# Jonetz/TreeDetection

Measured on AMD Instinct MI355X. Metric: tiles/sec (1000x1000 RGB+nDSM) predict_tiles model stage, higher is better.
Workload: dtype f32

## Files before the change

### include/treedet.h

```cpp
#ifndef TREEDET_H
#define TREEDET_H

#include <stddef.h>
#include <stdint.h>

#ifdef __cplusplus
extern "C" {
#endif

typedef int td_status;
typedef struct td_engine td_engine;

enum {
    TD_OK = 0,
    TD_ERR_INVALID = -1,
    TD_ERR_HIP = -2,
    TD_ERR_WEIGHTS = -3,
    TD_ERR_CAPACITY = -4,
    TD_ERR_STATE = -5,
    TD_ERR_UNSUPPORTED = -6
};

enum { TD_PRECISION_FP32 = 0, TD_PRECISION_FP16 = 1 };
enum { TD_INPUT_F32_CHW = 0,
       TD_INPUT_U8_HWC = 1 };

typedef struct td_model_desc {
    int32_t num_classes;
    int32_t precision;
    int32_t pre_nms_topk;
    int32_t post_nms_topk;
    int32_t detections_per_image;
    float rpn_nms_thresh;
    float score_thresh;
    float nms_thresh;
    float mask_thresh;
} td_model_desc;

typedef struct td_tensor_desc {
    const char* name;
    const float* data;
    int32_t ndim;
    int64_t shape[4];
} td_tensor_desc;

#define TD_MASK_SIDE 28

typedef struct td_detections {
    float* boxes;
    float* scores;
    int32_t* classes;
    int32_t* count;
    float* mask_probs;
    int32_t* mask_region;
    int64_t* mask_offset;
    uint32_t* mask_bits;
    int64_t mask_words_per_image;
} td_detections;

void td_model_desc_default(td_model_desc* desc);
td_status td_engine_create(const td_model_desc* desc, int device, td_engine** out);
td_status td_engine_load_weights(td_engine* e, const td_tensor_desc* tensors, size_t n);
td_status td_engine_reserve(td_engine* e, int max_batch, int max_hp, int max_wp);
td_status td_engine_forward(td_engine* e, const void* images, int input_format, const int32_t* hw_valid,
                            const int32_t* hw_out, int B, int Hp, int Wp, void* stream, td_detections* out);
#define TD_PHASE_STEM 6
td_status td_engine_forward_phase(td_engine* e, int phase, const void* images, int input_format, const int32_t* hw_valid,
                                  const int32_t* hw_out, int B, int Hp, int Wp, void* stream, td_detections* out);
td_status td_engine_tensor(td_engine* e, const char* name, void** dev_ptr, int64_t dims[4], int* elem_size);
td_status td_engine_read_tensor(td_engine* e, const char* name, void* dst_dev, int64_t bytes, void* stream);
#define TD_PROF_CATEGORIES 9
td_status td_engine_profile_enable(td_engine* e, int enable);
td_status td_engine_profile_read(td_engine* e, double* ms, int64_t* launches, double* flops, double* bytes, int reset);
#define TD_PROF_CLASSES 7
#define TD_CLS_WINO_GEMM 0
#define TD_CLS_WINO_XFORM 1
#define TD_CLS_CONV1X1 2
#define TD_CLS_CONV3X3 3
#define TD_CLS_FC 4
#define TD_CLS_MASK_HEAD 5
#define TD_CLS_TAIL 6
#define TD_PEAK_F32_MFMA_TFLOPS 157.3
#define TD_PEAK_F16_MFMA_TFLOPS 2500.0
#define TD_HBM_ACHIEVABLE_TBS 6.3
td_status td_engine_profile_classes(td_engine* e, double* ms, int64_t* launches, double* exec_flops, double* bytes, double* tmin_ms, int reset);
const char* td_last_error(void);
void td_engine_destroy(td_engine* e);

td_status td_resize_tile_u8(const uint8_t* src, int h, int w, int c, uint8_t* dst, int out_h, int out_w,
                            int dst_pitch_px, void* tmp_dev , void* stream);
td_status td_resize_batch_u8(const uint8_t* const* src_tiles, int n, int h, int w, int c, uint8_t* dst, int out_h,
                             int out_w, int dst_pitch_px, int64_t dst_image_stride_bytes, void* tmp_dev, void* stream);
td_status td_resize_bilinear_f64(const double* src, int c, int h, int w, float* dst, int out_h, int out_w, int dst_pitch_px,
                                 int64_t dst_plane_stride, void* stream);
td_status td_windows_u16_to_input(const uint16_t* raster, int height, int width, int c, const int32_t* windows, int n, int32_t* band1_max,
                                  float* dst, int out_h, int out_w, int dst_pitch_px, int64_t dst_plane_stride, int64_t dst_image_stride,
                                  void* stream);
void td_resize_shape(int h, int w, int short_edge, int max_size, int* out_h, int* out_w);

td_status td_bottleneck_tail_nhwc(const void* x, const void* w2, const float* scale2, const float* bias2, const void* w3,
                                  const float* scale3, const float* bias3, const void* shortcut, void* y, int B, int H, int W,
                                  int mid, int cout, int precision, void* stream);
td_status td_conv2d_nhwc(const void* x, const void* w, const float* scale, const float* bias,
                         const void* residual, int res_shift, void* y, int B, int H, int W, int Cin,
                         int Cout, int KH, int KW, int stride, int pad, int relu, int precision,
                         void* stream);
td_status td_conv2d_rows_nhwc(const void* x, const void* w, const float* scale, const float* bias, void* y, int B, int H, int W,
                              int Cin, int Cout, int KH, int KW, int pad, int relu, int out_mode, const int32_t* rows_dyn,
                              int rows_mul, int precision, void* stream);
td_status td_conv2d_head_nhwc(const void* x, const void* w, const float* bias, const void* head_w, const float* head_b,
                              float* head_y, int B, int H, int W, int Cin, int KH, int KW, int pad, int head_n, int precision,
                              void* stream);
td_status td_conv2d_winograd_nhwc(const float* x, const float* w, const float* scale, const float* bias, float* y, int B,
                                  int H, int W, int Cin, int Cout, int relu, void* stream);
td_status td_conv2d_winograd_head_nhwc(const float* x, const float* w, const float* bias, const float* head_w, const float* head_b,
                                       float* head_y, int B, int H, int W, int Cin, int head_n, void* stream);
td_status td_conv_path(const int32_t* rules, int64_t wino_elems, const int32_t* layer, const int32_t* call, const int32_t* head,
                       int32_t* out);
typedef struct td_workspace_row {
    char name[32];
    char public_name[32];
    int32_t kind;
    int32_t elem_size;
    int32_t phase;
    int32_t pad_;
    int64_t dims[4];
    int64_t alloc_bytes;
} td_workspace_row;
td_status td_workspace_plan(int precision, int winograd, int post_nms_topk, int detections_per_image, const int32_t* widths, int B,
                            int Hp, int Wp, td_workspace_row* rows, int cap, int* n_rows);
td_status td_nms(const float* boxes, const float* scores, int n, float iou_thresh, int32_t* keep_idx,
                 int32_t* keep_count, void* stream);
td_status td_roi_align(const void* feat, int H, int W, int C, const float* rois, int R, float spatial_scale,
                       int pooled, void* out, int precision, void* stream);
td_status td_paste_masks(const float* mask_probs, const float* boxes, int n, int out_h, int out_w,
                         float thresh, int32_t* mask_region, int64_t* mask_offset, uint32_t* mask_bits,
                         int64_t mask_words_cap, void* stream);

td_status td_paste_masks_batch(const float* mask_probs, const float* boxes, const int32_t* counts, const int32_t* out_hw,
                               int batch, int dets_per_image, float thresh, int32_t* mask_region, int64_t* mask_offset,
                               uint32_t* mask_bits, int64_t mask_words_per_image, void* stream);

#define TD_CONTOUR_MAX 256
td_status td_trace_contours_dev(const int32_t* mask_region, const int64_t* mask_offset, const uint32_t* mask_bits,
                                int64_t mask_words_per_image, const int32_t* counts, int batch, int dets_per_image,
                                int16_t* points, int points_cap, int32_t* image_points, int32_t* det_info,
                                int32_t* contour_info, void* stream);

int td_find_contours(const uint8_t* img, int h, int w, int32_t* points, int max_points, int32_t* starts,
                     int max_contours);
int td_tile_polygons_json(const int32_t* mask_region, const int64_t* mask_offset, const uint32_t* mask_bits,
                          int64_t mask_words, const float* scores, const int32_t* classes, int n,
                          const double* transform, const char* image_id, char* buf, int64_t cap, int64_t* needed);

int td_tile_prediction_file(int device, const int32_t* mask_region, const int64_t* mask_offset, const uint32_t* mask_bits_dev,
                            uint32_t* rows_host, int64_t mask_words, const float* scores, const int32_t* classes, int n,
                            const double* transform, const char* image_id, const char* path, int64_t* bytes_written);

int td_batch_prediction_files(int device, int n_tiles, int dets_per_image, const int32_t* mask_region, const int64_t* mask_offset,
                              const uint32_t* mask_bits_dev, uint32_t* rows_host, int64_t bits_stride_words, const float* scores,
                              const int32_t* classes, const int32_t* counts, const double* transforms, const char* image_id,
                              const char* const* paths, int threads, int32_t* status, int64_t* bytes_written);

int64_t td_tiff_lzw_decode(const uint8_t* src, int64_t n, uint8_t* dst, int64_t cap);
int64_t td_tiff_packbits_decode(const uint8_t* src, int64_t n, uint8_t* dst, int64_t cap);
int64_t td_tiff_lzw_encode(const uint8_t* src, int64_t n, uint8_t* dst, int64_t cap);
td_status td_tiff_lzw_decode_dev(const uint8_t* comp, const int64_t* block_off, const int64_t* block_nbytes, int nblocks,
                                 uint8_t* blocks_out, int64_t block_cap, int64_t* decoded, int32_t* status, void* stream);
td_status td_tiff_inflate_dev(const uint8_t* comp, const int64_t* block_off, const int64_t* block_nbytes, int nblocks,
                              uint8_t* blocks_out, int64_t block_cap, int64_t* decoded, int32_t* status, void* stream);
td_status td_tiff_inflate_verified_dev(const uint8_t* comp, const int64_t* block_off, const int64_t* block_nbytes, int nblocks,
                                       uint8_t* blocks_out, int64_t block_cap, int64_t* decoded, int32_t* status, int64_t* end_off,
                                       void* stream);
td_status td_tiff_adler32_blocks_dev(const uint8_t* blocks, int64_t block_cap, const int64_t* decoded, const uint8_t* comp,
                                     const int64_t* block_off, const int64_t* block_nbytes, const int64_t* end_off, int nblocks,
                                     int32_t* status, void* stream);
td_status td_adler32_dev(const uint8_t* data_dev, int64_t n, uint32_t* out_dev, void* stream);
int64_t td_tiff_inflate(const uint8_t* src, int64_t n, uint8_t* dst, int64_t cap);
int64_t td_tiff_inflate_verified(const uint8_t* src, int64_t n, uint8_t* dst, int64_t cap);
int64_t td_tiff_zstd_decode(const uint8_t* src, int64_t n, uint8_t* dst, int64_t cap);
#define TD_ZSTD_STATS 32
int64_t td_zstd_stream_stats(const uint8_t* src, int64_t n, int64_t* counters);
td_status td_tiff_zstd_decode_dev(const uint8_t* comp, const int64_t* block_off, const int64_t* block_nbytes, int nblocks,
                                  uint8_t* blocks_out, int64_t block_cap, int64_t* decoded, int32_t* status, uint8_t* scratch,
                                  int64_t scratch_bytes, void* stream);
int64_t td_tiff_zstd_scratch_bytes(int nblocks);
td_status td_tiff_blocks_to_image_dev(const uint8_t* blocks, int64_t block_cap, int block_w, int block_h, int blocks_across,
                                      int blocks_down, int spp, int predictor, uint8_t* image, int width, int height, void* stream);
td_status td_tiff_blocks_to_image_u16_dev(const uint8_t* blocks, int64_t block_cap, int block_w, int block_h, int blocks_across,
                                          int blocks_down, int spp, int predictor, uint16_t* image, int width, int height, void* stream);
td_status td_tiff_blocks_to_image_f32_dev(const uint8_t* blocks, int64_t block_cap, int block_w, int block_h, int blocks_across,
                                          int blocks_down, int spp, int predictor, float* image, int width, int height, void* stream);
td_status td_tiff_planes_to_image_dev(const uint8_t* blocks, int64_t block_cap, int block_w, int block_h, int blocks_across,
                                      int blocks_down, int spp, int plane_mask, int predictor, uint8_t* image, int width, int height,
                                      void* stream);
td_status td_tiff_planes_to_image_u16_dev(const uint8_t* blocks, int64_t block_cap, int block_w, int block_h, int blocks_across,
                                          int blocks_down, int spp, int plane_mask, int predictor, uint16_t* image, int width, int height,
                                          void* stream);
td_status td_tiff_planes_to_image_f32_dev(const uint8_t* blocks, int64_t block_cap, int block_w, int block_h, int blocks_across,
                                          int blocks_down, int spp, int plane_mask, int predictor, float* image, int width, int height,
                                          void* stream);
#define TD_JPEG_TABSET_BYTES 11904
td_status td_tiff_jpeg_plan(const uint8_t* tables, int64_t tables_len, const uint8_t* data, const int64_t* block_off,
                            const int64_t* block_nbytes, int nblocks, int photometric, int bands, int block_w, const int32_t* block_rows,
                            int64_t* block_info, int64_t* segs, int64_t seg_cap, void* tabsets, int64_t tabset_cap, int64_t* totals);
td_status td_tiff_jpeg_decode_dev(const uint8_t* comp, const int64_t* block_info, int nblocks, const int64_t* segs, int nseg,
                                  const void* tabsets, int16_t* coef, uint8_t* planes, int64_t coef_count, int32_t* status, uint8_t* image,
                                  int width, int height, int bands, int block_w, int block_h, int blocks_across, void* stream);
int64_t td_jpeg_decode(const uint8_t* src, int64_t n, uint8_t* dst, int64_t cap, int32_t* shape);
td_status td_tiff_jpeg_decode_long_dev(const uint8_t* comp, const int64_t* block_info, int nblocks, const int64_t* segs_short, int nshort,
                                       const int64_t* segs_long, int nlong, int subseq_bytes, const void* tabsets, int16_t* coef,
                                       uint8_t* planes, int64_t coef_count, int32_t* status, int64_t* stats, uint8_t* image, int width,
                                       int height, int bands, int block_w, int block_h, int blocks_across, void* stream);
int64_t td_jpeg_decode_sync(const uint8_t* src, int64_t n, uint8_t* dst, int64_t cap, int32_t* shape, int subseq_bytes, int lanes,
                            int64_t* stats);
int64_t td_read_window(int fd, int64_t file_off, int64_t row_stride, int64_t row_bytes, int64_t rows, uint8_t* dst);
int64_t td_read_windows(int fd, int n, const int64_t* file_off, int64_t row_stride, const int64_t* row_bytes, const int64_t* rows,
                        uint8_t* dst, const int64_t* dst_off, int threads);
int td_tiff_unpredict(void* data, int64_t rows, int64_t cols, int samples, int bytes_per_sample);
int td_tiff_unpredict_float(void* data, int64_t rows, int64_t cols, int samples, int bytes_per_sample);

int td_tile_polygons_json_dev(const int16_t* points, int64_t points_cap, const int32_t* det_info, const int32_t* contour_info,
                              const int32_t* mask_region, const int64_t* mask_offset, const uint32_t* mask_bits,
                              int64_t mask_words, const float* scores, const int32_t* classes, int n,
                              const double* transform, const char* image_id, char* buf, int64_t cap, int64_t* needed);

int td_simplify_ring(const double* xy, int n, double tolerance, double* out_xy, int out_cap);

int td_ring_is_valid(const double* xy, int n);
int td_stitch_tile_json(const char* json, int64_t len, const double* box, double tolerance, int32_t srs_id,
                        uint8_t* blobs, int64_t blob_cap, int64_t* blob_offsets, double* scores, int max_features,
                        int64_t* needed_bytes, int* needed_features);

int td_stitch_tile_files(const char* paths, const int64_t* path_offsets, int n_files, const double* boxes, double tolerance,
                         const int32_t* srs_ids, int threads, uint8_t* blobs, int64_t blob_cap, int64_t* blob_offsets,
                         double* scores, int max_features, int32_t* file_status, int64_t* needed_bytes, int* needed_features);

int td_region_relate(const double* ring_xy, const int64_t* ring_start, const int32_t* ring_poly, int n_rings,
                     const double* query_xy, const int64_t* query_start, int n_queries, uint8_t* flags);

#define TD_RELATE_QUERY_CAP 256
#define TD_RELATE_MEET_CAP 254
#define TD_RELATE_RING_CAP 64
td_status td_region_relate_dev(const double* ring_xy, const int64_t* ring_start, const int32_t* ring_poly, int n_rings, int64_t n_vertices,
                               const int32_t* edge_ring, const int32_t* bin_start, const int32_t* bin_edges, int n_bins,
                               int64_t n_bin_edges, double ymin, double ymax, double inv_h, const double* query_xy,
                               const int64_t* query_start, int n_queries, int64_t n_query_vertices, uint8_t* flags, int32_t* status,
                               int check_index, void* stream);

td_status td_crown_stats(const float* raster, int rows, int cols, const double* transform, const int32_t* window,
                         const float* circles, int n, int mode, float radius_scale, float* out, void* stream);

#define TD_ZONAL_RING_CAP 512
td_status td_crown_zonal_dev(const float* raster, int rows, int cols, const double* transform, const double* xy, int64_t n_xy,
                             const int64_t* start, int n, float* out, int32_t* pos, int32_t* status, void* stream);
// ... 46 lines not shown
```

### treedetection_amd/_lib.py

```python
from __future__ import annotations

import ctypes as C
import os
import threading
from typing import Optional

_HERE = os.path.dirname(os.path.abspath(__file__))
LIB_PATH = os.path.join(_HERE, "libtreedet_hip.so")

_lib: Optional[C.CDLL] = None
ERR_INVALID = -1
ERR_CAPACITY = -4
ERR_STATE = -5
ERR_UNSUPPORTED = -6
JPEG_TABSET_BYTES = 11904
SAMPLE_U8, SAMPLE_F32, SAMPLE_U16 = 0, 1, 2
RESAMPLE_MODES = {"f32": 0, "u8": 1, "ndvi": 2}
ZSTD_STATS = ("frames block_raw block_rle block_comp max_blocks_per_frame lit_raw lit_rle lit_huff lit_treeless lit_streams_1 lit_streams_4 "
              "hufw_direct hufw_fse seq0 LL_predef LL_rle LL_fse LL_repeat OF_predef OF_rle OF_fse OF_repeat ML_predef ML_rle ML_fse ML_repeat "
              "window_desc single_segment checksum seq_long seq_2byte skippable").split()
RING_PAIR_CAP, RING_PAIR_WPB, RING_PAIR_GRID = 1024, 4, 2048
RELATE_QUERY_CAP, RELATE_MEET_CAP, RELATE_RING_CAP = 256, 254, 64
ZONAL_RING_CAP = 512


class TdError(RuntimeError):
    """A libtreedet_hip call returned a negative status (message from td_last_error)."""


class ModelDesc(C.Structure):
    _fields_ = [("num_classes", C.c_int32), ("precision", C.c_int32), ("pre_nms_topk", C.c_int32),
                ("post_nms_topk", C.c_int32), ("detections_per_image", C.c_int32),
                ("rpn_nms_thresh", C.c_float), ("score_thresh", C.c_float), ("nms_thresh", C.c_float),
                ("mask_thresh", C.c_float)]


class TensorDesc(C.Structure):
    _fields_ = [("name", C.c_char_p), ("data", C.c_void_p), ("ndim", C.c_int32), ("shape", C.c_int64 * 4)]


class SeamSource(C.Structure):
    _fields_ = [("data", C.c_void_p), ("pitch", C.c_int64), ("rows", C.c_int32), ("row0", C.c_int32), ("col0", C.c_int32),
                ("r_lo", C.c_int32), ("c_lo", C.c_int32), ("r_hi", C.c_int32), ("c_hi", C.c_int32), ("has_own", C.c_int32),
                ("own", C.c_double)]


class WorkspaceRow(C.Structure):
    _fields_ = [("name", C.c_char * 32), ("public_name", C.c_char * 32), ("kind", C.c_int32), ("elem_size", C.c_int32),
                ("phase", C.c_int32), ("pad_", C.c_int32), ("dims", C.c_int64 * 4), ("alloc_bytes", C.c_int64)]


class Detections(C.Structure):
    _fields_ = [("boxes", C.c_void_p), ("scores", C.c_void_p), ("classes", C.c_void_p), ("count", C.c_void_p),
                ("mask_probs", C.c_void_p), ("mask_region", C.c_void_p), ("mask_offset", C.c_void_p),
                ("mask_bits", C.c_void_p), ("mask_words_per_image", C.c_int64)]


SIGNATURES = {
    "td_model_desc_default": (None, [C.POINTER(ModelDesc)]),
    "td_engine_create": (C.c_int, [C.POINTER(ModelDesc), C.c_int, C.POINTER(C.c_void_p)]),
    "td_engine_load_weights": (C.c_int, [C.c_void_p, C.POINTER(TensorDesc), C.c_size_t]),
    "td_engine_reserve": (C.c_int, [C.c_void_p, C.c_int, C.c_int, C.c_int]),
    "td_engine_forward": (C.c_int, [C.c_void_p, C.c_void_p, C.c_int, C.POINTER(C.c_int32), C.POINTER(C.c_int32),
                                    C.c_int, C.c_int, C.c_int, C.c_void_p, C.POINTER(Detections)]),
    "td_engine_forward_phase": (C.c_int, [C.c_void_p, C.c_int, C.c_void_p, C.c_int, C.POINTER(C.c_int32), C.POINTER(C.c_int32),
                                          C.c_int, C.c_int, C.c_int, C.c_void_p, C.POINTER(Detections)]),
    "td_engine_tensor": (C.c_int, [C.c_void_p, C.c_char_p, C.POINTER(C.c_void_p), C.POINTER(C.c_int64),
                                   C.POINTER(C.c_int)]),
    "td_engine_read_tensor": (C.c_int, [C.c_void_p, C.c_char_p, C.c_void_p, C.c_int64, C.c_void_p]),
    "td_engine_profile_enable": (C.c_int, [C.c_void_p, C.c_int]),
    "td_engine_profile_read": (C.c_int, [C.c_void_p, C.POINTER(C.c_double), C.POINTER(C.c_int64), C.POINTER(C.c_double),
                                         C.POINTER(C.c_double), C.c_int]),
    "td_engine_profile_classes": (C.c_int, [C.c_void_p, C.POINTER(C.c_double), C.POINTER(C.c_int64), C.POINTER(C.c_double),
                                            C.POINTER(C.c_double), C.POINTER(C.c_double), C.c_int]),
    "td_last_error": (C.c_char_p, []),
    "td_engine_destroy": (None, [C.c_void_p]),
    "td_resize_tile_u8": (C.c_int, [C.c_void_p, C.c_int, C.c_int, C.c_int, C.c_void_p, C.c_int, C.c_int, C.c_int,
                                    C.c_void_p, C.c_void_p]),
    "td_resize_batch_u8": (C.c_int, [C.POINTER(C.c_void_p), C.c_int, C.c_int, C.c_int, C.c_int, C.c_void_p, C.c_int, C.c_int,
                                     C.c_int, C.c_int64, C.c_void_p, C.c_void_p]),
    "td_bottleneck_tail_nhwc": (C.c_int, [C.c_void_p] * 9 + [C.c_int] * 6 + [C.c_void_p]),
    "td_resize_bilinear_f64": (C.c_int, [C.c_void_p, C.c_int, C.c_int, C.c_int, C.c_void_p, C.c_int, C.c_int, C.c_int, C.c_int64, C.c_void_p]),
    "td_windows_u16_to_input": (C.c_int, [C.c_void_p, C.c_int, C.c_int, C.c_int, C.c_void_p, C.c_int, C.c_void_p, C.c_void_p, C.c_int, C.c_int,
                                          C.c_int, C.c_int64, C.c_int64, C.c_void_p]),
    "td_resize_shape": (None, [C.c_int, C.c_int, C.c_int, C.c_int, C.POINTER(C.c_int), C.POINTER(C.c_int)]),
    "td_conv2d_nhwc": (C.c_int, [C.c_void_p, C.c_void_p, C.c_void_p, C.c_void_p, C.c_void_p, C.c_int, C.c_void_p]
                       + [C.c_int] * 11 + [C.c_void_p]),
    "td_conv2d_rows_nhwc": (C.c_int, [C.c_void_p] * 5 + [C.c_int] * 10 + [C.c_void_p, C.c_int, C.c_int, C.c_void_p]),
    "td_conv2d_head_nhwc": (C.c_int, [C.c_void_p] * 6 + [C.c_int] * 9 + [C.c_void_p]),
    "td_conv2d_winograd_head_nhwc": (C.c_int, [C.c_void_p] * 6 + [C.c_int] * 5 + [C.c_void_p]),
    "td_conv2d_winograd_nhwc": (C.c_int, [C.c_void_p] * 5 + [C.c_int] * 6 + [C.c_void_p]),
    "td_conv_path": (C.c_int, [C.POINTER(C.c_int32), C.c_int64, C.POINTER(C.c_int32), C.POINTER(C.c_int32), C.POINTER(C.c_int32),
                               C.POINTER(C.c_int32)]),
    "td_workspace_plan": (C.c_int, [C.c_int] * 4 + [C.POINTER(C.c_int32)] + [C.c_int] * 3 + [C.POINTER(WorkspaceRow), C.c_int, C.POINTER(C.c_int)]),
    "td_nms": (C.c_int, [C.c_void_p, C.c_void_p, C.c_int, C.c_float, C.c_void_p, C.c_void_p, C.c_void_p]),
    "td_roi_align": (C.c_int, [C.c_void_p, C.c_int, C.c_int, C.c_int, C.c_void_p, C.c_int, C.c_float, C.c_int,
                               C.c_void_p, C.c_int, C.c_void_p]),
    "td_paste_masks": (C.c_int, [C.c_void_p, C.c_void_p, C.c_int, C.c_int, C.c_int, C.c_float, C.c_void_p,
                                 C.c_void_p, C.c_void_p, C.c_int64, C.c_void_p]),
    "td_paste_masks_batch": (C.c_int, [C.c_void_p, C.c_void_p, C.c_void_p, C.POINTER(C.c_int32), C.c_int, C.c_int, C.c_float,
                                       C.c_void_p, C.c_void_p, C.c_void_p, C.c_int64, C.c_void_p]),
    "td_crown_stats": (C.c_int, [C.c_void_p, C.c_int, C.c_int, C.POINTER(C.c_double), C.POINTER(C.c_int32), C.c_void_p, C.c_int,
                                 C.c_int, C.c_float, C.c_void_p, C.c_void_p]),
    "td_crown_zonal_dev": (C.c_int, [C.c_void_p, C.c_int, C.c_int, C.POINTER(C.c_double), C.c_void_p, C.c_int64, C.c_void_p, C.c_int,
                                     C.c_void_p, C.c_void_p, C.c_void_p, C.c_void_p]),
    "td_crown_zonal": (C.c_int, [C.c_void_p, C.c_int, C.c_int, C.POINTER(C.c_double), C.c_void_p, C.c_int64, C.c_void_p, C.c_int,
                                 C.c_void_p, C.c_void_p, C.c_void_p]),
    "td_crown_labels_dev": (C.c_int, [C.c_int, C.c_int, C.POINTER(C.c_double), C.c_void_p, C.c_int64, C.c_void_p, C.c_void_p, C.c_int,
                                      C.c_void_p, C.c_void_p, C.c_void_p]),
    "td_crown_labels": (C.c_int, [C.c_int, C.c_int, C.POINTER(C.c_double), C.c_void_p, C.c_int64, C.c_void_p, C.c_void_p, C.c_int,
                                  C.c_void_p, C.c_void_p]),
    "td_resample_gdal_dev": (C.c_int, [C.c_void_p, C.c_int, C.c_int, C.c_int, C.c_int, C.POINTER(C.c_int32), C.c_int]
                             + [C.c_void_p] * 4 + [C.c_int, C.c_int64] + [C.c_void_p] * 4 + [C.c_int, C.c_int64]
                             + [C.c_void_p, C.c_void_p, C.c_int, C.c_void_p]),
    "td_seam_first_dev": (C.c_int, [C.c_void_p, C.c_int, C.c_int, C.c_int, C.c_int, C.c_double, C.POINTER(SeamSource), C.POINTER(SeamSource),
                                    C.c_void_p]),
    "td_crown_pairs_count": (C.c_int, [C.c_void_p, C.c_void_p, C.c_int, C.c_float, C.c_uint16, C.c_void_p, C.c_float, C.c_void_p, C.c_void_p,
                                       C.c_void_p]),
    "td_crown_pairs_fill": (C.c_int, [C.c_void_p, C.c_void_p, C.c_int, C.c_float, C.c_uint16, C.c_void_p, C.c_void_p, C.c_void_p, C.c_void_p]),
    "td_crown_pairs_greedy": (C.c_int, [C.c_void_p, C.c_void_p, C.c_void_p, C.c_void_p, C.c_int, C.c_void_p]),
    "td_ring_pairs_area_dev": (C.c_int, [C.c_void_p, C.c_void_p, C.c_int, C.c_void_p, C.c_void_p, C.c_int, C.c_void_p, C.c_int64, C.c_void_p,
                                         C.c_void_p, C.c_void_p]),
    "td_ring_pairs_area": (C.c_int, [C.c_void_p, C.c_void_p, C.c_int, C.c_void_p, C.c_void_p, C.c_int, C.c_void_p, C.c_int64, C.c_void_p,
                                     C.c_void_p]),
    "td_trace_contours_dev": (C.c_int, [C.c_void_p, C.c_void_p, C.c_void_p, C.c_int64, C.c_void_p, C.c_int, C.c_int, C.c_void_p,
                                        C.c_int, C.c_void_p, C.c_void_p, C.c_void_p, C.c_void_p]),
    "td_find_contours": (C.c_int, [C.c_void_p, C.c_int, C.c_int, C.c_void_p, C.c_int, C.c_void_p, C.c_int]),
    "td_batch_prediction_files": (C.c_int, [C.c_int, C.c_int, C.c_int, C.c_void_p, C.c_void_p, C.c_void_p, C.c_void_p, C.c_int64, C.c_void_p,
                                          C.c_void_p, C.c_void_p, C.c_void_p, C.c_char_p, C.POINTER(C.c_char_p), C.c_int, C.c_void_p, C.c_void_p]),
    "td_tiff_lzw_decode": (C.c_int64, [C.c_void_p, C.c_int64, C.c_void_p, C.c_int64]),
    "td_tiff_packbits_decode": (C.c_int64, [C.c_void_p, C.c_int64, C.c_void_p, C.c_int64]),
    "td_tiff_lzw_encode": (C.c_int64, [C.c_void_p, C.c_int64, C.c_void_p, C.c_int64]),
    "td_tiff_inflate": (C.c_int64, [C.c_void_p, C.c_int64, C.c_void_p, C.c_int64]),
    "td_tiff_inflate_dev": (C.c_int, [C.c_void_p, C.c_void_p, C.c_void_p, C.c_int, C.c_void_p, C.c_int64, C.c_void_p, C.c_void_p, C.c_void_p]),
    "td_tiff_inflate_verified": (C.c_int64, [C.c_void_p, C.c_int64, C.c_void_p, C.c_int64]),
    "td_tiff_inflate_verified_dev": (C.c_int, [C.c_void_p, C.c_void_p, C.c_void_p, C.c_int, C.c_void_p, C.c_int64, C.c_void_p, C.c_void_p, C.c_void_p,
                                               C.c_void_p]),
    "td_tiff_zstd_decode": (C.c_int64, [C.c_void_p, C.c_int64, C.c_void_p, C.c_int64]),
    "td_zstd_stream_stats": (C.c_int64, [C.c_void_p, C.c_int64, C.c_void_p]),
    "td_tiff_zstd_decode_dev": (C.c_int, [C.c_void_p, C.c_void_p, C.c_void_p, C.c_int, C.c_void_p, C.c_int64, C.c_void_p, C.c_void_p, C.c_void_p,
                                          C.c_int64, C.c_void_p]),
    "td_tiff_zstd_scratch_bytes": (C.c_int64, [C.c_int]),
    "td_tiff_adler32_blocks_dev": (C.c_int, [C.c_void_p, C.c_int64, C.c_void_p, C.c_void_p, C.c_void_p, C.c_void_p, C.c_void_p, C.c_int, C.c_void_p,
                                             C.c_void_p]),
    "td_adler32_dev": (C.c_int, [C.c_void_p, C.c_int64, C.c_void_p, C.c_void_p]),
    "td_tiff_lzw_decode_dev": (C.c_int, [C.c_void_p, C.c_void_p, C.c_void_p, C.c_int, C.c_void_p, C.c_int64, C.c_void_p, C.c_void_p, C.c_void_p]),
    "td_tiff_blocks_to_image_dev": (C.c_int, [C.c_void_p, C.c_int64, C.c_int, C.c_int, C.c_int, C.c_int, C.c_int, C.c_int, C.c_void_p, C.c_int, C.c_int, C.c_void_p]),
    "td_tiff_blocks_to_image_u16_dev": (C.c_int, [C.c_void_p, C.c_int64, C.c_int, C.c_int, C.c_int, C.c_int, C.c_int, C.c_int, C.c_void_p, C.c_int,
                                                  C.c_int, C.c_void_p]),
    "td_tiff_blocks_to_image_f32_dev": (C.c_int, [C.c_void_p, C.c_int64, C.c_int, C.c_int, C.c_int, C.c_int, C.c_int, C.c_int, C.c_void_p, C.c_int,
                                                  C.c_int, C.c_void_p]),
    "td_tiff_planes_to_image_dev": (C.c_int, [C.c_void_p, C.c_int64, C.c_int, C.c_int, C.c_int, C.c_int, C.c_int, C.c_int, C.c_int, C.c_void_p,
                                              C.c_int, C.c_int, C.c_void_p]),
    "td_tiff_planes_to_image_u16_dev": (C.c_int, [C.c_void_p, C.c_int64, C.c_int, C.c_int, C.c_int, C.c_int, C.c_int, C.c_int, C.c_int, C.c_void_p,
                                                  C.c_int, C.c_int, C.c_void_p]),
    "td_tiff_planes_to_image_f32_dev": (C.c_int, [C.c_void_p, C.c_int64, C.c_int, C.c_int, C.c_int, C.c_int, C.c_int, C.c_int, C.c_int, C.c_void_p,
                                                  C.c_int, C.c_int, C.c_void_p]),
    "td_tiff_jpeg_plan": (C.c_int, [C.c_void_p, C.c_int64, C.c_void_p, C.c_void_p, C.c_void_p, C.c_int, C.c_int, C.c_int, C.c_int, C.c_void_p,
                                    C.c_void_p, C.c_void_p, C.c_int64, C.c_void_p, C.c_int64, C.c_void_p]),
    "td_tiff_jpeg_decode_dev": (C.c_int, [C.c_void_p, C.c_void_p, C.c_int, C.c_void_p, C.c_int, C.c_void_p, C.c_void_p, C.c_void_p, C.c_int64,
                                          C.c_void_p, C.c_void_p] + [C.c_int] * 6 + [C.c_void_p]),
    "td_jpeg_decode": (C.c_int64, [C.c_void_p, C.c_int64, C.c_void_p, C.c_int64, C.c_void_p]),
    "td_tiff_jpeg_decode_long_dev": (C.c_int, [C.c_void_p, C.c_void_p, C.c_int, C.c_void_p, C.c_int, C.c_void_p, C.c_int, C.c_int, C.c_void_p,
                                               C.c_void_p, C.c_void_p, C.c_int64, C.c_void_p, C.c_void_p, C.c_void_p] + [C.c_int] * 6 + [C.c_void_p]),
    "td_jpeg_decode_sync": (C.c_int64, [C.c_void_p, C.c_int64, C.c_void_p, C.c_int64, C.c_void_p, C.c_int, C.c_int, C.c_void_p]),
    "td_read_windows": (C.c_int64, [C.c_int, C.c_int, C.c_void_p, C.c_int64, C.c_void_p, C.c_void_p, C.c_void_p, C.c_void_p, C.c_int]),
    "td_tiff_unpredict": (C.c_int, [C.c_void_p, C.c_int64, C.c_int64, C.c_int, C.c_int]),
    "td_tiff_unpredict_float": (C.c_int, [C.c_void_p, C.c_int64, C.c_int64, C.c_int, C.c_int]),
    "td_region_relate": (C.c_int, [C.c_void_p, C.c_void_p, C.c_void_p, C.c_int, C.c_void_p, C.c_void_p, C.c_int, C.c_void_p]),
    "td_region_relate_dev": (C.c_int, [C.c_void_p, C.c_void_p, C.c_void_p, C.c_int, C.c_int64, C.c_void_p, C.c_void_p, C.c_void_p, C.c_int, C.c_int64,
                                       C.c_double, C.c_double, C.c_double, C.c_void_p, C.c_void_p, C.c_int, C.c_int64, C.c_void_p, C.c_void_p,
                                       C.c_int, C.c_void_p]),
    "td_simplify_ring": (C.c_int, [C.c_void_p, C.c_int, C.c_double, C.c_void_p, C.c_int]),
    "td_ring_is_valid": (C.c_int, [C.c_void_p, C.c_int]),
    "td_stitch_tile_json": (C.c_int, [C.c_char_p, C.c_int64, C.POINTER(C.c_double), C.c_double, C.c_int32, C.c_void_p,
                                      C.c_int64, C.c_void_p, C.c_void_p, C.c_int, C.POINTER(C.c_int64), C.POINTER(C.c_int)]),
    "td_stitch_tile_files": (C.c_int, [C.c_char_p, C.c_void_p, C.c_int, C.c_void_p, C.c_double, C.c_void_p, C.c_int, C.c_void_p, C.c_int64,
                                       C.c_void_p, C.c_void_p, C.c_int, C.c_void_p, C.POINTER(C.c_int64), C.POINTER(C.c_int)]),
    "td_tile_polygons_json_dev": (C.c_int, [C.c_void_p, C.c_int64, C.c_void_p, C.c_void_p, C.c_void_p, C.c_void_p, C.c_void_p, C.c_int64,
                                            C.c_void_p, C.c_void_p, C.c_int, C.POINTER(C.c_double), C.c_char_p, C.c_void_p, C.c_int64,
                                            C.POINTER(C.c_int64)]),
    "td_read_window": (C.c_int64, [C.c_int, C.c_int64, C.c_int64, C.c_int64, C.c_int64, C.c_void_p]),
    "td_tile_prediction_file": (C.c_int, [C.c_int, C.c_void_p, C.c_void_p, C.c_void_p, C.c_void_p, C.c_int64, C.c_void_p, C.c_void_p,
                                          C.c_int, C.POINTER(C.c_double), C.c_char_p, C.c_char_p, C.POINTER(C.c_int64)]),
    "td_tile_polygons_json": (C.c_int, [C.c_void_p, C.c_void_p, C.c_void_p, C.c_int64, C.c_void_p, C.c_void_p, C.c_int,
                                        C.POINTER(C.c_double), C.c_char_p, C.c_void_p, C.c_int64, C.POINTER(C.c_int64)]),
}


def load() -> C.CDLL:
    global _lib
    if _lib is not None:
        return _lib
    host_only = os.environ.get("TD_HOST_LIB")
    if host_only:
        lib = C.CDLL(host_only, mode=C.RTLD_GLOBAL)
        for name, (res, args) in SIGNATURES.items():
            fn = getattr(lib, name, None)
            if fn is not None:
                fn.restype = res
                fn.argtypes = args
        _lib = lib
        return lib
    if not os.path.exists(LIB_PATH):
        raise TdError(f"{LIB_PATH} not found — build it first: python -c 'import __graft_entry__ as g; g.build()' "
                      f"(or make -C treedetection_amd/csrc). There is no CPU fallback.")
    import torch

    lib = C.CDLL(LIB_PATH, mode=C.RTLD_GLOBAL)
    for name, (res, args) in SIGNATURES.items():
        fn = getattr(lib, name)
        fn.restype = res
        fn.argtypes = args
    _lib = lib
    return lib


def check(status: int, what: str = "") -> None:
    if status < 0:
        msg = load().td_last_error().decode("utf-8", "replace")
        raise TdError(f"{what or 'libtreedet_hip'} failed ({status}): {msg}")


CONV_FORMS = ("direct", "split", "winograd F(2x2)", "winograd F(4x4)", "winograd F(4x4) folded")
CONV_HEADS = ("own launch", "in the output transform", "if the tile owns 256 channels")


def conv_path(rules, wino_elems, layer, call, head=None) -> dict:
    arr = lambda v, n: (C.c_int32 * n)(*[int(x) for x in v])
    out = (C.c_int32 * 10)()
    check(load().td_conv_path(arr(rules, 8), int(wino_elems), arr(layer, 9), arr(call, 10), arr(head, 9) if head is not None else None, out),
          "td_conv_path")
    return {"form": CONV_FORMS[out[0]], "head": CONV_HEADS[out[1]], "key": tuple(out[3:8]) if out[2] else None,
            "slab_tiles": out[8], "fold_group": out[9]}
# ... 42 lines not shown
```

### treedetection_amd/csrc/api.cpp

```cpp
#include "common.h"
#include "detect.h"
#include <cstdarg>
#include <cstdio>
#include <cmath>
#include <cstdlib>
#include <vector>


namespace {
td_status scratch(void** p, size_t bytes) {
    TD_HIP_CHECK(hipMalloc(p, bytes ? bytes : 16));
    return TD_OK;
}
}

extern "C" {

void td_model_desc_default(td_model_desc* d) {
    d->num_classes = 1;
    d->precision = TD_PRECISION_FP32;
    d->pre_nms_topk = 1000;
    d->post_nms_topk = 1000;
    d->detections_per_image = 100;
    d->rpn_nms_thresh = 0.7f;
    d->score_thresh = 0.3f;
    d->nms_thresh = 0.5f;
    d->mask_thresh = 0.5f;
}

static td_status conv2d_api(ConvArgs& a, int precision, void* stream);

td_status td_conv2d_nhwc(const void* x, const void* w, const float* scale, const float* bias,
                         const void* residual, int res_shift, void* y, int B, int H, int W, int Cin,
                         int Cout, int KH, int KW, int stride, int pad, int relu, int precision,
                         void* stream) {
    TD_REQUIRE(x && w && y, "td_conv2d_nhwc: null pointer");
    TD_REQUIRE(stride >= 1 && KH >= 1 && KW >= 1 && B >= 1, "td_conv2d_nhwc: bad geometry");
    ConvArgs a{};
    a.x = x; a.w = w; a.scale = scale; a.bias = bias; a.res = residual; a.y = y;
    a.B = B; a.H = H; a.W = W; a.Cin = Cin; a.Cout = Cout; a.KH = KH; a.KW = KW;
    a.stride = stride; a.pad = pad;
    a.Ho = (H + 2 * pad - KH) / stride + 1;
    a.Wo = (W + 2 * pad - KW) / stride + 1;
    a.res_shift = res_shift; a.relu = relu; a.out_mode = 0;
    a.M = B * a.Ho * a.Wo; a.m_dyn = nullptr; a.m_mul = 1;
    a.out_f32 = (precision & 0x10000) && (precision & 0xff) == TD_PRECISION_FP16 ? 1 : 0;
    a.tile_cfg = ((precision >> 8) & 0xff) - 1;
    a.tile_strict = (precision & 0x20000) ? 1 : 0;
    return conv2d_api(a, precision, stream);
}

td_status td_conv2d_rows_nhwc(const void* x, const void* w, const float* scale, const float* bias, void* y, int B, int H, int W,
                              int Cin, int Cout, int KH, int KW, int pad, int relu, int out_mode, const int32_t* rows_dyn,
                              int rows_mul, int precision, void* stream) {
    TD_REQUIRE(x && w && y, "td_conv2d_rows_nhwc: null pointer");
    TD_REQUIRE(KH >= 1 && KW >= 1 && B >= 1, "td_conv2d_rows_nhwc: bad geometry");
    TD_REQUIRE(out_mode == 0 || out_mode == 1, "td_conv2d_rows_nhwc: out_mode %d (0 plain, 1 pixel shuffle)", out_mode);
    TD_REQUIRE(!rows_dyn || rows_mul >= 1, "td_conv2d_rows_nhwc: rows_mul %d with a device row count", rows_mul);
    ConvArgs a{};
    a.x = x; a.w = w; a.scale = scale; a.bias = bias; a.y = y;
    a.B = B; a.H = H; a.W = W; a.Cin = Cin; a.Cout = Cout; a.KH = KH; a.KW = KW;
    a.stride = 1; a.pad = pad;
    a.Ho = H + 2 * pad - KH + 1;
    a.Wo = W + 2 * pad - KW + 1;
    a.relu = relu; a.out_mode = out_mode;
    a.M = B * a.Ho * a.Wo; a.m_dyn = rows_dyn; a.m_mul = rows_dyn ? rows_mul : 1;
    a.out_f32 = (precision & 0x10000) && (precision & 0xff) == TD_PRECISION_FP16 ? 1 : 0;
    a.tile_cfg = ((precision >> 8) & 0xff) - 1;
    a.tile_strict = (precision & 0x20000) ? 1 : 0;
    return conv2d_api(a, precision, stream);
}

td_status td_conv2d_head_nhwc(const void* x, const void* w, const float* bias, const void* head_w, const float* head_b,
                              float* head_y, int B, int H, int W, int Cin, int KH, int KW, int pad, int head_n, int precision,
                              void* stream) {
    TD_REQUIRE(x && w && head_w && head_y, "td_conv2d_head_nhwc: null pointer");
    TD_REQUIRE((precision & 0xff) == TD_PRECISION_FP16, "td_conv2d_head_nhwc: float16 tensors only");
    TD_REQUIRE(KH >= 1 && KW >= 1 && B >= 1 && head_n >= 1 && head_n <= 32, "td_conv2d_head_nhwc: bad geometry");
    ConvArgs a{};
    a.x = x; a.w = w; a.bias = bias;
    a.B = B; a.H = H; a.W = W; a.Cin = Cin; a.Cout = 256; a.KH = KH; a.KW = KW;
    a.stride = 1; a.pad = pad;
    a.Ho = H + 2 * pad - KH + 1;
    a.Wo = W + 2 * pad - KW + 1;
    a.relu = 1; a.M = B * a.Ho * a.Wo; a.m_mul = 1;
    a.tile_cfg = ((precision >> 8) & 0xff) - 1;
    TD_REQUIRE(conv_head_capable(a.tile_cfg, TD_PRECISION_FP16), "td_conv2d_head_nhwc: tile id %d does not own 256 output channels per block", a.tile_cfg);
    a.head_w = head_w; a.head_b = head_b; a.head_y = head_y; a.head_n = head_n;
    a.y = head_y;
    return conv2d_api(a, precision, stream);
}

static td_status conv2d_api(ConvArgs& a, int precision, void* stream) {
    hipStream_t s = static_cast<hipStream_t>(stream);
    ConvArgs with_frag = a;
    with_frag.w_frag = a.w;
    with_frag.w_split = a.w;
    if (conv_tile(a.tile_cfg) && conv_tile(a.tile_cfg)->family == TILE_SPLIT && !conv_tile_refusal(a.tile_cfg, with_frag, precision & 0xff)) {
        const size_t n = (size_t)a.Cout * a.Cin;
        std::vector<float> wh(n);
        std::vector<unsigned char> packed;
        TD_HIP_CHECK(hipStreamSynchronize(s));
        TD_HIP_CHECK(hipMemcpy(wh.data(), a.w, n * sizeof(float), hipMemcpyDeviceToHost));
        conv_split_pack(wh.data(), a.Cout, a.Cin, packed);
        void* ws = nullptr;
        td_status st = scratch(&ws, packed.size());
        if (st < 0) return st;
        hipError_t herr = hipMemcpy(ws, packed.data(), packed.size(), hipMemcpyHostToDevice);
        a.w_split = ws;
        if (herr == hipSuccess) st = conv2d_launch(a, precision & 0xff, s);
        hipError_t herr2 = hipStreamSynchronize(s);
        (void)hipFree(ws);
        if (st < 0) return st;
        TD_HIP_CHECK(herr);
        TD_HIP_CHECK(herr2);
        return TD_OK;
    }
    if (!conv_tile(a.tile_cfg) || !conv_tile(a.tile_cfg)->frag || conv_tile_refusal(a.tile_cfg, with_frag, precision & 0xff))
        return conv2d_launch(a, precision & 0xff, s);
    const int es = (precision & 0xff) == TD_PRECISION_FP16 ? 2 : 4;
    const size_t n = (size_t)a.Cout * a.KH * a.KW * a.Cin;
    std::vector<unsigned char> bits(n * es), packed;
    TD_HIP_CHECK(hipStreamSynchronize(s));
    TD_HIP_CHECK(hipMemcpy(bits.data(), a.w, n * es, hipMemcpyDeviceToHost));
    conv_bd_pack(bits.data(), es, a.Cout, a.KH, a.KW, a.Cin, packed);
    void* wf = nullptr;
    td_status st = scratch(&wf, packed.size());
    if (st < 0) return st;
    hipError_t herr = hipMemcpy(wf, packed.data(), packed.size(), hipMemcpyHostToDevice);
    a.w_frag = wf;
    if (herr == hipSuccess) st = conv2d_launch(a, precision & 0xff, s);
    hipError_t herr2 = hipStreamSynchronize(s);
    (void)hipFree(wf);
    if (st < 0) return st;
    TD_HIP_CHECK(herr);
    TD_HIP_CHECK(herr2);
    return TD_OK;
}

static td_status wino_api(const float* x, const float* w, const float* scale, const float* bias, float* y, int B, int H, int W, int Cin,
                          int Cout, int relu, void* stream, const float* head_w, const float* head_b, float* head_y, int head_n);

td_status td_conv2d_winograd_nhwc(const float* x, const float* w, const float* scale, const float* bias, float* y, int B, int H,
                                  int W, int Cin, int Cout, int relu, void* stream) {
    TD_REQUIRE(y, "td_conv2d_winograd_nhwc: bad arguments");
    return wino_api(x, w, scale, bias, y, B, H, W, Cin, Cout, relu, stream, nullptr, nullptr, nullptr, 0);
}

td_status td_conv2d_winograd_head_nhwc(const float* x, const float* w, const float* bias, const float* head_w, const float* head_b,
                                       float* head_y, int B, int H, int W, int Cin, int head_n, void* stream) {
    TD_REQUIRE(head_w && head_y && head_n >= 1 && head_n <= 32, "td_conv2d_winograd_head_nhwc: bad arguments");
    return wino_api(x, w, nullptr, bias, nullptr, B, H, W, Cin, 256, 1, stream, head_w, head_b, head_y, head_n);
}

static td_status wino_api(const float* x, const float* w, const float* scale, const float* bias, float* y, int B, int H, int W, int Cin,
                          int Cout, int relu, void* stream, const float* head_w, const float* head_b, float* head_y, int head_n) {
    TD_REQUIRE(x && w && B >= 1 && H >= 1 && W >= 1, "td_conv2d_winograd_nhwc: bad arguments");
    TD_REQUIRE(Cin % 32 == 0 && Cout % 4 == 0, "td_conv2d_winograd_nhwc: Cin must be a multiple of 32, Cout of 4");
    hipStream_t s = static_cast<hipStream_t>(stream);
    const char* tenv = getenv("TD_WINO_TILE");
    const bool f43 = head_w || (tenv && atoi(tenv) == 4);
    const int P = f43 ? 36 : 16;
    const size_t T = f43 ? (size_t)B * ((H + 3) / 4) * ((W + 3) / 4) : (size_t)B * ((H + 1) / 2) * ((W + 1) / 2);
    std::vector<float> wh((size_t)Cout * 9 * Cin), uh((size_t)P * Cout * Cin);
    TD_HIP_CHECK(hipMemcpy(wh.data(), w, wh.size() * sizeof(float), hipMemcpyDeviceToHost));
    if (f43) wino43_filter_transform(wh.data(), Cout, Cin, uh.data());
    else wino_filter_transform(wh.data(), Cout, Cin, uh.data());
    void *U = nullptr, *V = nullptr, *Mb = nullptr;
    td_status st;
    if ((st = scratch(&U, uh.size() * 4)) < 0 || (st = scratch(&V, P * T * Cin * 4)) < 0 || (st = scratch(&Mb, P * T * Cout * 4)) < 0) {
        (void)hipFree(U); (void)hipFree(V); (void)hipFree(Mb);
        return st;
    }
    TD_HIP_CHECK(hipMemcpy(U, uh.data(), uh.size() * 4, hipMemcpyHostToDevice));
    const char* folde = getenv("TD_WINO_FOLD");
    const bool fold = f43 && !head_w && folde && atoi(folde) != 0;
    if (fold) TD_REQUIRE(wino43_fused_ok(B, H, W, Cin, Cout), "td_conv2d_winograd_nhwc: TD_WINO_FOLD needs Cin %% 128 == 0, Cout %% 64 == 0");
    const char* fenv = getenv("TD_WINO_FUSED");
    WinoRun r{};
    r.form = fold ? CONV_WINO43_FOLD : f43 ? CONV_WINO43 : CONV_WINO22;
    r.fused_input = !fenv || atoi(fenv) != 0;
    r.slab_tiles = (int)T; r.fold_group = B;
    r.x = x; r.U = static_cast<float*>(U); r.scale = scale; r.bias = bias; r.y = y;
    r.B = B; r.H = H; r.W = W; r.cin = Cin; r.cout = Cout; r.relu = relu;
    r.V = static_cast<float*>(V); r.M = static_cast<float*>(Mb); r.m_mul = 1; r.gemm_cfg = -1;
    r.head_w = head_w; r.head_b = head_b; r.head_y = head_y; r.head_n = head_n;
    st = wino_run(r, s);
    hipError_t herr = hipStreamSynchronize(s);
    (void)hipFree(U); (void)hipFree(V); (void)hipFree(Mb);
    if (st < 0) return st;
    TD_HIP_CHECK(herr);
    return TD_OK;
}

td_status td_resize_tile_u8(const uint8_t* src, int h, int w, int c, uint8_t* dst, int out_h, int out_w,
                            int dst_pitch_px, void* tmp_dev, void* stream) {
    return resize_tile_u8_launch(src, h, w, c, dst, out_h, out_w, dst_pitch_px, tmp_dev, static_cast<hipStream_t>(stream));
}

td_status td_resize_batch_u8(const uint8_t* const* src_tiles, int n, int h, int w, int c, uint8_t* dst, int out_h,
                             int out_w, int dst_pitch_px, int64_t dst_image_stride_bytes, void* tmp_dev, void* stream) {
    return resize_batch_u8_launch(src_tiles, n, h, w, c, dst, out_h, out_w, dst_pitch_px, (size_t)dst_image_stride_bytes,
                                  tmp_dev, static_cast<hipStream_t>(stream));
}

td_status td_bottleneck_tail_nhwc(const void* x, const void* w2, const float* scale2, const float* bias2, const void* w3,
                                  const float* scale3, const float* bias3, const void* shortcut, void* y, int B, int H, int W,
                                  int mid, int cout, int precision, void* stream) {
    TD_REQUIRE(x && w2 && w3 && shortcut && y && B > 0 && H > 0 && W > 0, "td_bottleneck_tail_nhwc: null argument or empty tensor");
    TailArgs a{};
    a.x = x; a.w2 = w2; a.scale2 = scale2; a.bias2 = bias2; a.w3 = w3; a.scale3 = scale3; a.bias3 = bias3; a.res = shortcut; a.y = y;
    a.B = B; a.H = H; a.W = W; a.MID = mid; a.COUT = cout; a.M = B * H * W;
    return bottleneck_tail_launch(a, precision, static_cast<hipStream_t>(stream));
}

td_status td_resize_bilinear_f64(const double* src, int c, int h, int w, float* dst, int out_h, int out_w, int dst_pitch_px,
                                 int64_t dst_plane_stride, void* stream) {
    return resize_bilinear_f64_launch(src, c, h, w, dst, out_h, out_w, dst_pitch_px, (long long)dst_plane_stride, static_cast<hipStream_t>(stream));
}

td_status td_windows_u16_to_input(const uint16_t* raster, int height, int width, int c, const int32_t* windows, int n, int32_t* band1_max,
                                  float* dst, int out_h, int out_w, int dst_pitch_px, int64_t dst_plane_stride, int64_t dst_image_stride,
                                  void* stream) {
    return windows_u16_to_input_launch(raster, height, width, c, windows, n, band1_max, dst, out_h, out_w, dst_pitch_px,
                                       (long long)dst_plane_stride, (long long)dst_image_stride, static_cast<hipStream_t>(stream));
}

void td_resize_shape(int h, int w, int short_edge, int max_size, int* out_h, int* out_w) {
    const double scale = (double)short_edge / (double)(h < w ? h : w);
    double newh, neww;
    if (h < w) { newh = short_edge; neww = scale * w; }
    else { newh = scale * h; neww = short_edge; }
    const double mx = newh > neww ? newh : neww;
    if (mx > max_size) {
        const double s2 = (double)max_size / mx;
        newh *= s2;
        neww *= s2;
    }
    *out_h = (int)(newh + 0.5);
    *out_w = (int)(neww + 0.5);
}

td_status td_nms(const float* boxes, const float* scores, int n, float iou_thresh, int32_t* keep_idx,
                 int32_t* keep_count, void* stream) {
    TD_REQUIRE(boxes && scores && keep_idx && keep_count, "td_nms: null pointer");
    TD_REQUIRE(n >= 0 && n <= 32768, "td_nms: n=%d must be in [0, 32768]", n);
    hipStream_t s = static_cast<hipStream_t>(stream);
    if (n == 0) {
        TD_HIP_CHECK(hipMemsetAsync(keep_count, 0, sizeof(int32_t), s));
        return TD_OK;
    }
    void *sb = nullptr, *ss = nullptr, *si = nullptr, *sc = nullptr, *mk = nullptr, *kp = nullptr;
    td_status st;
    if ((st = scratch(&sb, sizeof(float) * 4 * n)) < 0) return st;
    if ((st = scratch(&ss, sizeof(float) * n)) < 0) return st;
    if ((st = scratch(&si, sizeof(int) * n)) < 0) return st;
    if ((st = scratch(&sc, sizeof(int))) < 0) return st;
    if ((st = scratch(&mk, sizeof(unsigned long long) * n * td_cdiv(n, 64))) < 0) return st;
    if ((st = scratch(&kp, sizeof(int) * n)) < 0) return st;
    if (n > 1024) {
        st = nms_big_launch(boxes, scores, n, iou_thresh, (float*)sb, (float*)ss, (int*)si, (int*)sc, (unsigned long long*)mk, (int*)kp, keep_count, s);
    } else {
        st = sort_boxes_launch(boxes, scores, nullptr, nullptr, 1, n, (float*)sb, (float*)ss, (int*)si, (int*)sc, s);
        if (st >= 0) st = nms_launch((float*)sb, (int*)sc, nullptr, 1, n, iou_thresh, (unsigned long long*)mk, (int*)kp, keep_count, n, s);
    }
    if (st >= 0) st = gather_keep_launch((int*)si, (int*)kp, keep_count, n, keep_idx, s);
    hipError_t herr = hipStreamSynchronize(s);
    (void)hipFree(sb); (void)hipFree(ss); (void)hipFree(si); (void)hipFree(sc); (void)hipFree(mk); (void)hipFree(kp);
    if (st < 0) return st;
    TD_HIP_CHECK(herr);
    return TD_OK;
}

td_status td_roi_align(const void* feat, int H, int W, int C, const float* rois, int R, float spatial_scale,
                       int pooled, void* out, int precision, void* stream) {
    TD_REQUIRE(feat && rois && out, "td_roi_align: null pointer");
    TD_REQUIRE(H >= 1 && W >= 1 && pooled >= 1 && R >= 0, "td_roi_align: bad geometry");
    if (R == 0) return TD_OK;
    return roi_align_single_launch(feat, H, W, C, rois, R, spatial_scale, pooled, out, precision, static_cast<hipStream_t>(stream));
}

td_status td_paste_masks(const float* mask_probs, const float* boxes, int n, int out_h, int out_w, float thresh,
                         int32_t* mask_region, int64_t* mask_offset, uint32_t* mask_bits, int64_t mask_words_cap,
                         void* stream) {
    TD_REQUIRE(mask_probs && boxes && mask_region && mask_offset && mask_bits, "td_paste_masks: null pointer");
    TD_REQUIRE(n >= 0 && n <= 1024 && out_h >= 1 && out_w >= 1, "td_paste_masks: bad shape");
    if (n == 0) return TD_OK;
    hipStream_t s = static_cast<hipStream_t>(stream);
    void* cnt = nullptr;
    td_status st = scratch(&cnt, sizeof(int));
    if (st < 0) return st;
    TD_HIP_CHECK(hipMemcpy(cnt, &n, sizeof(int), hipMemcpyHostToDevice));
    ImgSizes outsz{};
    outsz.h[0] = out_h;
    outsz.w[0] = out_w;
    st = paste_masks_launch(mask_probs, boxes, (int*)cnt, outsz, 1, n, thresh, mask_region,
                            reinterpret_cast<long long*>(mask_offset), mask_bits, mask_words_cap, s);
    hipError_t herr = hipStreamSynchronize(s);
    (void)hipFree(cnt);
    if (st < 0) return st;
    TD_HIP_CHECK(herr);
    return TD_OK;
}

td_status td_paste_masks_batch(const float* mask_probs, const float* boxes, const int32_t* counts, const int32_t* out_hw,
                               int batch, int dets_per_image, float thresh, int32_t* mask_region, int64_t* mask_offset,
                               uint32_t* mask_bits, int64_t mask_words_per_image, void* stream) {
    TD_REQUIRE(mask_probs && boxes && counts && out_hw && mask_region && mask_offset && mask_bits,
               "td_paste_masks_batch: null pointer");
    TD_REQUIRE(batch >= 1 && batch <= TD_MAX_BATCH && dets_per_image >= 1 && dets_per_image <= 1024,
               "td_paste_masks_batch: batch %d (max %d) / detections per image %d (max 1024)", batch, TD_MAX_BATCH, dets_per_image);
    ImgSizes outsz{};
    for (int i = 0; i < batch; ++i) {
        TD_REQUIRE(out_hw[2 * i] >= 1 && out_hw[2 * i + 1] >= 1, "td_paste_masks_batch: bad output size of image %d", i);
        outsz.h[i] = out_hw[2 * i];
        outsz.w[i] = out_hw[2 * i + 1];
        const int64_t need = (int64_t)dets_per_image * ((outsz.w[i] + 2 + 31) / 32) * outsz.h[i];
        TD_REQUIRE(mask_words_per_image >= need, "td_paste_masks_batch: image %d needs %lld mask words, capacity %lld", i,
                   (long long)need, (long long)mask_words_per_image);
    }
    return paste_masks_launch(mask_probs, boxes, counts, outsz, batch, dets_per_image, thresh, mask_region,
                              reinterpret_cast<long long*>(mask_offset), mask_bits, mask_words_per_image,
                              static_cast<hipStream_t>(stream));
}

}
```

### treedetection_amd/csrc/bottleneck.hip

```cpp
#include "common.h"
#include "conv_tiles.h"
#include <cstdlib>
#include <utility>

namespace {

constexpr int cmax(int x, int y) { return x > y ? x : y; }

template <typename F, int... I>
__device__ __forceinline__ void static_for_impl(F&& f, std::integer_sequence<int, I...>) {
    (f(std::integral_constant<int, I>{}), ...);
}
template <int N, typename F>
__device__ __forceinline__ void static_for(F&& f) {
    static_for_impl(f, std::make_integer_sequence<int, N>{});
}

template <typename T, int MID, bool OVERLAP, int MT, bool FAST = false>
struct TailGeom {
    static constexpr int ES = sizeof(T);
    static constexpr int KE = Elem<T>::PER_CHUNK;
    static constexpr int KC = MID / KE;
    static constexpr int BM = 64 * MT, THREADS = 256, LDROWS = 32;
    static constexpr int NT1 = MID / 64;
    static constexpr int STAGE1 = 2 * (BM + MID) * CHUNK_BYTES;
    static constexpr int W3_BYTES = KC * 128 * CHUNK_BYTES;
    static_assert(!FAST || MT == 1, "the wave-private epilogue is written for 64-row blocks");
    static constexpr int EPI_BYTES = FAST ? 4 * 16 * 64 * 4 : conv_epilogue_lds_bytes<T, MT, 2, 2, 2, 1, false>();
    static constexpr int EPI_OFF = OVERLAP || (FAST && ES == 2) ? W3_BYTES : 0;
    static constexpr int R0 = cmax(STAGE1, cmax(W3_BYTES, EPI_OFF + EPI_BYTES));
    static constexpr int T2_BYTES = KC * BM * CHUNK_BYTES;
    static constexpr int LDS_BYTES = R0 + T2_BYTES;
    static constexpr int BPC = 160 * 1024 / LDS_BYTES >= 4 ? 4 : 160 * 1024 / LDS_BYTES;
};

template <typename T, int MID, bool OVERLAP, int MT, bool FAST>
__device__ __forceinline__ void bottleneck_tail_body(const TailArgs& a, char* lds) {
    typedef TailGeom<T, MID, OVERLAP, MT, FAST> G;
    constexpr int ES = G::ES, KE = G::KE, KC = G::KC, BM = G::BM, LDROWS = G::LDROWS, NT1 = G::NT1;
    constexpr int AROWS = BM / LDROWS, BROWS1 = MID / LDROWS, BROWS3 = 128 / LDROWS;
    char* As = lds;
    char* Bs = lds + 2 * BM * CHUNK_BYTES;
    char* W3s = lds;
    char* Epi = lds + G::EPI_OFF;
    char* T2s = lds + G::R0;

    const int M = a.M;
    const int nblk = (M + BM - 1) / BM;
    if ((int)blockIdx.x >= nblk) return;
    const int m0 = xcd_remap(blockIdx.x, nblk) * BM;
    const int tid = threadIdx.x;
    const int lane = tid & 63, wave = tid >> 6;
    const int wm = wave >> 1, wn = wave & 1;
    const int ld_c = tid & 7, ld_r = tid >> 3;

    const int K2 = 9 * MID;
    const int nit = 9 * KC;
    const unsigned pix_bytes = (unsigned)MID * ES;
    const __amdgpu_buffer_rsrc_t xrsrc = __builtin_amdgcn_make_buffer_rsrc(
        const_cast<void*>(a.x), 0, (int)((size_t)a.B * a.H * a.W * pix_bytes), 0x00020000);
    const __amdgpu_buffer_rsrc_t w2rsrc = __builtin_amdgcn_make_buffer_rsrc(
        const_cast<void*>(a.w2), 0, (int)((size_t)MID * K2 * ES), 0x00020000);
    const __amdgpu_buffer_rsrc_t w3rsrc = __builtin_amdgcn_make_buffer_rsrc(
        const_cast<void*>(a.w3), 0, (int)((size_t)a.COUT * MID * ES), 0x00020000);
    constexpr unsigned OOB = 0xfffffff0u;
    const unsigned src_piece = (unsigned)(ld_c ^ ((ld_r >> 1) & 7)) * 16;

    unsigned a_off[AROWS], a_ok[AROWS];
#pragma unroll
    for (int i = 0; i < AROWS; ++i) {
        const int m = m0 + ld_r + LDROWS * i;
        a_off[i] = 0;
        a_ok[i] = 0;
        if (m < M) {
            const int hw = a.H * a.W;
            const int b = m / hw;
            const int rem = m - b * hw;
            const int oy = rem / a.W;
            const int ox = rem - oy * a.W;
            const int iy0 = oy - 1, ix0 = ox - 1;
            a_off[i] = (unsigned)((b * a.H + iy0) * a.W + ix0) * pix_bytes + src_piece;
            for (int ky = 0; ky < 3; ++ky)
                for (int kx = 0; kx < 3; ++kx)
                    if ((unsigned)(iy0 + ky) < (unsigned)a.H && (unsigned)(ix0 + kx) < (unsigned)a.W)
                        a_ok[i] |= 1u << (ky * 3 + kx);
        }
    }
    unsigned b_off[BROWS1];
#pragma unroll
    for (int i = 0; i < BROWS1; ++i) b_off[i] = (unsigned)(ld_r + LDROWS * i) * (unsigned)K2 * ES + src_piece;

    typedef __attribute__((address_space(3))) void lds_void;
    const unsigned wave_rows = (unsigned)__builtin_amdgcn_readfirstlane(wave) * 8u;
    int ld_tap = 0, ld_ky = 0, ld_kx = 0, ld_cc = 0;
    auto stage = [&](int buf) {
        const unsigned xs = (unsigned)(ld_ky * a.W + ld_kx) * pix_bytes + (unsigned)ld_cc * CHUNK_BYTES;
        const unsigned ws = (unsigned)ld_tap * pix_bytes + (unsigned)ld_cc * CHUNK_BYTES;
#pragma unroll
        for (int i = 0; i < AROWS; ++i) {
            const unsigned off = ((a_ok[i] >> ld_tap) & 1u) ? a_off[i] + xs : OOB;
            char* dst = As + ((unsigned)buf * BM + (unsigned)LDROWS * i + wave_rows) * CHUNK_BYTES;
            __builtin_amdgcn_raw_ptr_buffer_load_lds(xrsrc, (lds_void*)dst, 16, off, 0, 0, 0);
        }
#pragma unroll
        for (int i = 0; i < BROWS1; ++i) {
            char* dst = Bs + ((unsigned)buf * MID + (unsigned)LDROWS * i + wave_rows) * CHUNK_BYTES;
            __builtin_amdgcn_raw_ptr_buffer_load_lds(w2rsrc, (lds_void*)dst, 16, b_off[i] + ws, 0, 0, 0);
        }
        if (++ld_kx == 3) {
            ld_kx = 0;
            ++ld_ky;
        }
        if (++ld_tap == 9) {
            ld_tap = 0;
            ld_ky = 0;
            ld_kx = 0;
            ++ld_cc;
        }
    };

    const unsigned swz = (lane >> 1) & 7, hi = lane >> 5;
    unsigned frag_off[4];
#pragma unroll
    for (int kk = 0; kk < 4; ++kk) frag_off[kk] = (unsigned)(lane & 31) * CHUNK_BYTES + (((unsigned)(2 * kk) + hi) ^ swz) * 16;

    float sc2[NT1], bi2[NT1];
#pragma unroll
    for (int j = 0; j < NT1; ++j) {
        const int n = wn * 32 * NT1 + j * 32 + (lane & 31);
        sc2[j] = a.scale2 ? a.scale2[n] : 1.f;
        bi2[j] = a.bias2 ? a.bias2[n] : 0.f;
    }
    constexpr int NP = MID / 32;
    [[maybe_unused]] float sc3[NP][2], bi3[NP][2];
    if constexpr (FAST) {
#pragma unroll
        for (int nc = 0; nc < NP; ++nc)
#pragma unroll
            for (int j = 0; j < 2; ++j) {
                const int n = nc * 128 + wn * 64 + j * 32 + (lane & 31);
                sc3[nc][j] = a.scale3 ? a.scale3[n] : 1.f;
                bi3[nc][j] = a.bias3 ? a.bias3[n] : 0.f;
            }
    }

    f32x16 acc2[MT][NT1];
#pragma unroll
    for (int i = 0; i < MT; ++i)
#pragma unroll
        for (int j = 0; j < NT1; ++j)
#pragma unroll
            for (int r = 0; r < 16; ++r) acc2[i][j][r] = 0.f;

#if defined(TD_TAIL_DIAG) && (TD_TAIL_DIAG & 1)
    if (false)
#endif
    {
    stage(0);
    asm volatile("s_waitcnt vmcnt(0)" ::: "memory");
    __builtin_amdgcn_s_barrier();
    }
#if defined(TD_TAIL_DIAG) && (TD_TAIL_DIAG & 1)
    for (int it = 0; it < 0; ++it) {
#else
    for (int it = 0; it < nit; ++it) {
#endif
        const int cur = it & 1;
        if (it + 1 < nit) stage(cur ^ 1);
        const char* Ab = &As[(cur * BM + wm * 32 * MT) * CHUNK_BYTES];
        const char* Bb = &Bs[(cur * MID + wn * 32 * NT1) * CHUNK_BYTES];
#pragma unroll
        for (int kk = 0; kk < 4; ++kk) {
            f32x4 fa[MT], fb[NT1];
#pragma unroll
            for (int i = 0; i < MT; ++i) fa[i] = *reinterpret_cast<const f32x4*>(Ab + i * 32 * CHUNK_BYTES + frag_off[kk]);
#pragma unroll
            for (int j = 0; j < NT1; ++j) fb[j] = *reinterpret_cast<const f32x4*>(Bb + j * 32 * CHUNK_BYTES + frag_off[kk]);
#pragma unroll
            for (int i = 0; i < MT; ++i)
#pragma unroll
                for (int j = 0; j < NT1; ++j) Elem<T>::mma(fa[i], fb[j], acc2[i][j]);
        }
        asm volatile("s_waitcnt vmcnt(0)" ::: "memory");
        asm volatile("s_waitcnt lgkmcnt(0)" ::: "memory");
        __builtin_amdgcn_s_barrier();
    }

    auto stage_w3 = [&](int nc) {
#pragma unroll
        for (int kc = 0; kc < KC; ++kc)
#pragma unroll
            for (int i = 0; i < BROWS3; ++i) {
                const unsigned n = (unsigned)nc * 128u + (unsigned)(ld_r + LDROWS * i);
                const unsigned off = n < (unsigned)a.COUT ? n * pix_bytes + (unsigned)kc * CHUNK_BYTES + src_piece : OOB;
                char* dst = W3s + ((unsigned)kc * 128 + (unsigned)LDROWS * i + wave_rows) * CHUNK_BYTES;
                __builtin_amdgcn_raw_ptr_buffer_load_lds(w3rsrc, (lds_void*)dst, 16, off, 0, 0, 0);
            }
    };
    stage_w3(0);

    typedef unsigned u32x4 __attribute__((ext_vector_type(4)));
    constexpr int NDMA3 = KC * BROWS3;
    const int er = lane >> 3, ec = (lane & 7) * 8;
    [[maybe_unused]] u32x4 rb[2][4];
    [[maybe_unused]] unsigned eoff[4];
    [[maybe_unused]] __amdgpu_buffer_rsrc_t rrsrc, yrsrc;
    [[maybe_unused]] auto load_res = [&](int nc, int slot) __attribute__((always_inline)) {
#pragma unroll
        for (int k = 0; k < 4; ++k)
            rb[slot][k] = __builtin_amdgcn_raw_buffer_load_b128(rrsrc, eoff[k] == OOB ? OOB : eoff[k] + (unsigned)nc * 256u, 0, 0);
    };
    const int er4 = lane >> 4, ec4 = (lane & 15) * 4;
    [[maybe_unused]] u32x4 rbf[8];
    [[maybe_unused]] unsigned eoff8[8];
    [[maybe_unused]] auto load_res4 = [&](int nc) __attribute__((always_inline)) {
#pragma unroll
        for (int k = 0; k < 8; ++k)
            rbf[k] = __builtin_amdgcn_raw_buffer_load_b128(rrsrc, eoff8[k] == OOB ? OOB : eoff8[k] + (unsigned)nc * 512u, 0, 0);
    };
    if constexpr (FAST && sizeof(T) == 4) {
        const int bytes = (int)((size_t)M * a.COUT * ES);
        rrsrc = __builtin_amdgcn_make_buffer_rsrc(const_cast<void*>(a.res ? a.res : a.y), 0, bytes, 0x00020000);
        yrsrc = __builtin_amdgcn_make_buffer_rsrc(a.y, 0, bytes, 0x00020000);
#pragma unroll
        for (int k = 0; k < 8; ++k) {
            const int m = m0 + wm * 32 + 4 * k + er4;
            eoff8[k] = m < M ? ((unsigned)m * (unsigned)a.COUT + (unsigned)(wn * 64 + ec4)) * ES : OOB;
        }
#if !(defined(TD_TAIL_DIAG) && (TD_TAIL_DIAG & 4))
        if (a.res) load_res4(0);
#endif
    }
    if constexpr (FAST && sizeof(T) == 2) {
        const int bytes = (int)((size_t)M * a.COUT * ES);
        rrsrc = __builtin_amdgcn_make_buffer_rsrc(const_cast<void*>(a.res ? a.res : a.y), 0, bytes, 0x00020000);
        yrsrc = __builtin_amdgcn_make_buffer_rsrc(a.y, 0, bytes, 0x00020000);
#pragma unroll
        for (int k = 0; k < 4; ++k) {
            const int m = m0 + wm * 32 + 8 * k + er;
            eoff[k] = m < M ? ((unsigned)m * (unsigned)a.COUT + (unsigned)(wn * 64 + ec)) * ES : OOB;
        }
#if !(defined(TD_TAIL_DIAG) && (TD_TAIL_DIAG & 4))
        if (a.res) {
            load_res(0, 0);
            load_res(1, 1);
        }
#endif
    }

#pragma unroll
    for (int j = 0; j < NT1; ++j) {
        const int n = wn * 32 * NT1 + j * 32 + (lane & 31);
        const float sc = sc2[j], bi = bi2[j];
        const unsigned c = (unsigned)n / KE, e = (unsigned)n % KE;
        const unsigned piece = (e * ES) >> 4, inb = (e * ES) & 15;
#pragma unroll
        for (int i = 0; i < MT; ++i) {
            if constexpr (sizeof(T) == 4) {
#pragma unroll
                for (int q = 0; q < 16; ++q) {
                    float t = acc2[i][j][q];
                    if (a.scale2) t = __fmul_rn(t, sc);
                    if (a.bias2) t = __fadd_rn(t, bi);
                    t = t > 0.f ? t : 0.f;
                    const unsigned row = (unsigned)(wm * 32 * MT + i * 32 + (q & 3) + 8 * (q >> 2) + 4 * (lane >> 5));
                    *reinterpret_cast<float*>(T2s + (c * BM + row) * CHUNK_BYTES + ((piece ^ ((row >> 1) & 7)) << 4) + inb) = t;
                }
            } else {
                const int odd = lane & 1;
                const unsigned inb2 = ((e & ~1u) * ES) & 15;
#pragma unroll
                for (int q = 0; q < 16; q += 2) {
                    float t0 = acc2[i][j][q], t1 = acc2[i][j][q + 1];
                    if (a.scale2) { t0 = __fmul_rn(t0, sc); t1 = __fmul_rn(t1, sc); }
                    if (a.bias2) { t0 = __fadd_rn(t0, bi); t1 = __fadd_rn(t1, bi); }
                    t0 = t0 > 0.f ? t0 : 0.f;
                    t1 = t1 > 0.f ? t1 : 0.f;
                    const float give = odd ? t0 : t1;
                    const float got = __builtin_bit_cast(float, __builtin_amdgcn_update_dpp(
                        0, __builtin_bit_cast(int, give), 0xB1 , 0xf, 0xf, false));
                    typedef _Float16 f16x2 __attribute__((ext_vector_type(2)));
                    f16x2 pk;
                    pk[0] = (_Float16)(odd ? got : t0);
                    pk[1] = (_Float16)(odd ? t1 : got);
                    const unsigned row = (unsigned)(wm * 32 * MT + i * 32 + (q & 3) + 8 * (q >> 2) + 4 * (lane >> 5) + odd);
                    *reinterpret_cast<f16x2*>(T2s + (c * BM + row) * CHUNK_BYTES + ((piece ^ ((row >> 1) & 7)) << 4) + inb2) = pk;
                }
            }
        }
    }
    if constexpr (FAST) {
        if (a.res) asm volatile("s_waitcnt vmcnt(8) lgkmcnt(0)" ::: "memory");
        else asm volatile("s_waitcnt vmcnt(0) lgkmcnt(0)" ::: "memory");
    } else {
        asm volatile("s_waitcnt vmcnt(0) lgkmcnt(0)" ::: "memory");
    }
    __builtin_amdgcn_s_barrier();

#if defined(TD_TAIL_DIAG) && (TD_TAIL_DIAG & 2)
    if (tid == 0 && m0 == 0x7fffff00) static_cast<T*>(a.y)[0] = *reinterpret_cast<const T*>(T2s);
    return;
#endif
    if constexpr (FAST && sizeof(T) == 4) {
        float* Ew = reinterpret_cast<float*>(Epi) + (wave * 16 * 64);
        auto piece4 = [&](auto nc_c) __attribute__((always_inline)) {
            constexpr int nc = decltype(nc_c)::value;
            f32x16 acc3[2];
#pragma unroll
            for (int j = 0; j < 2; ++j)
#pragma unroll
                for (int r = 0; r < 16; ++r) acc3[j][r] = 0.f;
#pragma unroll
            for (int kc = 0; kc < KC; ++kc) {
                const char* Ab = T2s + (kc * BM + wm * 32) * CHUNK_BYTES;
                const char* Bb = W3s + (kc * 128 + wn * 64) * CHUNK_BYTES;
#pragma unroll
                for (int kk = 0; kk < 4; ++kk) {
                    const f32x4 fa = *reinterpret_cast<const f32x4*>(Ab + frag_off[kk]);
                    f32x4 fb[2];
#pragma unroll
                    for (int j = 0; j < 2; ++j) fb[j] = *reinterpret_cast<const f32x4*>(Bb + j * 32 * CHUNK_BYTES + frag_off[kk]);
#pragma unroll
                    for (int j = 0; j < 2; ++j) Elem<T>::mma(fa, fb[j], acc3[j]);
                }
            }
            asm volatile("s_waitcnt lgkmcnt(0)" ::: "memory");
            __builtin_amdgcn_s_barrier();
            f32x4 out[8];
#pragma unroll
            for (int h = 0; h < 2; ++h) {
#pragma unroll
                for (int g = 0; g < 2; ++g)
#pragma unroll
                    for (int e = 0; e < 4; ++e) {
                        const int lr = e + 8 * g + 4 * (lane >> 5);
                        const int flip = (((lr >> 2) & 1) << 5) ^ ((lr & 1) << 2);
#pragma unroll
                        for (int j = 0; j < 2; ++j) {
                            float t = acc3[j][4 * (2 * h + g) + e];
                            if (a.scale3) t = __fmul_rn(t, sc3[nc][j]);
                            if (a.bias3) t = __fadd_rn(t, bi3[nc][j]);
                            Ew[lr * 64 + ((j * 32 + (lane & 31)) ^ flip)] = t;
                        }
                    }
                __builtin_amdgcn_wave_barrier();
#pragma unroll
                for (int p = 0; p < 4; ++p) {
                    const int lr = 4 * p + er4;
                    const int flip = (((lr >> 2) & 1) << 5) ^ ((lr & 1) << 2);
                    const f32x4 v = *reinterpret_cast<const f32x4*>(&Ew[lr * 64 + (ec4 ^ flip)]);
                    const f32x4 rs = __builtin_bit_cast(f32x4, rbf[4 * h + p]);
                    f32x4 o;
#pragma unroll
                    for (int q = 0; q < 4; ++q) {
                        float t = v[q];
#if !(defined(TD_TAIL_DIAG) && (TD_TAIL_DIAG & 4))
                        if (a.res) t = __fadd_rn(t, rs[q]);
#endif
                        o[q] = t > 0.f ? t : 0.f;
                    }
                    out[4 * h + p] = o;
                }
                __builtin_amdgcn_wave_barrier();
            }
            if constexpr (nc + 1 < NP) {
                asm volatile("s_waitcnt lgkmcnt(0)" ::: "memory");
                __builtin_amdgcn_s_barrier();
                stage_w3(nc + 1);
#if !(defined(TD_TAIL_DIAG) && (TD_TAIL_DIAG & 4))
                if (a.res) {
                    load_res4(nc + 1);
                    asm volatile("s_waitcnt vmcnt(8)" ::: "memory");
                } else
#endif
                {
                    asm volatile("s_waitcnt vmcnt(0)" ::: "memory");
                }
                __builtin_amdgcn_s_barrier();
            }
#if !(defined(TD_TAIL_DIAG) && (TD_TAIL_DIAG & 8))
#pragma unroll
            for (int k = 0; k < 8; ++k)
                __builtin_amdgcn_raw_buffer_store_b128(__builtin_bit_cast(u32x4, out[k]), yrsrc, eoff8[k] == OOB ? OOB : eoff8[k] + (unsigned)nc * 512u, 0, 0);
#else
            if (m0 == 0x7fffff00) __builtin_amdgcn_raw_buffer_store_b128(__builtin_bit_cast(u32x4, out[0] + out[7]), yrsrc, 0, 0, 0);
#endif
        };
        static_for<NP>(piece4);
        return;
    }
    if constexpr (FAST && sizeof(T) == 2) {
        float* Ew = reinterpret_cast<float*>(Epi) + (wave * 16 * 64);
        auto piece = [&](auto nc_c) __attribute__((always_inline)) {
            constexpr int nc = decltype(nc_c)::value;
            f32x16 acc3[2];
#pragma unroll
            for (int j = 0; j < 2; ++j)
#pragma unroll
                for (int r = 0; r < 16; ++r) acc3[j][r] = 0.f;
#pragma unroll
            for (int kc = 0; kc < KC; ++kc) {
                const char* Ab = T2s + (kc * BM + wm * 32) * CHUNK_BYTES;
                const char* Bb = W3s + (kc * 128 + wn * 64) * CHUNK_BYTES;
#pragma unroll
                for (int kk = 0; kk < 4; ++kk) {
                    const f32x4 fa = *reinterpret_cast<const f32x4*>(Ab + frag_off[kk]);
                    f32x4 fb[2];
#pragma unroll
                    for (int j = 0; j < 2; ++j) fb[j] = *reinterpret_cast<const f32x4*>(Bb + j * 32 * CHUNK_BYTES + frag_off[kk]);
#pragma unroll
                    for (int j = 0; j < 2; ++j) Elem<T>::mma(fa, fb[j], acc3[j]);
                }
            }
            asm volatile("s_waitcnt lgkmcnt(0)" ::: "memory");
            __builtin_amdgcn_s_barrier();
            if constexpr (nc + 1 < NP) stage_w3(nc + 1);
            u32x4 out[4];
#pragma unroll
            for (int h = 0; h < 2; ++h) {
#pragma unroll
                for (int g = 0; g < 2; ++g)
#pragma unroll
                    for (int e = 0; e < 4; ++e) {
                        const int lr = e + 8 * g + 4 * (lane >> 5);
                        const int flip = (((lr >> 2) & 1) << 5) ^ ((lr & 1) << 2);
#pragma unroll
                        for (int j = 0; j < 2; ++j) {
                            float t = acc3[j][4 * (2 * h + g) + e];
                            if (a.scale3) t = __fmul_rn(t, sc3[nc][j]);
                            if (a.bias3) t = __fadd_rn(t, bi3[nc][j]);
                            Ew[lr * 64 + ((j * 32 + (lane & 31)) ^ flip)] = t;
                        }
                    }
                __builtin_amdgcn_wave_barrier();
#pragma unroll
                for (int p = 0; p < 2; ++p) {
                    const int lr = 8 * p + er;
                    const int flip = (((lr >> 2) & 1) << 5) ^ ((lr & 1) << 2);
                    f32x4 v[2];
                    v[0] = *reinterpret_cast<const f32x4*>(&Ew[lr * 64 + (ec ^ flip)]);
                    v[1] = *reinterpret_cast<const f32x4*>(&Ew[lr * 64 + ((ec + 4) ^ flip)]);
                    if constexpr (nc == 0) {
                        if (h == 0 && p == 0) asm volatile("s_waitcnt vmcnt(%0)" ::"n"(4 + (NP > 1 ? NDMA3 : 0)) : "memory");
                    }
                    typedef _Float16 f16x8v __attribute__((ext_vector_type(8)));
                    const f16x8v rs = __builtin_bit_cast(f16x8v, rb[nc & 1][2 * h + p]);
                    f16x8v o;
#pragma unroll
                    for (int q = 0; q < 8; ++q) {
                        float t = v[q >> 2][q & 3];
#if !(defined(TD_TAIL_DIAG) && (TD_TAIL_DIAG & 4))
                        if (a.res) t = __fadd_rn(t, (float)rs[q]);
#endif
                        t = t > 0.f ? t : 0.f;
                        o[q] = (_Float16)t;
                    }
                    out[2 * h + p] = __builtin_bit_cast(u32x4, o);
                }
                __builtin_amdgcn_wave_barrier();
            }
            if constexpr (nc + 1 < NP) {
                asm volatile("s_waitcnt vmcnt(0)" ::: "memory");
                __builtin_amdgcn_s_barrier();
            }
#if !(defined(TD_TAIL_DIAG) && (TD_TAIL_DIAG & 8))
#pragma unroll
            for (int k = 0; k < 4; ++k)
                __builtin_amdgcn_raw_buffer_store_b128(out[k], yrsrc, eoff[k] == OOB ? OOB : eoff[k] + (unsigned)nc * 256u, 0, 0);
#else
            if (m0 == 0x7fffff00) __builtin_amdgcn_raw_buffer_store_b128(out[0] + out[1] + out[2] + out[3], yrsrc, 0, 0, 0);
#endif
            if constexpr (nc + 2 < NP) {
#if !(defined(TD_TAIL_DIAG) && (TD_TAIL_DIAG & 4))
                if (a.res) load_res(nc + 2, nc & 1);
#endif
            }
        };
        static_for<NP>(piece);
        return;
    }
    ConvArgs e{};
    e.y = a.y; e.res = a.res; e.scale = a.scale3; e.bias = a.bias3;
#if defined(TD_TAIL_DIAG) && (TD_TAIL_DIAG & 4)
    e.res = nullptr;
#endif
    e.Cout = a.COUT; e.relu = 1; e.out_mode = 0; e.res_shift = 0; e.Ho = a.H; e.Wo = a.W;
    const int npieces = (a.COUT + 127) / 128;
    for (int nc = 0; nc < npieces; ++nc) {
        f32x16 acc3[MT][2];
#pragma unroll
        for (int i = 0; i < MT; ++i)
#pragma unroll
            for (int j = 0; j < 2; ++j)
#pragma unroll
                for (int r = 0; r < 16; ++r) acc3[i][j][r] = 0.f;
#pragma unroll
        for (int kc = 0; kc < KC; ++kc) {
            const char* Ab = T2s + (kc * BM + wm * 32 * MT) * CHUNK_BYTES;
            const char* Bb = W3s + (kc * 128 + wn * 64) * CHUNK_BYTES;
#pragma unroll
            for (int kk = 0; kk < 4; ++kk) {
                f32x4 fa[MT], fb[2];
#pragma unroll
                for (int i = 0; i < MT; ++i) fa[i] = *reinterpret_cast<const f32x4*>(Ab + i * 32 * CHUNK_BYTES + frag_off[kk]);
#pragma unroll
                for (int j = 0; j < 2; ++j) fb[j] = *reinterpret_cast<const f32x4*>(Bb + j * 32 * CHUNK_BYTES + frag_off[kk]);
#pragma unroll
                for (int i = 0; i < MT; ++i)
#pragma unroll
                    for (int j = 0; j < 2; ++j) Elem<T>::mma(fa[i], fb[j], acc3[i][j]);
            }
        }
        asm volatile("s_waitcnt lgkmcnt(0)" ::: "memory");
        __builtin_amdgcn_s_barrier();
        const bool more = nc + 1 < npieces;
        if (OVERLAP && more) stage_w3(nc + 1);
        conv_epilogue<T, T, MT, 2, 2, 2, 1, false>(e, acc3, Epi, M, m0, nc * 128, tid, lane, wm, wn);
        if (more) {
            if (!OVERLAP) {
                __syncthreads();
                stage_w3(nc + 1);
            }
            asm volatile("s_waitcnt vmcnt(0)" ::: "memory");
            __builtin_amdgcn_s_barrier();
        }
    }
}

template <typename T, int MID, bool OVERLAP, int MT, bool FAST, int BPC>
__global__ __launch_bounds__(256, BPC)
void bottleneck_tail_kernel(const TailArgs a) {
    static_assert(BPC >= 1 && BPC * TailGeom<T, MID, OVERLAP, MT, FAST>::LDS_BYTES <= 160 * 1024, "LDS footprint does not allow that many blocks per CU");
    __shared__ __attribute__((aligned(16))) char lds[TailGeom<T, MID, OVERLAP, MT, FAST>::LDS_BYTES];
    bottleneck_tail_body<T, MID, OVERLAP, MT, FAST>(a, lds);
}

template <typename T, int MID, bool OVERLAP, int MT, bool FAST = false>
td_status launch_tail(const TailArgs& a, hipStream_t stream) {
    typedef TailGeom<T, MID, OVERLAP, MT, FAST> G;
    const int tiles = td_cdiv(a.M, G::BM);
    hipLaunchKernelGGL((bottleneck_tail_kernel<T, MID, OVERLAP, MT, FAST, G::BPC>), dim3(tiles), dim3(256), 0, stream, a);
    TD_KERNEL_CHECK();
    return TD_OK;
}

}

bool bottleneck_tail_ok(int precision, int mid, int cout) {
    if (cout != 4 * mid) return false;
    if (precision == TD_PRECISION_FP32) return mid == 64;
    return mid == 64 || mid == 128;
}

td_status bottleneck_tail_launch(const TailArgs& a, int precision, hipStream_t stream) {
    TD_REQUIRE(bottleneck_tail_ok(precision, a.MID, a.COUT), "bottleneck tail: unsupported shape (precision %d, mid %d, out %d)", precision, a.MID, a.COUT);
    TD_REQUIRE(a.M == a.B * a.H * a.W && a.M > 0, "bottleneck tail: M must be B*H*W");
    const size_t es = precision == TD_PRECISION_FP16 ? 2 : 4;
    TD_REQUIRE((size_t)a.M * a.MID * es < 0xfffffff0ull - (1u << 20), "bottleneck tail: input tensor must stay below 4 GB (32-bit buffer offsets)");
    static const int forced = getenv("TD_TAIL_BM") ? atoi(getenv("TD_TAIL_BM")) : 0;
    const int bm = forced == 64 || forced == 128 ? forced : 64;
    static const int fast_env32 = getenv("TD_TAIL_FAST") ? atoi(getenv("TD_TAIL_FAST")) : 1;
    const bool fast32 = fast_env32 && (size_t)a.M * a.COUT * es < 0xfffffff0ull - (1u << 20);
    if (precision == TD_PRECISION_FP32) {
        if (bm == 64) return fast32 ? launch_tail<float, 64, false, 1, true>(a, stream) : launch_tail<float, 64, false, 1>(a, stream);
        return launch_tail<float, 64, false, 2>(a, stream);
    }
    static const int fast_env = getenv("TD_TAIL_FAST") ? atoi(getenv("TD_TAIL_FAST")) : 1;
    const bool fast = fast_env && (size_t)a.M * a.COUT * es < 0xfffffff0ull - (1u << 20);
    if (a.MID == 64) {
        if (bm == 64) return fast ? launch_tail<_Float16, 64, false, 1, true>(a, stream) : launch_tail<_Float16, 64, false, 1>(a, stream);
        return launch_tail<_Float16, 64, true, 2>(a, stream);
    }
    if (bm == 64) return fast ? launch_tail<_Float16, 128, false, 1, true>(a, stream) : launch_tail<_Float16, 128, false, 1>(a, stream);
    return launch_tail<_Float16, 128, true, 2>(a, stream);
}
```

### treedetection_amd/csrc/common.h

```cpp
#pragma once
#include <hip/hip_runtime.h>
#include <hip/hip_fp16.h>
#include <cstdint>
#include <cstddef>
#include "../../include/treedet.h"
#include "conv_path.h"
#include <string>
#include <vector>

void td_set_error(const char* fmt, ...);

int td_polygons_json_text(const int32_t* mask_region, const int64_t* mask_offset, const uint32_t* mask_bits, int64_t mask_words,
                          const float* scores, const int32_t* classes, int n, const double* transform, const char* image_id,
                          std::string& out, const char* who);

#define TD_HIP_CHECK(expr)                                                                         \
    do {                                                                                           \
        hipError_t _e = (expr);                                                                    \
        if (_e != hipSuccess) {                                                                    \
            td_set_error("%s failed: %s (%s:%d)", #expr, hipGetErrorString(_e), __FILE__, __LINE__); \
            return TD_ERR_HIP;                                                                     \
        }                                                                                          \
    } while (0)

#define TD_REQUIRE(cond, ...)            \
    do {                                 \
        if (!(cond)) {                   \
            td_set_error(__VA_ARGS__);   \
            return TD_ERR_INVALID;       \
        }                                \
    } while (0)

#define TD_KERNEL_CHECK() TD_HIP_CHECK(hipGetLastError())

td_status td_decode_ticket(hipStream_t s, int** ticket, int* cus);

static inline int td_cdiv(int a, int b) { return (a + b - 1) / b; }

struct ConvArgs {
    const void* x;
    const void* w;
    const float* scale;
    const float* bias;
    const void* res;
    void* y;
    int B, H, W, Cin, Cout, KH, KW, stride, pad, Ho, Wo;
    int res_shift;
    int relu;
    int out_mode;
    int M;
    const int* m_dyn;
    int m_mul;
    int m_off;
    int out_f32;
    int batch_count;
    long long x_bs, w_bs, y_bs;
    const void* w_frag;
    const void* w_split;
    int tile_cfg;
    int tile_strict;
    const void* head_w;
    const float* head_b;
    float* head_y;
    int head_n;
    int nlev;
    struct Level {
        const void* x;
        const void* w;
        const float* bias;
        void* y;
        float* head_y;
        int H, W, M, tile0;
    } lev[5];
    int ntiles;
};
enum ConvFamily : unsigned char { TILE_IGEMM, TILE_PP8, TILE_PLANE, TILE_BD, TILE_BS, TILE_RETIRED, TILE_SPLIT };
enum : unsigned char { TILE_F32 = 1 << TD_PRECISION_FP32, TILE_F16 = 1 << TD_PRECISION_FP16, TILE_ANY = TILE_F32 | TILE_F16 };
struct ConvTile {
    ConvFamily family;
    unsigned char variant;
    unsigned char prec;
    bool head;
    bool frag;
    signed char tune_rank;
    unsigned char max_ksteps;
    short min_cout, max_cout;
};
inline constexpr ConvTile TD_CONV_TILES[] = {
    {TILE_IGEMM,   0, TILE_ANY, false, false,  5, 0,   0,  0},
    {TILE_IGEMM,   0, TILE_ANY, false, false, 10, 0,   0,  0},
    {TILE_IGEMM,   0, TILE_ANY, false, false, 11, 0,   0,  0},
    {TILE_IGEMM,   0, TILE_ANY, false, false, 16, 0,   0,  0},
    {TILE_IGEMM,   0, TILE_ANY, false, false, -1, 0,   0,  0},
    {TILE_IGEMM,   0, TILE_ANY, false, false, -1, 0,   0,  0},
    {TILE_IGEMM,   0, TILE_ANY, false, false, -1, 0,   0,  0},
    {TILE_IGEMM,   0, TILE_ANY, false, false, -1, 0,   0,  0},
    {TILE_IGEMM,   0, TILE_ANY, false, false, -1, 0,   0,  0},
    {TILE_IGEMM,   0, TILE_ANY, true,  false, -1, 0,   0,  0},
    {TILE_IGEMM,   0, TILE_ANY, true,  false,  1, 0,   0,  0},
    {TILE_IGEMM,   0, TILE_ANY, false, false, -1, 0,   0,  0},
    {TILE_IGEMM,   0, TILE_ANY, true,  false, -1, 0,   0,  0},
    {TILE_IGEMM,   0, TILE_ANY, true,  false, -1, 0,   0,  0},
    {TILE_IGEMM,   0, TILE_ANY, false, false, -1, 4,   0,  0},
    {TILE_IGEMM,   0, TILE_ANY, false, false,  6, 4,   0,  0},
    {TILE_IGEMM,   0, TILE_ANY, false, false,  4, 4,   0,  0},
    {TILE_PP8,     0, TILE_F16, true,  false,  2, 0, 128,  0},
    {TILE_PLANE,   0, TILE_F32, false, false, 18, 0,   0,  0},
    {TILE_PLANE,   0, TILE_F32, false, false, 19, 0,   0,  0},
    {TILE_PLANE,   0, TILE_F32, false, false, 20, 0,   0,  0},
    {TILE_RETIRED, 0, 0,        false, false, -1, 0,   0,  0},
    {TILE_RETIRED, 0, 0,        false, false, -1, 0,   0,  0},
    {TILE_BD,      0, TILE_ANY, true,  true,   8, 0,   0,  0},
    {TILE_BD,      1, TILE_ANY, false, true,  12, 0,   0,  0},
    {TILE_BD,      2, TILE_ANY, false, true,  13, 0,   0,  0},
    {TILE_BD,      3, TILE_ANY, false, true,  14, 0,   0,  0},
    {TILE_BD,      4, TILE_ANY, true,  true,   9, 0,   0,  0},
    {TILE_RETIRED, 0, 0,        false, false, -1, 0,   0,  0},
    {TILE_BD,      5, TILE_ANY, true,  true,   3, 0,   0,  0},
    {TILE_BD,      6, TILE_ANY, false, true,   7, 0,   0,  0},
    {TILE_IGEMM,   0, TILE_ANY, false, false, 15, 0,   0, 32},
    {TILE_IGEMM,   0, TILE_ANY, false, false, 17, 0,   0, 32},
    {TILE_BS,      0, TILE_ANY, false, true,   0, 4, 128,  0},
    {TILE_SPLIT,   0, TILE_F32, false, false, 21, 0,   0,  0},
    {TILE_SPLIT,   1, TILE_F32, false, false, 22, 0,   0,  0},
    {TILE_SPLIT,   2, TILE_F32, false, false, 23, 0,   0,  0},
    {TILE_SPLIT,   3, TILE_F32, false, false, 24, 0,   0,  0},
};
static inline const ConvTile* conv_tile(int id) { return id >= 0 && id < (int)(sizeof TD_CONV_TILES / sizeof *TD_CONV_TILES) ? &TD_CONV_TILES[id] : nullptr; }
static inline bool conv_head_capable(int id, int precision) { return precision == TD_PRECISION_FP16 && conv_tile(id) && conv_tile(id)->head; }
const char* conv_tile_refusal(int id, const ConvArgs& a, int precision);
td_status conv2d_launch(const ConvArgs& a, int precision, hipStream_t stream);
td_status conv_pp8_grouped_launch(ConvArgs a, hipStream_t stream);
void conv_bd_pack(const void* w_ohwi, int elem_bytes, int cout, int kh, int kw, int cin, std::vector<unsigned char>& out);
bool conv_bd_ok(const ConvArgs& a, int precision);
td_status conv_bd_launch(const ConvArgs& a, int precision, int variant, hipStream_t stream);
bool conv_bs_ok(const ConvArgs& a, int precision);
td_status conv_bs_launch(const ConvArgs& a, int precision, hipStream_t stream);
void conv_split_pack(const float* w, int cout, int cin, std::vector<unsigned char>& out);
bool conv_split_ok(const ConvArgs& a, int precision);
td_status conv_split_launch(const ConvArgs& a, int variant, hipStream_t stream);
td_status wino_gemm_launch(const ConvArgs& a, hipStream_t stream);

struct TailArgs {
    const void* x;
    const void* w2;
    const float* scale2;
    const float* bias2;
    const void* w3;
    const float* scale3;
    const float* bias3;
    const void* res;
    void* y;
    int B, H, W, MID, COUT, M;
};
bool bottleneck_tail_ok(int precision, int mid, int cout);
td_status bottleneck_tail_launch(const TailArgs& a, int precision, hipStream_t stream);

td_status wino_input_launch(const float* x, int B, int H, int W, int C, float* V, const int* m_dyn, int m_mul, long long t0, int Ts,
                            hipStream_t s);
td_status wino_output_launch(const float* Mb, int B, int H, int W, int N, const float* scale, const float* bias, int relu,
                             float* y, const int* m_dyn, int m_mul, long long t0, int Ts, hipStream_t s);
void wino_filter_transform(const float* w_ohwi, int N, int C, float* U);
td_status wino43_input_launch(const float* x, int B, int H, int W, int C, float* V, const int* m_dyn, hipStream_t s);
td_status wino43_fused_launch(const float* V, const float* U, int B, int H, int W, int C, int N, const float* scale, const float* bias,
                              int relu, float* y, const int* m_dyn, hipStream_t s);
td_status wino43_output_launch(const float* Mb, int B, int H, int W, int N, const float* scale, const float* bias, int relu,
                               float* y, const int* m_dyn, hipStream_t s);
td_status wino43_output_head_launch(const float* Mb, int B, int H, int W, int N, const float* scale, const float* bias, int relu,
                                    const float* head_w, const float* head_b, float* head_y, int head_n, hipStream_t s);
void wino43_filter_transform(const float* w_ohwi, int N, int C, float* U);
struct WinoRun {
    int form;
    bool fused_input;
    int slab_tiles;
    int fold_group;
    const float *x, *U, *scale, *bias;
    float* y;
    int B, H, W, cin, cout, relu;
    float *V, *M;
    const int* m_dyn;
    int m_mul;
    int gemm_cfg;
    const float *head_w, *head_b;
    float* head_y;
    int head_n;
};
ConvArgs wino_plane_args(const WinoRun& r, int n, long long t0);
ConvArgs wino43_plane_args(const WinoRun& r);
enum { WINO_STEP_INPUT, WINO_STEP_GEMM, WINO_STEP_OUTPUT };
struct WinoHook {
    void* ctx;
    void (*begin)(void* ctx, int step, long long n);
    void (*end)(void* ctx);
};
td_status wino_run(const WinoRun& r, hipStream_t s, const WinoHook* hook = nullptr);

struct ImgSizes {
    int h[64];
    int w[64];
};
#define TD_MAX_BATCH 64
td_status stem_launch(const void* images, int input_format, const ImgSizes& valid, int B, int Hp, int Wp,
                      const float* w_kc , const float* scale, const float* bias, void* y,
                      int cout, int precision, hipStream_t stream, const void* w16 = nullptr, const float* bias16 = nullptr);
void stem_mfma_prepare(const float* w_kc, const float* scale, const float* bias, int cout, std::vector<unsigned short>& w16_bits,
                       std::vector<float>& bias16);
td_status maxpool3x3s2_launch(const void* x, void* y, int B, int H, int W, int C, int precision, hipStream_t stream);
td_status subsample2_launch(const void* x, void* y, int B, int H, int W, int C, int precision, hipStream_t stream);
td_status resize_batch_u8_launch(const uint8_t* const* srcs, int n, int h, int w, int c, uint8_t* dst, int out_h,
                                 int out_w, int dst_pitch_px, size_t dst_img_bytes, void* tmp, hipStream_t stream);
td_status resize_bilinear_f64_launch(const double* src, int c, int h, int w, float* dst, int out_h, int out_w, int dst_pitch,
                                     long long dst_plane, hipStream_t stream);
td_status windows_u16_to_input_launch(const uint16_t* raster, int H, int W, int C, const int32_t* windows, int n, int* band1_max, float* dst,
                                      int out_h, int out_w, int dst_pitch, long long dst_plane, long long dst_image, hipStream_t stream);
td_status resize_tile_u8_launch(const uint8_t* src, int h, int w, int c, uint8_t* dst, int out_h, int out_w,
                                int dst_pitch_px, void* tmp, hipStream_t stream);
```

### treedetection_amd/csrc/conv_split.hip

```cpp
#include "common.h"
#include "conv_tiles.h"
#include <utility>

namespace {

typedef __bf16 bf16x8 __attribute__((ext_vector_type(8)));
typedef __bf16 bf16x2 __attribute__((ext_vector_type(2)));
typedef float f32x2 __attribute__((ext_vector_type(2)));
typedef unsigned u32x4 __attribute__((ext_vector_type(4)));

constexpr int SPLIT_CHUNK_BYTES = 6144;

template <int... R, class F>
__device__ __forceinline__ void static_for(std::integer_sequence<int, R...>, F&& f) {
    (f(std::integral_constant<int, R>{}), ...);
}

__device__ __forceinline__ void split8(const f32x4& lo, const f32x4& hi, bf16x8 (&p)[3]) {
    u32x4 w[3];
#pragma unroll
    for (int e = 0; e < 4; ++e) {
        f32x2 v = e < 2 ? f32x2{lo[2 * e], lo[2 * e + 1]} : f32x2{hi[2 * e - 4], hi[2 * e - 3]};
#pragma unroll
        for (int k = 0; k < 3; ++k) {
            const unsigned u = __builtin_bit_cast(unsigned, __builtin_convertvector(v, bf16x2));
            w[k][e] = u;
            if (k < 2) {
                const f32x2 back = {__builtin_bit_cast(float, u << 16), __builtin_bit_cast(float, u & 0xffff0000u)};
                v = v - back;
            }
        }
    }
#pragma unroll
    for (int k = 0; k < 3; ++k) p[k] = __builtin_bit_cast(bf16x8, w[k]);
}

template <int MT, int NT, int WM, int WN>
__device__ __forceinline__ void conv_split_body(const ConvArgs& a, char* lds) {
    constexpr int THREADS = 64 * WM * WN;
    constexpr int BM = 32 * MT * WM, BN = 32 * NT * WN;
    constexpr int LDROWS = THREADS / 8;
    constexpr int AROWS = BM / LDROWS;
    static_assert(BM % LDROWS == 0 && AROWS >= 1 && LDROWS % 16 == 0, "tile / thread-count mismatch");
    char* As = lds;

    int M = a.M;
    if (a.m_dyn) {
        int md = *a.m_dyn * a.m_mul - a.m_off;
        md = md < 0 ? 0 : md;
        M = md < M ? md : M;
    }
    const int tiles_n = (a.Cout + BN - 1) / BN;
    const int tiles_m = (M + BM - 1) / BM;
    const int nblk = tiles_m * tiles_n;
    if ((int)blockIdx.x >= nblk) return;
    const int pid = xcd_remap(blockIdx.x, nblk);
    const int tm = pid / tiles_n, tn = pid - tm * tiles_n;
    const int m0 = tm * BM, n0 = tn * BN;

    const int tid = threadIdx.x;
    const int lane = tid & 63, wave = tid >> 6;
    const int wm = wave / WN, wn = wave - wm * WN;
    const int ld_c = tid & 7, ld_r = tid >> 3;
    const int nit = a.Cin / 32;
    const unsigned pix_bytes = (unsigned)a.Cin * 4u;
    const __amdgpu_buffer_rsrc_t xrsrc = __builtin_amdgcn_make_buffer_rsrc(
        const_cast<void*>(a.x), 0, (int)((size_t)a.B * a.H * a.W * pix_bytes), 0x00020000);
    const int ntiles32 = (a.Cout + 31) / 32;
    const __amdgpu_buffer_rsrc_t wrsrc = __builtin_amdgcn_make_buffer_rsrc(
        const_cast<void*>(a.w_split), 0, (int)((size_t)ntiles32 * nit * SPLIT_CHUNK_BYTES), 0x00020000);
    constexpr unsigned OOB = 0xfffffff0u;
    const unsigned src_piece = (unsigned)(ld_c ^ ((ld_r >> 1) & 7)) * 16;

    unsigned a_off[AROWS];
#pragma unroll
    for (int i = 0; i < AROWS; ++i) {
        const int m = m0 + ld_r + LDROWS * i;
        a_off[i] = OOB;
        if (m < M && a.stride == 1) {
            a_off[i] = (unsigned)m * pix_bytes + src_piece;
        } else if (m < M) {
            const int hw = a.Ho * a.Wo;
            const int b = m / hw;
            const int rem = m - b * hw;
            const int oy = rem / a.Wo;
            const int ox = rem - oy * a.Wo;
            a_off[i] = (unsigned)((b * a.H + oy * a.stride) * a.W + ox * a.stride) * pix_bytes + src_piece;
        }
    }
    unsigned w_off[NT];
#pragma unroll
    for (int j = 0; j < NT; ++j) {
        const int nt = n0 / 32 + wn * NT + j;
        w_off[j] = nt < ntiles32 ? (unsigned)nt * (unsigned)nit * (unsigned)SPLIT_CHUNK_BYTES + (unsigned)lane * 16u : OOB;
    }

    unsigned w_dead[NT], a_dead[AROWS];
#pragma unroll
    for (int j = 0; j < NT; ++j) w_dead[j] = w_off[j] == OOB ? ~0u : 0u;
#pragma unroll
    for (int i = 0; i < AROWS; ++i) a_dead[i] = a_off[i] == OOB ? ~0u : 0u;

    typedef __attribute__((address_space(3))) void lds_void;
    const unsigned wave_rows = (unsigned)__builtin_amdgcn_readfirstlane(wave) * 8u;
    auto stage_a = [&](int stage, int it) {
#pragma unroll
        for (int i = 0; i < AROWS; ++i) {
            const unsigned off = a_off[i] == OOB || it >= nit ? OOB : a_off[i] + (unsigned)it * CHUNK_BYTES;
            char* dst = As + ((unsigned)stage * BM + (unsigned)LDROWS * i + wave_rows) * CHUNK_BYTES;
            __builtin_amdgcn_raw_ptr_buffer_load_lds(xrsrc, (lds_void*)dst, 16, off, 0, 0, 0);
        }
    };
    auto load_b = [&](f32x4 (&fb)[NT][3], int it, int sl) {
#pragma unroll
        for (int j = 0; j < NT; ++j)
#pragma unroll
            for (int q = 0; q < 3; ++q) {
                const unsigned off = w_off[j] == OOB || it >= nit ? OOB : w_off[j] + (unsigned)it * (unsigned)SPLIT_CHUNK_BYTES + (unsigned)(3 * sl + q) * 1024u;
                fb[j][q] = __builtin_bit_cast(f32x4, __builtin_amdgcn_raw_buffer_load_b128(wrsrc, off, 0, 0));
            }
    };

    f32x16 acc[MT][NT];
#pragma unroll
    for (int i = 0; i < MT; ++i)
#pragma unroll
        for (int j = 0; j < NT; ++j)
#pragma unroll
            for (int r = 0; r < 16; ++r) acc[i][j][r] = 0.f;
    const unsigned swz = (lane >> 1) & 7, hi = lane >> 5;
    unsigned frag_off[4];
#pragma unroll
    for (int kk = 0; kk < 4; ++kk)
        frag_off[kk] = (unsigned)(wm * 32 * MT + (lane & 31)) * CHUNK_BYTES + (((unsigned)(2 * kk) + hi) ^ swz) * 16;
    auto split_a = [&](int stage, int sl, bf16x8 (&pa)[MT][3]) {
        const char* Ab = &As[stage * BM * CHUNK_BYTES];
#pragma unroll
        for (int i = 0; i < MT; ++i) {
            const f32x4 lo = *reinterpret_cast<const f32x4*>(Ab + i * 32 * CHUNK_BYTES + frag_off[2 * sl]);
            const f32x4 up = *reinterpret_cast<const f32x4*>(Ab + i * 32 * CHUNK_BYTES + frag_off[2 * sl + 1]);
            split8(lo, up, pa[i]);
        }
    };
    auto mma_range = [&](const bf16x8 (&pa)[MT][3], const f32x4 (&fb)[NT][3], auto q0_c, auto q1_c) {
        constexpr int PA[6] = {0, 2, 1, 0, 1, 0}, QB[6] = {2, 0, 1, 1, 0, 0};
        constexpr int Q0 = decltype(q0_c)::value, Q1 = decltype(q1_c)::value;
#pragma unroll
        for (int q = Q0; q < Q1; ++q) {
            const int t = q / (MT * NT), i = (q / NT) % MT, j = q % NT;
            acc[i][j] = __builtin_amdgcn_mfma_f32_32x32x16_bf16(pa[i][PA[t]], __builtin_bit_cast(bf16x8, fb[j][QB[t]]), acc[i][j], 0, 0, 0);
        }
    };
    auto mma = [&](const bf16x8 (&pa)[MT][3], const f32x4 (&fb)[NT][3]) {
        mma_range(pa, fb, std::integral_constant<int, 0>{}, std::integral_constant<int, 6 * MT * NT>{});
    };

    constexpr bool PACED = MT == 4;
    constexpr int PACE_VALU = 4;
    constexpr int A_YOUNGER = 3 * NT * 3 + AROWS;
    static_assert(A_YOUNGER < 64, "vmcnt immediate");
    f32x4 fb[3][NT][3];
    bf16x8 pa[2][MT][3];
    stage_a(0, 0);
    stage_a(1, 1);
    stage_a(2, 2);
    load_b(fb[0], 0, 0);
    load_b(fb[1], 0, 1);
    asm volatile("s_waitcnt vmcnt(0)" ::: "memory");
    __builtin_amdgcn_s_barrier();
    split_a(0, 0, pa[0]);
    auto step = [&](auto c_c, auto s_c, int it) {
        constexpr int C = decltype(c_c)::value, S = decltype(s_c)::value, G = 2 * C + S;
        if constexpr (S == 1) {
            asm volatile("s_waitcnt vmcnt(%0)" ::"n"(A_YOUNGER) : "memory");
            asm volatile("s_waitcnt lgkmcnt(0)" ::: "memory");
            __builtin_amdgcn_s_barrier();
        }
        if constexpr (!PACED) {
            load_b(fb[(G + 2) % 3], it + 1, S);
            if constexpr (S == 1) stage_a(C, it + 3);
            __builtin_amdgcn_sched_barrier(0);
            if constexpr (S == 0) split_a(C, 1, pa[1]);
            else split_a((C + 1) % 3, 0, pa[0]);
            mma(pa[S], fb[G % 3]);
        } else {
            constexpr int REQS = 3 * NT + (S == 1 ? AROWS : 0), NMMA = 6 * MT * NT;
            static_assert(REQS < NMMA && PACE_VALU * (NMMA - REQS) >= 36 * MT, "the paced step has a gap for every request and for the split");
            const char* Ab = &As[(S == 0 ? C : (C + 1) % 3) * BM * CHUNK_BYTES];
            f32x4 raw[MT][2];
#pragma unroll
            for (int i = 0; i < MT; ++i)
#pragma unroll
                for (int h = 0; h < 2; ++h) raw[i][h] = *reinterpret_cast<const f32x4*>(Ab + i * 32 * CHUNK_BYTES + frag_off[2 * (1 - S) + h]);
            __builtin_amdgcn_sched_barrier(0);
            f32x4 (&fn)[NT][3] = fb[(G + 2) % 3];
            static_for(std::make_integer_sequence<int, REQS>{}, [&](auto r_c) {
                constexpr int R = decltype(r_c)::value;
                mma_range(pa[S], fb[G % 3], std::integral_constant<int, R>{}, std::integral_constant<int, R + 1>{});
                if constexpr (R < 3 * NT) {
                    constexpr int j = R / 3, q = R % 3;
                    const unsigned dead = w_dead[j] | (it + 1 >= nit ? ~0u : 0u);
                    const unsigned off = ((w_off[j] + (unsigned)(it + 1) * (unsigned)SPLIT_CHUNK_BYTES + (unsigned)(3 * S + q) * 1024u) & ~dead) | (OOB & dead);
                    fn[j][q] = __builtin_bit_cast(f32x4, __builtin_amdgcn_raw_buffer_load_b128(wrsrc, off, 0, 0));
                } else {
                    constexpr int i = R - 3 * NT;
                    const unsigned dead = a_dead[i] | (it + 3 >= nit ? ~0u : 0u);
                    const unsigned off = ((a_off[i] + (unsigned)(it + 3) * CHUNK_BYTES) & ~dead) | (OOB & dead);
                    char* dst = As + ((unsigned)C * BM + (unsigned)LDROWS * i + wave_rows) * CHUNK_BYTES;
                    __builtin_amdgcn_raw_ptr_buffer_load_lds(xrsrc, (lds_void*)dst, 16, off, 0, 0, 0);
                }
                __builtin_amdgcn_sched_barrier(0);
            });
            mma_range(pa[S], fb[G % 3], std::integral_constant<int, REQS>{}, std::integral_constant<int, NMMA>{});
#pragma unroll
            for (int i = 0; i < MT; ++i) {
                split8(raw[i][0], raw[i][1], pa[1 - S][i]);
#pragma unroll
                for (int k = 0; k < 3; ++k) {
                    u32x4 pin = __builtin_bit_cast(u32x4, pa[1 - S][i][k]);
                    asm volatile("" : "+v"(pin));
                    pa[1 - S][i][k] = __builtin_bit_cast(bf16x8, pin);
                }
            }
#pragma unroll
            for (int g = REQS; g < NMMA; ++g) {
                __builtin_amdgcn_sched_group_barrier(0x008, 1, 0);
                __builtin_amdgcn_sched_group_barrier(0x002, PACE_VALU, 0);
            }
            __builtin_amdgcn_sched_barrier(0);
        }
    };
    for (int it = 0; it < nit; it += 3) {
        step(std::integral_constant<int, 0>{}, std::integral_constant<int, 0>{}, it);
        step(std::integral_constant<int, 0>{}, std::integral_constant<int, 1>{}, it);
        if (it + 1 < nit) {
            step(std::integral_constant<int, 1>{}, std::integral_constant<int, 0>{}, it + 1);
            step(std::integral_constant<int, 1>{}, std::integral_constant<int, 1>{}, it + 1);
        }
        if (it + 2 < nit) {
            step(std::integral_constant<int, 2>{}, std::integral_constant<int, 0>{}, it + 2);
            step(std::integral_constant<int, 2>{}, std::integral_constant<int, 1>{}, it + 2);
        }
    }
    asm volatile("s_waitcnt vmcnt(0)" ::: "memory");
    asm volatile("s_waitcnt lgkmcnt(0)" ::: "memory");
    __builtin_amdgcn_s_barrier();
    conv_epilogue<float, float, MT, NT, WM, WN, 1>(a, acc, lds, M, m0, n0, tid, lane, wm, wn);
}

template <int MT, int NT, int WM, int WN, int WPE>
__global__ __launch_bounds__(64 * WM * WN, WPE)
void conv_split_kernel(const ConvArgs a) {
    constexpr int STAGE_BYTES = 3 * 32 * MT * WM * CHUNK_BYTES;
    constexpr int EPI_BYTES = conv_epilogue_lds_bytes<float, MT, NT, WM, WN, 1>();
    constexpr int LDS_BYTES = STAGE_BYTES > EPI_BYTES ? STAGE_BYTES : EPI_BYTES;
    constexpr int BLOCKS_PER_CU = 4 * WPE / (WM * WN) > 0 ? 4 * WPE / (WM * WN) : 1;
    static_assert(LDS_BYTES * BLOCKS_PER_CU <= 160 * 1024, "the blocks the registers allow on a CU must fit its LDS");
    __shared__ __attribute__((aligned(16))) char lds[LDS_BYTES];
    conv_split_body<MT, NT, WM, WN>(a, lds);
}

template <int MT, int NT, int WM, int WN, int WPE>
td_status launch_split(const ConvArgs& a, hipStream_t stream) {
    const int tiles = td_cdiv(a.M, 32 * MT * WM) * td_cdiv(a.Cout, 32 * NT * WN);
    hipLaunchKernelGGL((conv_split_kernel<MT, NT, WM, WN, WPE>), dim3(tiles), dim3(64 * WM * WN), 0, stream, a);
    TD_KERNEL_CHECK();
    return TD_OK;
}

inline unsigned short bf16_rne(float f) {
    unsigned u = __builtin_bit_cast(unsigned, f);
    if ((u & 0x7fffffffu) > 0x7f800000u) return (unsigned short)((u >> 16) | 0x40);
    u += 0x7fffu + ((u >> 16) & 1u);
    return (unsigned short)(u >> 16);
}

}

void conv_split_pack(const float* w, int cout, int cin, std::vector<unsigned char>& out) {
    const int nit = cin / 32, nt32 = (cout + 31) / 32;
    out.assign((size_t)nt32 * nit * SPLIT_CHUNK_BYTES, (unsigned char)0);
    unsigned short* o = reinterpret_cast<unsigned short*>(out.data());
    for (int t = 0; t < nt32; ++t)
        for (int c = 0; c < nit; ++c)
            for (int s = 0; s < 2; ++s)
                for (int l = 0; l < 64; ++l) {
                    const int n = t * 32 + (l & 31), h = l >> 5;
                    if (n >= cout) continue;
                    for (int e = 0; e < 8; ++e) {
                        float v = w[(size_t)n * cin + (size_t)c * 32 + 16 * s + 8 * (e >> 2) + 4 * h + (e & 3)];
                        for (int p = 0; p < 3; ++p) {
                            const unsigned short b = bf16_rne(v);
                            o[(((((size_t)t * nit + c) * 2 + s) * 3 + p) * 64 + l) * 8 + e] = b;
                            v = v - __builtin_bit_cast(float, (unsigned)b << 16);
                        }
                    }
                }
}

bool conv_split_ok(const ConvArgs& a, int precision) {
    return precision == TD_PRECISION_FP32 && a.w_split && a.KH == 1 && a.KW == 1 && a.pad == 0 && a.stride >= 1 && a.out_mode == 0 &&
           a.batch_count <= 1 && !a.out_f32 && !a.head_w && a.Cin >= 32 && a.Cin % 32 == 0 &&
           (size_t)((a.Cout + 31) / 32) * (size_t)(a.Cin / 32) * SPLIT_CHUNK_BYTES < 0xfffffff0ull - (1u << 20);
}

td_status conv_split_launch(const ConvArgs& a, int variant, hipStream_t stream) {
    TD_REQUIRE(conv_split_ok(a, TD_PRECISION_FP32), "split-bf16 contraction: unsupported launch (fp32 1x1 without padding, split filter bank)");
    switch (variant) {
        case 3: return launch_split<2, 2, 1, 2, 2>(a, stream);
        case 2: return launch_split<2, 4, 1, 2, 1>(a, stream);
        case 1: return launch_split<2, 2, 2, 2, 2>(a, stream);
        default: return launch_split<4, 2, 1, 4, 1>(a, stream);
    }
}
```

### treedetection_amd/csrc/conv_tiles.h

```cpp
#pragma once
#include "common.h"
#include <type_traits>

typedef float f32x16 __attribute__((ext_vector_type(16)));
typedef float f32x4 __attribute__((ext_vector_type(4)));
typedef _Float16 f16x8 __attribute__((ext_vector_type(8)));
typedef _Float16 f16x4 __attribute__((ext_vector_type(4)));

namespace {

constexpr int CHUNK_BYTES = 128;

__device__ __forceinline__ int xcd_remap(int bid, int nblk) {
    const int q = nblk >> 3, r = nblk & 7;
    const int xcd = bid & 7, local = bid >> 3;
    const int start = xcd < r ? xcd * (q + 1) : r * (q + 1) + (xcd - r) * q;
    return start + local;
}

template <typename T>
struct Elem;
template <>
struct Elem<float> {
    static constexpr int PER_CHUNK = 32;
    static __device__ __forceinline__ void mma(const f32x4& fa, const f32x4& fb, f32x16& acc) {
#pragma unroll
        for (int e = 0; e < 4; ++e) acc = __builtin_amdgcn_mfma_f32_32x32x2f32(fa[e], fb[e], acc, 0, 0, 0);
    }
    static __device__ __forceinline__ float to_f32(float v) { return v; }
};
template <>
struct Elem<_Float16> {
    static constexpr int PER_CHUNK = 64;
    static __device__ __forceinline__ void mma(const f32x4& fa, const f32x4& fb, f32x16& acc) {
#if defined(TD_DIAG_MFMA16B)
        f32x4 q[2];
#pragma unroll
        for (int k = 0; k < 2; ++k) {
            q[k] = f32x4{acc[4 * k], acc[4 * k + 1], acc[4 * k + 2], acc[4 * k + 3]};
            q[k] = __builtin_amdgcn_mfma_f32_16x16x32_f16(__builtin_bit_cast(f16x8, fa), __builtin_bit_cast(f16x8, fb), q[k], 0, 0, 0);
#pragma unroll
            for (int e = 0; e < 4; ++e) acc[4 * k + e] = q[k][e];
        }
#elif defined(TD_DIAG_MFMA16)
        f32x4 q[4];
#pragma unroll
        for (int k = 0; k < 4; ++k) {
            q[k] = f32x4{acc[4 * k], acc[4 * k + 1], acc[4 * k + 2], acc[4 * k + 3]};
            q[k] = __builtin_amdgcn_mfma_f32_16x16x32_f16(__builtin_bit_cast(f16x8, fa), __builtin_bit_cast(f16x8, fb), q[k], 0, 0, 0);
#pragma unroll
            for (int e = 0; e < 4; ++e) acc[4 * k + e] = q[k][e];
        }
#else
        acc = __builtin_amdgcn_mfma_f32_32x32x16_f16(__builtin_bit_cast(f16x8, fa), __builtin_bit_cast(f16x8, fb), acc, 0, 0, 0);
#endif
    }
    static __device__ __forceinline__ float to_f32(_Float16 v) { return (float)v; }
};

template <typename TO, int MT, int NT, int WM, int WN, int RWM, bool WIDE_OK = true>
constexpr int conv_epilogue_lds_bytes() {
    constexpr int BM = 32 * MT * WM, BN = 32 * NT * WN;
    constexpr int f32 = RWM * 32 * MT * (BN + 4) * 4;
    constexpr int f16 = sizeof(TO) == 2 && WIDE_OK ? BM * (BN + 8) * 2 : 0;
    return f32 > f16 ? f32 : f16;
}

template <typename T, typename TO, int MT, int NT, int WM, int WN, int RWM, bool WIDE_OK = true>
__device__ __forceinline__ void conv_epilogue(const ConvArgs& a, f32x16 (&acc)[MT][NT], char* lds, int M, int m0, int n0,
                                              int tid, int lane, int wm, int wn) {
    constexpr int THREADS = 64 * WM * WN;
    constexpr int BM = 32 * MT * WM, BN = 32 * NT * WN;
    constexpr int CS = BN + 4;
    constexpr int WROW = 32 * MT;
    TO* __restrict__ Y = static_cast<TO*>(a.y);
    const T* __restrict__ Rs = static_cast<const T*>(a.res);
    const int hw = a.Ho * a.Wo;

    constexpr bool WIDE = sizeof(TO) == 2 && THREADS >= 512 && WIDE_OK;
    constexpr bool E16 = sizeof(TO) == 2 && WIDE_OK;
    if constexpr (E16) {
        if (!Rs && a.out_mode == 0 && (a.Cout & 7) == 0) {
            constexpr int HS = BN + 8;
            _Float16* Hs = reinterpret_cast<_Float16*>(lds);
            const int odd = lane & 1;
#pragma unroll
            for (int j = 0; j < NT; ++j) {
                const int col = wn * 32 * NT + j * 32 + (lane & 31);
                const int nn = n0 + col;
                float sc = 1.f, bi = 0.f;
                if (nn < a.Cout) {
                    if (a.scale) sc = a.scale[nn];
                    if (a.bias) bi = a.bias[nn];
                }
#pragma unroll
                for (int i = 0; i < MT; ++i) {
#pragma unroll
                    for (int r = 0; r < 16; r += 2) {
                        float t0 = acc[i][j][r], t1 = acc[i][j][r + 1];
                        if (a.scale) { t0 = __fmul_rn(t0, sc); t1 = __fmul_rn(t1, sc); }
                        if (a.bias) { t0 = __fadd_rn(t0, bi); t1 = __fadd_rn(t1, bi); }
                        if (a.relu) { t0 = t0 > 0.f ? t0 : 0.f; t1 = t1 > 0.f ? t1 : 0.f; }
                        const float give = odd ? t0 : t1;
                        const float got = __builtin_bit_cast(float, __builtin_amdgcn_update_dpp(
                            0, __builtin_bit_cast(int, give), 0xB1 , 0xf, 0xf, false));
                        typedef _Float16 f16x2 __attribute__((ext_vector_type(2)));
                        f16x2 pk;
                        pk[0] = (_Float16)(odd ? got : t0);
                        pk[1] = (_Float16)(odd ? t1 : got);
                        const int row = wm * WROW + i * 32 + (r & 3) + 8 * (r >> 2) + 4 * (lane >> 5) + odd;
                        *reinterpret_cast<f16x2*>(&Hs[row * HS + (col & ~1)]) = pk;
                        __builtin_amdgcn_sched_barrier(0);
                    }
                }
            }
            __syncthreads();
            if constexpr (BN == 256 && sizeof(T) == 2) {
                if (a.head_w) {
                    constexpr int NWAVE = THREADS / 64, RT = BM / 32;
                    const int wv = tid >> 6;
                    const int col = lane & 31, kh8 = (lane >> 5) * 8;
                    const _Float16* __restrict__ Wh = static_cast<const _Float16*>(a.head_w);
                    const bool live = col < a.head_n;
                    const float hb = live && a.head_b ? a.head_b[col] : 0.f;
                    f32x4 fbh[16];
#pragma unroll
                    for (int kk = 0; kk < 16; ++kk) {
                        f32x4 z = {0.f, 0.f, 0.f, 0.f};
                        fbh[kk] = live ? *reinterpret_cast<const f32x4*>(Wh + (size_t)col * BN + kk * 16 + kh8) : z;
                    }
                    for (int rt = wv; rt < RT; rt += NWAVE) {
                        f32x16 hacc;
#pragma unroll
                        for (int r = 0; r < 16; ++r) hacc[r] = 0.f;
#pragma unroll
                        for (int kk = 0; kk < 16; ++kk) {
                            const f32x4 fah = *reinterpret_cast<const f32x4*>(&Hs[(rt * 32 + col) * HS + kk * 16 + kh8]);
                            Elem<T>::mma(fah, fbh[kk], hacc);
                        }
                        if (live) {
#pragma unroll
                            for (int r = 0; r < 16; ++r) {
                                const int m = m0 + rt * 32 + (r & 3) + 8 * (r >> 2) + 4 * (lane >> 5);
                                if (m < M) a.head_y[(size_t)m * a.head_n + col] = a.head_b ? __fadd_rn(hacc[r], hb) : hacc[r];
                            }
                        }
                    }
                    return;
                }
            }
            constexpr int PIECES = BN / 8;
            constexpr int ROWS_PER_PASS = THREADS / PIECES;
            static_assert(BM % ROWS_PER_PASS == 0, "fp16 epilogue rows must split evenly over the threads");
            const int pc = tid % PIECES, pr = tid / PIECES;
            const int n = n0 + pc * 8;
            if (n < a.Cout) {
#pragma unroll 4
                for (int it = 0; it < BM / ROWS_PER_PASS; ++it) {
                    const int row = pr + it * ROWS_PER_PASS;
                    const int m = m0 + row;
                    if (m >= M) break;
                    const f32x4 v = *reinterpret_cast<const f32x4*>(&Hs[row * HS + pc * 8]);
                    *reinterpret_cast<f32x4*>(Y + (size_t)m * a.Cout + n) = v;
                }
            }
            return;
        }
    }

    float* Cs = reinterpret_cast<float*>(lds);
    const int Cq = a.out_mode == 1 ? a.Cout >> 2 : a.Cout;
    constexpr int CPL = WIDE ? 8 : 4;
    constexpr int CHUNKS = BN / CPL;
    constexpr int ROWS_PER_PASS = THREADS / CHUNKS;
    const int c4 = tid % CHUNKS;
    const int n = n0 + c4 * CPL;
    const bool vec = (a.Cout % CPL) == 0 && n + CPL - 1 < a.Cout;
    float sc[CPL], bi[CPL];
#pragma unroll
    for (int e = 0; e < CPL; ++e) {
        sc[e] = 1.f;
        bi[e] = 0.f;
        if (n + e < a.Cout) {
            const int co = a.out_mode == 1 ? (n + e) % Cq : n + e;
            if (a.scale) sc[e] = a.scale[co];
            if (a.bias) bi[e] = a.bias[co];
        }
    }
    for (int q = 0; q < WM; q += RWM) {
        if (q > 0) __syncthreads();
        if (wm >= q && wm < q + RWM) {
#pragma unroll
            for (int i = 0; i < MT; ++i)
#pragma unroll
                for (int j = 0; j < NT; ++j)
#pragma unroll
                    for (int r = 0; r < 16; ++r) {
                        const int row = (wm - q) * WROW + i * 32 + (r & 3) + 8 * (r >> 2) + 4 * (lane >> 5);
                        const int col = wn * 32 * NT + j * 32 + (lane & 31);
                        Cs[row * CS + col] = acc[i][j][r];
                    }
        }
        __syncthreads();
        constexpr int ITERS = (RWM * WROW) / ROWS_PER_PASS;
        static_assert((RWM * WROW) % ROWS_PER_PASS == 0 && ITERS >= 1, "epilogue rows must split evenly over the threads");
        constexpr int UMAX = CPL == 8 ? 4 : 8;
        constexpr int U = ITERS < UMAX ? ITERS : UMAX;
        static_assert(ITERS % U == 0, "epilogue batch must divide the rows per thread");
        typedef _Float16 f16x8v __attribute__((ext_vector_type(8)));
        typedef typename std::conditional<sizeof(T) == 4, f32x4, typename std::conditional<CPL == 8, f16x8v, f16x4>::type>::type ResVec;
        auto res_offset = [&](int m) -> size_t {
// ... 90 lines not shown
```

### treedetection_amd/csrc/engine.cpp

```cpp
#include "common.h"
#include "detect.h"
#include "workspace.h"

#include <cmath>
#include <cstdio>
#include <cstdlib>
#include <cstring>
#include <algorithm>
#include <functional>
#include <map>
#include <optional>
#include <string>
#include <tuple>
#include <vector>

namespace {

struct HostTensor {
    const float* data = nullptr;
    std::vector<int64_t> shape;
    int64_t numel() const {
        int64_t n = 1;
        for (auto s : shape) n *= s;
        return n;
    }
};

enum { SPLIT_FC = 1, SPLIT_LATERAL = 2, SPLIT_CONV1 = 4, SPLIT_CONV3 = 8, SPLIT_SHORTCUT = 16,
       SPLIT_DEFAULT = SPLIT_FC | SPLIT_LATERAL | SPLIT_CONV1 | SPLIT_SHORTCUT };

struct ConvLayer {
    int cout = 0, cin = 0, kh = 1, kw = 1;
    void* w = nullptr;
    float* scale = nullptr;
    float* bias = nullptr;
    bool out_f32 = false;
    void* w_frag = nullptr;
    void* w_split = nullptr;
    float* wino_u = nullptr;
    float* wino_u43 = nullptr;
};

struct Block {
    ConvLayer c1, c2, c3, sc;
    bool has_sc = false;
    int stride = 1;
};

struct NamedTensor { void* p; WsDims dims; int elem; };

}

struct td_engine : Workspace {
    td_model_desc desc{};
    int device = 0;
    bool loaded = false;
    std::vector<void*> weight_allocs;
    std::vector<void*> ws_allocs;

    float* stem_w = nullptr;
    float* stem_scale = nullptr;
    float* stem_bias = nullptr;
    unsigned short* stem_w16 = nullptr;
    float* stem_bias16 = nullptr;
    int stem_c = 64;
    std::vector<Block> stages[4];
    ConvLayer lateral[4], fpn_out[4];
    ConvLayer rpn_conv, rpn_head;
    ConvLayer fc1, fc2, pred;
    ConvLayer mask_fcn[4], deconv;
    float* mask_pred_w = nullptr;
    float mask_pred_b = 0.f;
    int fpn_c = 256, fc_dim = 1024;

    int rB = 0, rHp = 0, rWp = 0;
    std::map<std::string, NamedTensor> named;

    int backbone_subbatch = 0;
    std::map<std::tuple<int, int, int, int, int>, int> tuned;
    bool winograd = true;
    size_t wino_elems = 0;
    bool group_levels = true;
    bool fuse_head = true;
    bool fuse_tail = true;
    bool fuse_tail_fp16 = false;
    bool wino_fused = true;
    int wino_slab = 0;
    int wino_minc = 128;
    int wino43_min = 12;
    int wino_fold = 39;
    int f32_split = SPLIT_DEFAULT;
    std::string tune_cache;
    void* tune_evict = nullptr;
    size_t tune_evict_bytes = 0;

    struct FwdCtx {
        const void* images = nullptr;
        int input_format = 0, B = 0, Hp = 0, Wp = 0;
        ImgSizes valid{}, outsz{};
        td_detections out{};
        bool valid_ctx = false;
    } ctx;
    hipEvent_t phase_ev[7] = {};
    bool phase_ev_recorded[7] = {};
    hipEvent_t prev5_ev = nullptr;
    bool prev5_recorded = false;
    bool stem_done = false;

    bool prof = false;
    bool prof_group_open = false;
    struct ProfRec { hipEvent_t a, b; int cat; };
    std::vector<ProfRec> prof_recs;
    std::vector<hipEvent_t> prof_free;
    double prof_ms[TD_PROF_CATEGORIES] = {};
    int64_t prof_launches[TD_PROF_CATEGORIES] = {};
    double prof_flops[TD_PROF_CATEGORIES] = {};
    double prof_bytes[TD_PROF_CATEGORIES] = {};
    bool prof_detail = false;
    double cls_ms[TD_PROF_CLASSES] = {};
    int64_t cls_launches[TD_PROF_CLASSES] = {};
    double cls_flops[TD_PROF_CLASSES] = {};
    double cls_bytes[TD_PROF_CLASSES] = {};
    double cls_tmin_ms[TD_PROF_CLASSES] = {};
    struct ClsRec { hipEvent_t a, b; int cls; };
    std::vector<ClsRec> cls_recs;
};

namespace {

td_status dev_alloc(std::vector<void*>& pool, void** p, size_t bytes) {
    if (bytes == 0) bytes = 16;
    TD_HIP_CHECK(hipMalloc(p, bytes));
    pool.push_back(*p);
    return TD_OK;
}

template <typename T>
td_status upload(td_engine* e, const std::vector<T>& h, T** d) {
    void* p = nullptr;
    td_status st = dev_alloc(e->weight_allocs, &p, h.size() * sizeof(T));
    if (st < 0) return st;
    TD_HIP_CHECK(hipMemcpy(p, h.data(), h.size() * sizeof(T), hipMemcpyHostToDevice));
    *d = static_cast<T*>(p);
    return TD_OK;
}

td_status upload_w(td_engine* e, const std::vector<float>& h, void** d) {
    if (e->desc.precision == TD_PRECISION_FP16) {
        std::vector<_Float16> hh(h.size());
        for (size_t i = 0; i < h.size(); ++i) hh[i] = (_Float16)h[i];
        _Float16* p = nullptr;
        td_status st = upload(e, hh, &p);
        *d = p;
        return st;
    }
    float* p = nullptr;
    td_status st = upload(e, h, &p);
    *d = p;
    return st;
}

td_status upload_frag(td_engine* e, const std::vector<float>& h, ConvLayer& L) {
    L.w_frag = nullptr;
    static const bool off = getenv("TD_BDIRECT") && atoi(getenv("TD_BDIRECT")) == 0;
    const bool f16 = e->desc.precision == TD_PRECISION_FP16;
    const int ke = f16 ? 64 : 32;
    if (off || L.cin % ke != 0 || L.kh * L.kw > 32 || (size_t)L.cout * L.kh * L.kw * L.cin != h.size()) return TD_OK;
    std::vector<unsigned char> packed;
    if (f16) {
        std::vector<unsigned short> bits(h.size());
        for (size_t i = 0; i < h.size(); ++i) bits[i] = __builtin_bit_cast(unsigned short, (_Float16)h[i]);
        conv_bd_pack(bits.data(), 2, L.cout, L.kh, L.kw, L.cin, packed);
    } else {
        conv_bd_pack(h.data(), 4, L.cout, L.kh, L.kw, L.cin, packed);
    }
    unsigned char* d = nullptr;
    td_status st = upload(e, packed, &d);
    L.w_frag = d;
    return st;
}

td_status upload_split(td_engine* e, const std::vector<float>& h, ConvLayer& L, int cls) {
    L.w_split = nullptr;
    if (e->desc.precision != TD_PRECISION_FP32 || !(e->f32_split & cls) || L.kh != 1 || L.kw != 1 || L.cin < 256 || L.cin % 32 != 0 ||
        (size_t)L.cout * L.cin != h.size())
        return TD_OK;
    std::vector<unsigned char> packed;
    conv_split_pack(h.data(), L.cout, L.cin, packed);
    unsigned char* d = nullptr;
    td_status st = upload(e, packed, &d);
    L.w_split = d;
    return st;
}

using TensorMap = std::map<std::string, HostTensor>;

td_status need(const TensorMap& tm, const std::string& name, int ndim, const HostTensor** out) {
    auto it = tm.find(name);
    if (it == tm.end()) {
        td_set_error("load_weights: tensor '%s' missing", name.c_str());
        return TD_ERR_WEIGHTS;
    }
    if ((int)it->second.shape.size() != ndim) {
        td_set_error("load_weights: tensor '%s' has %d dims, expected %d", name.c_str(), (int)it->second.shape.size(), ndim);
        return TD_ERR_WEIGHTS;
    }
    *out = &it->second;
    return TD_OK;
}

std::vector<float> pack_ohwi(const HostTensor& t) {
    const int co = (int)t.shape[0], ci = (int)t.shape[1], kh = (int)t.shape[2], kw = (int)t.shape[3];
    std::vector<float> out((size_t)co * ci * kh * kw);
    for (int o = 0; o < co; ++o)
        for (int c = 0; c < ci; ++c)
            for (int y = 0; y < kh; ++y)
                for (int x = 0; x < kw; ++x)
                    out[(((size_t)o * kh + y) * kw + x) * ci + c] = t.data[(((size_t)o * ci + c) * kh + y) * kw + x];
    return out;
}

td_status bn_fold(const TensorMap& tm, const std::string& p, int c, std::vector<float>& scale, std::vector<float>& bias) {
    const HostTensor *g, *b, *m, *v;
    td_status st;
    if ((st = need(tm, p + ".norm.weight", 1, &g)) < 0) return st;
    if ((st = need(tm, p + ".norm.bias", 1, &b)) < 0) return st;
    if ((st = need(tm, p + ".norm.running_mean", 1, &m)) < 0) return st;
    if ((st = need(tm, p + ".norm.running_var", 1, &v)) < 0) return st;
    if (g->shape[0] != c || b->shape[0] != c || m->shape[0] != c || v->shape[0] != c) {
        td_set_error("load_weights: norm tensors of '%s' do not have %d channels", p.c_str(), c);
        return TD_ERR_WEIGHTS;
    }
    scale.resize(c);
    bias.resize(c);
    for (int i = 0; i < c; ++i) {
        const float r = 1.0f / std::sqrt(v->data[i] + 1e-5f);
        const float s = g->data[i] * r;
        const float ms = m->data[i] * s;
        scale[i] = s;
        bias[i] = b->data[i] - ms;
    }
    return TD_OK;
}

td_status upload_wino(td_engine* e, const std::vector<float>& w_ohwi, ConvLayer& L) {
    L.wino_u = nullptr;
    if (e->desc.precision != TD_PRECISION_FP32 || !e->winograd || L.kh != 3 || L.kw != 3 || L.cin % 32 != 0 || L.cout % 4 != 0)
        return TD_OK;
    std::vector<float> u((size_t)16 * L.cout * L.cin);
    wino_filter_transform(w_ohwi.data(), L.cout, L.cin, u.data());
    td_status st = upload(e, u, &L.wino_u);
    if (st < 0 || e->wino43_min <= 0 || L.cin < e->wino_minc || L.cout < e->wino_minc) return st;
    std::vector<float> u43((size_t)36 * L.cout * L.cin);
    wino43_filter_transform(w_ohwi.data(), L.cout, L.cin, u43.data());
    return upload(e, u43, &L.wino_u43);
}

td_status load_conv_bn(td_engine* e, const TensorMap& tm, const std::string& p, ConvLayer& L, int split_cls = 0) {
    const HostTensor* w;
    td_status st = need(tm, p + ".weight", 4, &w);
    if (st < 0) return st;
    L.cout = (int)w->shape[0];
    L.cin = (int)w->shape[1];
    L.kh = (int)w->shape[2];
    L.kw = (int)w->shape[3];
    const std::vector<float> packed = pack_ohwi(*w);
    if ((st = upload_w(e, packed, &L.w)) < 0) return st;
    if ((st = upload_frag(e, packed, L)) < 0) return st;
    if ((st = upload_split(e, packed, L, split_cls)) < 0) return st;
    if ((st = upload_wino(e, packed, L)) < 0) return st;
    std::vector<float> s, b;
    if ((st = bn_fold(tm, p, L.cout, s, b)) < 0) return st;
    if ((st = upload(e, s, &L.scale)) < 0) return st;
    return upload(e, b, &L.bias);
}

td_status load_conv_bias(td_engine* e, const TensorMap& tm, const std::string& p, ConvLayer& L, int split_cls = 0) {
    const HostTensor *w, *b;
    td_status st = need(tm, p + ".weight", 4, &w);
    if (st < 0) return st;
    if ((st = need(tm, p + ".bias", 1, &b)) < 0) return st;
    L.cout = (int)w->shape[0];
    L.cin = (int)w->shape[1];
    L.kh = (int)w->shape[2];
    L.kw = (int)w->shape[3];
    if (b->shape[0] != L.cout) {
        td_set_error("load_weights: bias of '%s' has wrong length", p.c_str());
        return TD_ERR_WEIGHTS;
    }
    const std::vector<float> packed = pack_ohwi(*w);
    if ((st = upload_w(e, packed, &L.w)) < 0) return st;
    if ((st = upload_frag(e, packed, L)) < 0) return st;
    if ((st = upload_split(e, packed, L, split_cls)) < 0) return st;
    if ((st = upload_wino(e, packed, L)) < 0) return st;
    L.scale = nullptr;
    return upload(e, std::vector<float>(b->data, b->data + L.cout), &L.bias);
}

WsGeom engine_geom(const td_engine* e, int B, int Hp, int Wp) {
    int32_t c[WS_WIDTHS] = {e->stem_c};
    for (int s = 0; s < 4; ++s) { c[1 + s] = e->stages[s][0].c1.cout; c[5 + s] = e->stages[s][0].c2.cout; c[9 + s] = e->stages[s][0].c3.cout; }
    c[13] = e->fpn_c; c[14] = e->fc_dim; c[15] = e->deconv.cout / 4;
    return ws_geom(e->desc.precision, e->winograd, e->desc.post_nms_topk, e->desc.detections_per_image, c, B, Hp, Wp);
}

void publish(td_engine* e, const WsGeom& g, int phase) {
    for (const WsRow& r : ws_rows())
        for (int i = 0; r.pub && (r.phase == phase || (phase == 0 && r.phase == TD_PHASE_STEM)) && i < r.count; ++i) {
            char name[32];
            snprintf(name, sizeof name, r.pub, i + 2);
            e->named[name] = NamedTensor{*ws_slot(e, r, i), r.dims(g, i), (int)ws_elem_bytes(r, g)};
        }
}

hipEvent_t prof_event(td_engine* e) {
    hipEvent_t ev = nullptr;
    if (!e->prof_free.empty()) {
        ev = e->prof_free.back();
        e->prof_free.pop_back();
    } else {
        (void)hipEventCreate(&ev);
    }
    return ev;
}

struct ProfScope {
    td_engine* e;
    hipStream_t s;
    hipEvent_t a = nullptr;
    int cat;
    bool group;
    ProfScope(td_engine* e_, hipStream_t s_, int cat_, double flops = 0.0, double bytes = 0.0, bool group_ = false)
        : e(e_), s(s_), cat(cat_), group(group_) {
        if (!e->prof) return;
        if (!group) {
            e->prof_flops[cat] += flops;
            e->prof_bytes[cat] += bytes;
            e->prof_launches[cat] += 1;
        }
        if (e->prof_group_open) return;
        a = prof_event(e);
        (void)hipEventRecord(a, s);
        if (group) e->prof_group_open = true;
    }
    ~ProfScope() {
        if (!a) return;
        hipEvent_t b = prof_event(e);
        (void)hipEventRecord(b, s);
        e->prof_recs.push_back({a, b, cat});
        if (group) e->prof_group_open = false;
    }
};

struct ClassScope {
    td_engine* e;
    hipStream_t s;
    hipEvent_t a = nullptr;
    int cls;
    ClassScope(td_engine* e_, hipStream_t s_, int cls_, double exec_flops, double bytes) : e(e_), s(s_), cls(cls_) {
        if (!e->prof) return;
        const double peak = (e->desc.precision == TD_PRECISION_FP16 ? TD_PEAK_F16_MFMA_TFLOPS : TD_PEAK_F32_MFMA_TFLOPS) * 1e12;
        e->cls_launches[cls] += 1;
        e->cls_flops[cls] += exec_flops;
        e->cls_bytes[cls] += bytes;
        e->cls_tmin_ms[cls] += 1e3 * std::max(exec_flops / peak, bytes / (TD_HBM_ACHIEVABLE_TBS * 1e12));
        if (!e->prof_detail) return;
        a = prof_event(e);
        (void)hipEventRecord(a, s);
    }
    ~ClassScope() {
        if (!a) return;
        hipEvent_t b = prof_event(e);
        (void)hipEventRecord(b, s);
        e->cls_recs.push_back({a, b, cls});
    }
};

void load_tune_cache(td_engine* e) {
    if (e->tune_cache.empty()) return;
    if (FILE* f = fopen(e->tune_cache.c_str(), "r")) {
        int pr, a0, a1, a2, a3, a4, cfg;
        while (fscanf(f, "%d %d %d %d %d %d %d", &pr, &a0, &a1, &a2, &a3, &a4, &cfg) == 7) {
            if (pr == e->desc.precision && conv_tile(cfg)) e->tuned[std::make_tuple(a0, a1, a2, a3, a4)] = cfg;
        }
        fclose(f);
    }
}

void free_pool(std::vector<void*>& pool) {
    for (void* p : pool) (void)hipFree(p);
    pool.clear();
}

void read_rule_switches(td_engine* e) {
    if (const char* wg = getenv("TD_WINOGRAD")) e->winograd = atoi(wg) != 0;
    if (const char* ws = getenv("TD_WINO_SLAB")) e->wino_slab = atoi(ws);
    if (const char* wf = getenv("TD_WINO_FUSED")) e->wino_fused = atoi(wf) != 0;
    if (const char* fh = getenv("TD_FUSE_HEAD")) e->fuse_head = atoi(fh) != 0;
    if (const char* w4 = getenv("TD_WINO43_MIN")) e->wino43_min = atoi(w4);
    if (const char* wf2 = getenv("TD_WINO_FOLD")) e->wino_fold = atoi(wf2);
    if (const char* wc = getenv("TD_WINO_MINC")) e->wino_minc = atoi(wc);
}

ConvRules conv_rules(const td_engine* e) {
    return {e->desc.precision, e->winograd, e->wino_fused, e->wino_minc, e->wino43_min, e->wino_fold, e->wino_slab, e->fuse_head, e->wino_elems};
}

}

extern "C" {

td_status td_engine_create(const td_model_desc* desc, int device, td_engine** out) {
    TD_REQUIRE(out, "td_engine_create: out is NULL");
    td_model_desc d;
    if (desc) d = *desc; else td_model_desc_default(&d);
    TD_REQUIRE(d.num_classes == 1, "td_engine_create: num_classes=%d (the reference configures exactly 1, config.py:35)", d.num_classes);
    TD_REQUIRE(d.precision == TD_PRECISION_FP32 || d.precision == TD_PRECISION_FP16, "td_engine_create: bad precision %d", d.precision);
    TD_REQUIRE(d.pre_nms_topk >= 1 && d.pre_nms_topk <= RPN_CAND, "td_engine_create: pre_nms_topk must be in [1,%d]", RPN_CAND);
    TD_REQUIRE(d.post_nms_topk >= 1 && d.post_nms_topk <= 1024, "td_engine_create: post_nms_topk must be in [1,1024]");
    TD_REQUIRE(d.detections_per_image >= 1 && d.detections_per_image <= 1024, "td_engine_create: detections_per_image must be in [1,1024]");
    int ndev = 0;
    TD_HIP_CHECK(hipGetDeviceCount(&ndev));
    TD_REQUIRE(device >= 0 && device < ndev, "td_engine_create: device %d of %d", device, ndev);
    TD_HIP_CHECK(hipSetDevice(device));
    td_engine* e = new td_engine();
    if (const char* sbenv = getenv("TD_BACKBONE_SUBBATCH")) e->backbone_subbatch = atoi(sbenv);
    if (const char* tc = getenv("TD_TUNE_CACHE")) e->tune_cache = tc;
    if (const char* gl = getenv("TD_GROUP_LEVELS")) e->group_levels = atoi(gl) != 0;
    if (const char* ft = getenv("TD_FUSE_TAIL")) { e->fuse_tail = atoi(ft) != 0; e->fuse_tail_fp16 = atoi(ft) == 2; }
    if (const char* sp = getenv("TD_F32_SPLIT")) e->f32_split = atoi(sp);
    e->desc = d;
    read_rule_switches(e);
    load_tune_cache(e);
    e->device = device;
    *out = e;
    return TD_OK;
}

void td_engine_destroy(td_engine* e) {
    if (!e) return;
    (void)hipSetDevice(e->device);
    free_pool(e->weight_allocs);
    free_pool(e->ws_allocs);
    if (e->tune_evict) (void)hipFree(e->tune_evict);
    for (auto& r : e->prof_recs) { (void)hipEventDestroy(r.a); (void)hipEventDestroy(r.b); }
    for (auto& r : e->cls_recs) { (void)hipEventDestroy(r.a); (void)hipEventDestroy(r.b); }
    for (auto ev : e->prof_free) (void)hipEventDestroy(ev);
    for (auto ev : e->phase_ev) if (ev) (void)hipEventDestroy(ev);
    if (e->prev5_ev) (void)hipEventDestroy(e->prev5_ev);
    delete e;
}

td_status td_conv_path(const int32_t* rules, int64_t wino_elems, const int32_t* layer, const int32_t* call, const int32_t* head, int32_t* out) {
    TD_REQUIRE(rules && layer && call && out && wino_elems >= 0, "td_conv_path: bad argument");
    TD_REQUIRE(call[0] >= 1 && call[1] >= 1 && call[2] >= 1 && call[3] >= 1 && layer[2] >= 1 && layer[3] >= 1, "td_conv_path: bad geometry");
    td_engine fresh;
    fresh.desc.precision = rules[0];
    fresh.wino_elems = (size_t)wino_elems;
    read_rule_switches(&fresh);
    ConvRules r = conv_rules(&fresh);
    if (rules[1] >= 0) r.winograd = rules[1] != 0;
    if (rules[2] >= 0) r.wino_fused = rules[2] != 0;
    if (rules[3] >= 0) r.wino_minc = rules[3];
    if (rules[4] >= 0) r.wino43_min = rules[4];
    if (rules[5] >= 0) r.wino_fold = rules[5];
    if (rules[6] >= 0) r.wino_slab = rules[6];
    if (rules[7] >= 0) r.fuse_head = rules[7] != 0;
    auto facts = [](const int32_t* f) { return ConvLayerFacts{f[0], f[1], f[2], f[3], f[4] != 0, f[5] != 0, f[6] != 0, f[7] != 0, f[8] != 0}; };
    const ConvSite s{facts(layer), call[0], call[1], call[2], call[3], call[4], call[5] != 0, call[6] != 0, call[7], call[8] != 0, call[9],
                     head != nullptr, head ? facts(head) : ConvLayerFacts{}};
    const ConvPath p = conv_path(r, s);
    out[0] = p.form; out[1] = p.head; out[2] = p.tune ? 1 : 0;
    for (int i = 0; i < 5; ++i) out[3 + i] = p.tune ? p.key[i] : 0;
    out[8] = p.slab_tiles; out[9] = p.fold_group;
    return TD_OK;
}

td_status td_engine_load_weights(td_engine* e, const td_tensor_desc* tensors, size_t n) {
    TD_REQUIRE(e && tensors, "td_engine_load_weights: null argument");
    TD_HIP_CHECK(hipSetDevice(e->device));
    TensorMap tm;
    for (size_t i = 0; i < n; ++i) {
        TD_REQUIRE(tensors[i].name && tensors[i].data && tensors[i].ndim >= 1 && tensors[i].ndim <= 4,
                   "td_engine_load_weights: bad tensor descriptor %zu", i);
        HostTensor t;
        t.data = tensors[i].data;
        t.shape.assign(tensors[i].shape, tensors[i].shape + tensors[i].ndim);
        tm[tensors[i].name] = t;
    }
    free_pool(e->weight_allocs);
    e->loaded = false;
    td_status st;
    {
        const HostTensor* w;
        if ((st = need(tm, "backbone.bottom_up.stem.conv1.weight", 4, &w)) < 0) return st;
        if (w->shape[1] != 3 || w->shape[2] != 7 || w->shape[3] != 7) {
            td_set_error("load_weights: stem conv must be [C,3,7,7] (RGB+nDSM tiles still feed 3 channels, prediction.py:166)");
            return TD_ERR_WEIGHTS;
        }
        e->stem_c = (int)w->shape[0];
        std::vector<float> p((size_t)147 * e->stem_c);
        for (int co = 0; co < e->stem_c; ++co)
            for (int c = 0; c < 3; ++c)
                for (int ky = 0; ky < 7; ++ky)
                    for (int kx = 0; kx < 7; ++kx)
                        p[(size_t)((ky * 7 + kx) * 3 + c) * e->stem_c + co] = w->data[(((size_t)co * 3 + c) * 7 + ky) * 7 + kx];
        if ((st = upload(e, p, &e->stem_w)) < 0) return st;
        std::vector<float> s, b;
        if ((st = bn_fold(tm, "backbone.bottom_up.stem.conv1", e->stem_c, s, b)) < 0) return st;
        if ((st = upload(e, s, &e->stem_scale)) < 0) return st;
        if ((st = upload(e, b, &e->stem_bias)) < 0) return st;
        const char* mfma_stem = getenv("TD_STEM_MFMA");
        if (e->desc.precision == TD_PRECISION_FP16 && e->stem_c == 64 && !(mfma_stem && atoi(mfma_stem) == 0)) {
            std::vector<unsigned short> w16;
            std::vector<float> b16;
            stem_mfma_prepare(p.data(), s.data(), b.data(), e->stem_c, w16, b16);
            if ((st = upload(e, w16, &e->stem_w16)) < 0) return st;
            if ((st = upload(e, b16, &e->stem_bias16)) < 0) return st;
        }
    }
    for (int si = 0; si < 4; ++si) {
        e->stages[si].clear();
        for (int bi = 0;; ++bi) {
            const std::string p = "backbone.bottom_up.res" + std::to_string(si + 2) + "." + std::to_string(bi);
            if (tm.find(p + ".conv1.weight") == tm.end()) break;
            Block blk;
            blk.stride = (bi == 0 && si > 0) ? 2 : 1;
            if ((st = load_conv_bn(e, tm, p + ".conv1", blk.c1, si > 0 ? SPLIT_CONV1 : 0)) < 0) return st;
            if ((st = load_conv_bn(e, tm, p + ".conv2", blk.c2)) < 0) return st;
            if ((st = load_conv_bn(e, tm, p + ".conv3", blk.c3, si > 0 ? SPLIT_CONV3 : 0)) < 0) return st;
            blk.has_sc = tm.find(p + ".shortcut.weight") != tm.end();
            if (blk.has_sc && (st = load_conv_bn(e, tm, p + ".shortcut", blk.sc, si > 0 ? SPLIT_SHORTCUT : 0)) < 0) return st;
            e->stages[si].push_back(blk);
        }
        if (e->stages[si].empty()) {
            td_set_error("load_weights: no blocks found for res%d", si + 2);
            return TD_ERR_WEIGHTS;
        }
    }
    for (int l = 0; l < 4; ++l) {
        if ((st = load_conv_bias(e, tm, "backbone.fpn_lateral" + std::to_string(l + 2), e->lateral[l], SPLIT_LATERAL)) < 0) return st;
        if ((st = load_conv_bias(e, tm, "backbone.fpn_output" + std::to_string(l + 2), e->fpn_out[l])) < 0) return st;
    }
    e->fpn_c = e->lateral[0].cout;
    if ((st = load_conv_bias(e, tm, "proposal_generator.rpn_head.conv", e->rpn_conv)) < 0) return st;
    {
        const HostTensor *wo, *bo, *wd, *bd;
        if ((st = need(tm, "proposal_generator.rpn_head.objectness_logits.weight", 4, &wo)) < 0) return st;
        if ((st = need(tm, "proposal_generator.rpn_head.objectness_logits.bias", 1, &bo)) < 0) return st;
        if ((st = need(tm, "proposal_generator.rpn_head.anchor_deltas.weight", 4, &wd)) < 0) return st;
        if ((st = need(tm, "proposal_generator.rpn_head.anchor_deltas.bias", 1, &bd)) < 0) return st;
        if (wo->shape[0] != RPN_A || wd->shape[0] != 4 * RPN_A || wo->shape[1] != e->fpn_c || wd->shape[1] != e->fpn_c) {
            td_set_error("load_weights: RPN head must have %d anchors per position", RPN_A);
            return TD_ERR_WEIGHTS;
        }
        const int c = e->fpn_c;
        std::vector<float> w((size_t)RPN_HEAD_C * c), b(RPN_HEAD_C);
        std::memcpy(w.data(), wo->data, sizeof(float) * RPN_A * c);
        std::memcpy(w.data() + (size_t)RPN_A * c, wd->data, sizeof(float) * 4 * RPN_A * c);
        std::memcpy(b.data(), bo->data, sizeof(float) * RPN_A);
        std::memcpy(b.data() + RPN_A, bd->data, sizeof(float) * 4 * RPN_A);
        e->rpn_head.cout = RPN_HEAD_C; e->rpn_head.cin = c; e->rpn_head.kh = e->rpn_head.kw = 1;
        e->rpn_head.out_f32 = true;
        if ((st = upload_w(e, w, &e->rpn_head.w)) < 0) return st;
        if ((st = upload_frag(e, w, e->rpn_head)) < 0) return st;
        if ((st = upload(e, b, &e->rpn_head.bias)) < 0) return st;
    }
    {
        const HostTensor *w, *b;
        if ((st = need(tm, "roi_heads.box_head.fc1.weight", 2, &w)) < 0) return st;
        if ((st = need(tm, "roi_heads.box_head.fc1.bias", 1, &b)) < 0) return st;
        const int c = e->fpn_c, o = (int)w->shape[0];
        if (w->shape[1] != (int64_t)c * 49) {
            td_set_error("load_weights: fc1 expects %d inputs", c * 49);
            return TD_ERR_WEIGHTS;
        }
        std::vector<float> p((size_t)o * c * 49);
        for (int r = 0; r < o; ++r)
            for (int ch = 0; ch < c; ++ch)
                for (int q = 0; q < 49; ++q) p[(size_t)r * c * 49 + (size_t)q * c + ch] = w->data[(size_t)r * c * 49 + (size_t)ch * 49 + q];
        e->fc1.cout = o; e->fc1.cin = c * 49; e->fc1.kh = e->fc1.kw = 1;
        e->fc_dim = o;
        if ((st = upload_w(e, p, &e->fc1.w)) < 0) return st;
        if ((st = upload_frag(e, p, e->fc1)) < 0) return st;
        if ((st = upload_split(e, p, e->fc1, SPLIT_FC)) < 0) return st;
        if ((st = upload(e, std::vector<float>(b->data, b->data + o), &e->fc1.bias)) < 0) return st;
    }
    {
        const HostTensor *w, *b;
        if ((st = need(tm, "roi_heads.box_head.fc2.weight", 2, &w)) < 0) return st;
        if ((st = need(tm, "roi_heads.box_head.fc2.bias", 1, &b)) < 0) return st;
        e->fc2.cout = (int)w->shape[0]; e->fc2.cin = (int)w->shape[1]; e->fc2.kh = e->fc2.kw = 1;
        const std::vector<float> w2v(w->data, w->data + w->numel());
        if ((st = upload_w(e, w2v, &e->fc2.w)) < 0) return st;
        if ((st = upload_frag(e, w2v, e->fc2)) < 0) return st;
        if ((st = upload_split(e, w2v, e->fc2, SPLIT_FC)) < 0) return st;
        if ((st = upload(e, std::vector<float>(b->data, b->data + e->fc2.cout), &e->fc2.bias)) < 0) return st;
    }
    {
        const HostTensor *wc, *bc, *wr, *br;
        if ((st = need(tm, "roi_heads.box_predictor.cls_score.weight", 2, &wc)) < 0) return st;
        if ((st = need(tm, "roi_heads.box_predictor.cls_score.bias", 1, &bc)) < 0) return st;
        if ((st = need(tm, "roi_heads.box_predictor.bbox_pred.weight", 2, &wr)) < 0) return st;
        if ((st = need(tm, "roi_heads.box_predictor.bbox_pred.bias", 1, &br)) < 0) return st;
        if (wc->shape[0] != 2 || wr->shape[0] != 4) {
            td_set_error("load_weights: box predictor must be 1 class (+background), got cls %lld / reg %lld rows",
                         (long long)wc->shape[0], (long long)wr->shape[0]);
            return TD_ERR_WEIGHTS;
        }
        const int k = (int)wc->shape[1];
        std::vector<float> w((size_t)6 * k), b(6);
        std::memcpy(w.data(), wc->data, sizeof(float) * 2 * k);
        std::memcpy(w.data() + (size_t)2 * k, wr->data, sizeof(float) * 4 * k);
        std::memcpy(b.data(), bc->data, sizeof(float) * 2);
        std::memcpy(b.data() + 2, br->data, sizeof(float) * 4);
        e->pred.cout = 6; e->pred.cin = k; e->pred.kh = e->pred.kw = 1;
        e->pred.out_f32 = true;
        if ((st = upload_w(e, w, &e->pred.w)) < 0) return st;
        if ((st = upload_frag(e, w, e->pred)) < 0) return st;
        if ((st = upload(e, b, &e->pred.bias)) < 0) return st;
    }
    for (int i = 0; i < 4; ++i)
        if ((st = load_conv_bias(e, tm, "roi_heads.mask_head.mask_fcn" + std::to_string(i + 1), e->mask_fcn[i])) < 0) return st;
    {
        const HostTensor *w, *b;
        if ((st = need(tm, "roi_heads.mask_head.deconv.weight", 4, &w)) < 0) return st;
        if ((st = need(tm, "roi_heads.mask_head.deconv.bias", 1, &b)) < 0) return st;
        const int ci = (int)w->shape[0], co = (int)w->shape[1];
        if (w->shape[2] != 2 || w->shape[3] != 2) {
            td_set_error("load_weights: mask deconv must be 2x2");
            return TD_ERR_WEIGHTS;
        }
        std::vector<float> p((size_t)4 * co * ci);
        for (int i = 0; i < ci; ++i)
            for (int o = 0; o < co; ++o)
                for (int q = 0; q < 4; ++q) p[((size_t)q * co + o) * ci + i] = w->data[((size_t)i * co + o) * 4 + q];
        e->deconv.cout = 4 * co; e->deconv.cin = ci; e->deconv.kh = e->deconv.kw = 1;
        if ((st = upload_w(e, p, &e->deconv.w)) < 0) return st;
        if ((st = upload(e, std::vector<float>(b->data, b->data + co), &e->deconv.bias)) < 0) return st;
    }
    {
        const HostTensor *w, *b;
        if ((st = need(tm, "roi_heads.mask_head.predictor.weight", 4, &w)) < 0) return st;
        if ((st = need(tm, "roi_heads.mask_head.predictor.bias", 1, &b)) < 0) return st;
        if (w->shape[0] != 1) {
            td_set_error("load_weights: mask predictor must have 1 output channel");
            return TD_ERR_WEIGHTS;
        }
        if ((st = upload(e, std::vector<float>(w->data, w->data + w->shape[1]), &e->mask_pred_w)) < 0) return st;
        e->mask_pred_b = b->data[0];
    }
    e->loaded = true;
    return TD_OK;
}

td_status td_engine_reserve(td_engine* e, int B, int Hp, int Wp) {
    TD_REQUIRE(e, "td_engine_reserve: null engine");
    TD_REQUIRE(e->loaded, "td_engine_reserve: load weights first");
    TD_REQUIRE(B >= 1 && B <= TD_MAX_BATCH, "td_engine_reserve: batch %d not in [1,%d]", B, TD_MAX_BATCH);
    TD_REQUIRE(Hp >= 64 && Wp >= 64 && Hp % 32 == 0 && Wp % 32 == 0, "td_engine_reserve: padded size %dx%d must be multiples of 32 (>= 64)", Hp, Wp);
    if (B <= e->rB && Hp <= e->rHp && Wp <= e->rWp) return TD_OK;
    B = B > e->rB ? B : e->rB;
    Hp = Hp > e->rHp ? Hp : e->rHp;
    Wp = Wp > e->rWp ? Wp : e->rWp;
    TD_HIP_CHECK(hipSetDevice(e->device));
    free_pool(e->ws_allocs);
    e->named.clear();
    e->rB = e->rHp = e->rWp = 0;
    const WsGeom g = engine_geom(e, B, Hp, Wp);
    e->wino_v = e->wino_m = nullptr;
    for (size_t k = 0; k < ws_row_count(g); ++k)
        for (int i = 0; i < ws_rows()[k].count; ++i)
            if (td_status st = dev_alloc(e->ws_allocs, ws_slot(e, ws_rows()[k], i), ws_alloc_bytes(ws_rows()[k], g, i)); st < 0) return st;
    e->wino_elems = ws_wino_elems(g);
    e->rB = B;
    e->rHp = Hp;
    e->rWp = Wp;
    return TD_OK;
}

}

namespace {
// ... 78 lines not shown
    *cfg_out = best_cfg;
    return TD_OK;
}

struct WinoBooks {
    td_engine* e;
    hipStream_t s;
    const WinoRun& r;
    std::optional<ClassScope> cs;
    static void begin(void* ctx, int step, long long n) {
        WinoBooks& k = *static_cast<WinoBooks*>(ctx);
        const WinoRun& r = k.r;
        if (r.m_dyn) {
            k.cs.emplace(k.e, k.s, TD_CLS_MASK_HEAD, 0.0, 0.0);
            return;
        }
        const bool f22 = r.form == CONV_WINO22;
        const double P = f22 ? 16.0 : 36.0;
        const double T = f22 ? (double)n : (double)r.B * ((r.H + 3) / 4) * ((r.W + 3) / 4);
        const double share = f22 ? 1.0 : (double)n / r.B;
        const double px = (double)r.B * r.H * r.W;
        const double xb = 4.0 * px * r.cin, yb = 4.0 * px * r.cout, ub = 4.0 * P * r.cout * r.cin;
        const double vb = 4.0 * P * T * r.cin, mb = 4.0 * P * T * r.cout, pf = 2.0 * P * T * (double)r.cin * r.cout;
        if (step == WINO_STEP_INPUT) {
            k.cs.emplace(k.e, k.s, TD_CLS_WINO_XFORM, 0.0, (xb + vb) * share);
        } else if (step == WINO_STEP_GEMM) {
            k.cs.emplace(k.e, k.s, TD_CLS_WINO_GEMM, pf * share,
                         r.form == CONV_WINO43_FOLD ? (vb + yb) * share + ub : (f22 && r.fused_input ? xb : vb) + ub + mb);
        } else if (r.head_w) {
            k.cs.emplace(k.e, k.s, TD_CLS_WINO_XFORM, 2.0 * px * r.head_n * r.cout, mb + (4.0 * px * r.head_n + 4.0 * r.head_n * r.cout));
        } else {
            k.cs.emplace(k.e, k.s, TD_CLS_WINO_XFORM, 0.0, mb + yb);
        }
    }
    static void end(void* ctx) { static_cast<WinoBooks*>(ctx)->cs.reset(); }
};

td_status run_wino(td_engine* e, const WinoRun& r, hipStream_t s) {
    if (!e->prof) return wino_run(r, s);
    WinoBooks books{e, s, r, std::nullopt};
    const WinoHook hook{&books, WinoBooks::begin, WinoBooks::end};
    return wino_run(r, s, &hook);
}

ConvLayerFacts layer_facts(const ConvLayer& L) {
    return {L.cout, L.cin, L.kh, L.kw, L.scale != nullptr, L.out_f32, L.wino_u != nullptr, L.wino_u43 != nullptr, L.w_split != nullptr};
}

td_status run_conv(td_engine* e, const ConvLayer& L, const void* x_, int B_, int H_, int W_, int stride, int pad, bool relu, void* y_,
                   const void* res_, int res_shift, hipStream_t s_, const int* m_dyn = nullptr, int m_mul = 1, int out_mode = 0,
                   const ConvLayer* head = nullptr, float* head_y = nullptr, bool* head_fused = nullptr) {
    const int prec_ = e->desc.precision;
    const ConvSite site{layer_facts(L), B_, H_, W_, stride, pad, relu, res_ != nullptr, out_mode, m_dyn != nullptr, m_mul,
                        head != nullptr, head ? layer_facts(*head) : ConvLayerFacts{}};
    const ConvPath path = conv_path(conv_rules(e), site);
    const bool split = path.form == CONV_SPLIT, use_wino = path.form >= CONV_WINO22, use_43 = path.form >= CONV_WINO43;
    const int Ho = (H_ + 2 * pad - L.kh) / stride + 1, Wo = (W_ + 2 * pad - L.kw) / stride + 1;
    const double M = (double)B_ * Ho * Wo, K = (double)L.kh * L.kw * L.cin;
    const double flops = 2.0 * M * L.cout * K;
    const double es = prec_ == TD_PRECISION_FP16 ? 2.0 : 4.0;
    const double bytes = es * ((double)B_ * H_ * W_ * L.cin / (stride * stride) + M * L.cout * (res_ ? 2.0 : 1.0)) + (split ? 6.0 : es) * L.cout * K;
    td_status st2;
    ConvArgs ca{};
    ca.x = x_; ca.w = L.w; ca.w_frag = L.w_frag; ca.w_split = split ? L.w_split : nullptr; ca.scale = L.scale; ca.bias = L.bias; ca.res = res_; ca.y = y_;
    ca.B = B_; ca.H = H_; ca.W = W_; ca.Cin = L.cin; ca.Cout = L.cout; ca.KH = L.kh; ca.KW = L.kw;
    ca.stride = stride; ca.pad = pad; ca.Ho = Ho; ca.Wo = Wo;
    ca.res_shift = res_shift; ca.relu = relu ? 1 : 0; ca.out_mode = out_mode;
    ca.M = B_ * Ho * Wo; ca.m_dyn = m_dyn; ca.m_mul = m_mul; ca.tile_cfg = -1; ca.out_f32 = L.out_f32 ? 1 : 0;
    WinoRun wr{};
    if (use_wino) {
        wr.form = path.form; wr.fused_input = e->wino_fused; wr.slab_tiles = path.slab_tiles; wr.fold_group = path.fold_group;
        wr.x = static_cast<const float*>(x_); wr.U = use_43 ? L.wino_u43 : L.wino_u; wr.scale = L.scale; wr.bias = L.bias; wr.y = static_cast<float*>(y_);
        wr.B = B_; wr.H = H_; wr.W = W_; wr.cin = L.cin; wr.cout = L.cout; wr.relu = relu ? 1 : 0;
        wr.V = e->wino_v; wr.M = e->wino_m; wr.m_dyn = m_dyn; wr.m_mul = m_mul; wr.gemm_cfg = -1;
    }
    if (path.tune) {
        const auto key = std::make_tuple(path.key[0], path.key[1], path.key[2], path.key[3], path.key[4]);
        if (use_wino) {
            auto wino = [&](int c) { WinoRun q = wr; q.gemm_cfg = c; return run_wino(e, q, s_); };
            st2 = tuned_cfg(e, key, prec_, use_43 ? wino43_plane_args(wr) : wino_plane_args(wr, path.key[3], 0), s_, wino, &wr.gemm_cfg);
        } else {
            auto direct = [&](int c) { ConvArgs a = ca; a.tile_cfg = c; return conv2d_launch(a, prec_, s_); };
            st2 = tuned_cfg(e, key, prec_, ca, s_, direct, &ca.tile_cfg);
        }
        if (st2 < 0) return st2;
    }
    const bool fuse_head = path.head == HEAD_IN_TRANSFORM || (path.head == HEAD_IF_TILE_OWNS_256 && conv_head_capable(ca.tile_cfg, prec_));
    if (head_fused) *head_fused = fuse_head;
    const double hflops = fuse_head ? 2.0 * M * head->cout * L.cout : 0.0, hbytes = fuse_head ? 4.0 * M * head->cout + es * head->cout * L.cout : 0.0;
    ProfScope ps(e, s_, m_dyn ? 7 : 0, m_dyn ? 0.0 : flops, m_dyn ? 0.0 : bytes);
    if (e->prof && !m_dyn) {
        const double padded = use_43 ? (double)(((H_ + 3) / 4) * 4) * (((W_ + 3) / 4) * 4) / ((double)H_ * W_) : 1.0;
        e->prof_flops[8] += use_43 ? flops * padded * 0.25 : (use_wino ? flops * 4.0 / 9.0 : (split ? flops * 6.0 / 16.0 : flops));
        e->prof_launches[8] += use_wino ? 1 : 0;
    }
    if (e->prof && fuse_head) {
        e->prof_flops[0] += hflops;
        e->prof_flops[8] += hflops;
        e->prof_launches[0] += 1;
        e->prof_bytes[0] += hbytes + es * M * L.cout;
    }
    if (use_wino) {
        if (fuse_head) { wr.head_w = static_cast<const float*>(head->w); wr.head_b = head->bias; wr.head_y = head_y; wr.head_n = head->cout; }
        return run_wino(e, wr, s_);
    }
    const int cls = m_dyn ? TD_CLS_MASK_HEAD : (H_ == 1 && W_ == 1 ? TD_CLS_FC : (L.kh == 1 && L.kw == 1 ? TD_CLS_CONV1X1 : TD_CLS_CONV3X3));
    if (fuse_head) {
        ca.head_w = head->w; ca.head_b = head->bias; ca.head_y = head_y; ca.head_n = head->cout;
        ClassScope cs(e, s_, cls, flops + hflops, bytes - es * M * L.cout + hbytes);
        return conv2d_launch(ca, prec_, s_);
    }
    ClassScope cs(e, s_, cls, m_dyn ? 0.0 : (split ? flops * 6.0 / 16.0 : flops), m_dyn ? 0.0 : bytes);
    return conv2d_launch(ca, prec_, s_);
}

td_status forward_impl(td_engine* e, unsigned phase_mask, hipStream_t s) {
    const td_engine::FwdCtx& c = e->ctx;
    const void* images = c.images;
    const int input_format = c.input_format, B = c.B, Hp = c.Hp, Wp = c.Wp;
    const ImgSizes& valid = c.valid;
    const ImgSizes& outsz = c.outsz;
    const td_detections* out = &c.out;
    const int prec = e->desc.precision;
    auto PH = [&](int k) { return (phase_mask >> k) & 1u; };
    if (PH(0)) e->named.clear();
    td_status st;
    auto groupable = [&](const ConvLayer& L) {
        return L.kh == 3 && L.kw == 3 && L.cout == 256 && L.cin % 64 == 0 && !L.scale && L.bias && !L.out_f32;
    };
    auto run_grouped = [&](const ConvLayer* const* Ls, const void* const* xs, void* const* ys, float* const* head_ys, int nl, const int* Hs,
                           const int* Ws, bool relu, const ConvLayer* head, hipStream_t s_) -> td_status {
        ConvArgs a{};
        a.B = B; a.Cin = Ls[0]->cin; a.Cout = 256; a.KH = a.KW = 3; a.stride = 1; a.pad = 1; a.relu = relu ? 1 : 0; a.m_mul = 1; a.nlev = nl;
        a.tile_cfg = 17;
        double flops = 0.0, bytes = 0.0, unfused_bytes = 0.0;
        for (int l = 0; l < nl; ++l) {
            a.lev[l].x = xs[l]; a.lev[l].w = Ls[l]->w; a.lev[l].bias = Ls[l]->bias;
            a.lev[l].y = ys ? ys[l] : nullptr; a.lev[l].head_y = head_ys ? head_ys[l] : nullptr;
            a.lev[l].H = Hs[l]; a.lev[l].W = Ws[l];
            const double M = (double)B * Hs[l] * Ws[l], K = 9.0 * a.Cin;
            flops += 2.0 * M * 256 * K + (head ? 2.0 * M * head->cout * 256 : 0.0);
            bytes += 2.0 * (M * a.Cin + (head ? 0.0 : M * 256) + 256 * K) + (head ? 4.0 * M * head->cout + 2.0 * head->cout * 256 : 0.0);
            unfused_bytes += head ? 2.0 * 2.0 * M * 256 : 0.0;
        }
        if (head) { a.head_w = head->w; a.head_b = head->bias; a.head_n = head->cout; }
        ProfScope ps(e, s_, 0, flops, bytes + unfused_bytes);
        if (e->prof) {
            e->prof_flops[8] += flops;
            e->prof_launches[0] += nl * (head ? 2 : 1) - 1;
        }
        ClassScope cs(e, s_, TD_CLS_CONV3X3, flops, bytes);
        return conv_pp8_grouped_launch(a, s_);
    };
    auto run_tail = [&](const Block& blk, const void* t1_, int B_, int H_, int W_, void* y_, const void* shortcut_, hipStream_t s_) -> td_status {
        TailArgs a{};
        a.x = t1_; a.w2 = blk.c2.w; a.scale2 = blk.c2.scale; a.bias2 = blk.c2.bias;
        a.w3 = blk.c3.w; a.scale3 = blk.c3.scale; a.bias3 = blk.c3.bias; a.res = shortcut_; a.y = y_;
        a.B = B_; a.H = H_; a.W = W_; a.MID = blk.c2.cout; a.COUT = blk.c3.cout; a.M = B_ * H_ * W_;
        const double M = (double)a.M, mid = a.MID, co = a.COUT, es = prec == TD_PRECISION_FP16 ? 2.0 : 4.0;
        const double flops = 2.0 * M * mid * (9.0 * mid) + 2.0 * M * co * mid;
        const double bytes = es * (M * mid + 2.0 * M * co + 9.0 * mid * mid + co * mid);
        ProfScope ps(e, s_, 0, flops, bytes);
        if (e->prof) {
            e->prof_flops[8] += flops;
            e->prof_launches[0] += 1;
            e->prof_bytes[0] += es * 2.0 * M * mid;
        }
        ClassScope cs(e, s_, TD_CLS_TAIL, flops, bytes);
        return bottleneck_tail_launch(a, prec, s_);
    };
    const WsGeom g = engine_geom(e, B, Hp, Wp);
    const int *hs = g.h, *wsz = g.w;
    auto off = [&](void* p, size_t elems) -> void* { return static_cast<char*>(p) + elems * g.es; };
    int sb = e->backbone_subbatch > 0 ? e->backbone_subbatch : B;
    if (sb > B) sb = B;
    const bool do_stem = PH(6) || (PH(0) && !e->stem_done);
    std::optional<ProfScope> trunk_group;
    for (int b0 = 0; (PH(0) || PH(6)) && b0 < B; b0 += sb) {
        const int nb_img = (B - b0) < sb ? (B - b0) : sb;
        ImgSizes vsub{};
        for (int i = 0; i < nb_img; ++i) {
            vsub.h[i] = valid.h[b0 + i];
            vsub.w[i] = valid.w[b0 + i];
        }
        const size_t in_img = input_format == TD_INPUT_U8_HWC ? (size_t)Hp * Wp * 3 : (size_t)Hp * Wp * 3 * 4;
        const void* img_sub = static_cast<const char*>(images) + (size_t)b0 * in_img;
        void* stem_sub = off(e->stem_out, (size_t)b0 * (Hp / 2) * (Wp / 2) * e->stem_c);
        void* pool_sub = off(e->pool_out, (size_t)b0 * hs[0] * wsz[0] * e->stem_c);
        if (do_stem) {
            { ProfScope ps(e, s, 1);
            if ((st = stem_launch(img_sub, input_format, vsub, nb_img, Hp, Wp, e->stem_w, e->stem_scale, e->stem_bias, stem_sub,
                                  e->stem_c, prec, s, e->stem_w16, e->stem_bias16)) < 0) return st; }
            { ProfScope ps(e, s, 2);
            if ((st = maxpool3x3s2_launch(stem_sub, pool_sub, nb_img, Hp / 2, Wp / 2, e->stem_c, prec, s)) < 0) return st; }
        }
        if (!PH(0)) continue;
        if (!trunk_group && sb >= B) trunk_group.emplace(e, s, 0, 0.0, 0.0, true);
        const void* x = pool_sub;
        int xh = hs[0], xw = wsz[0];
        ProfScope backbone_group(e, s, 0, 0.0, 0.0, true);
        for (int si = 0; si < 4; ++si) {
            const int nb = (int)e->stages[si].size();
            const int oh = hs[si], ow = wsz[si];
            const size_t px = (size_t)b0 * oh * ow;
            const int mid = e->stages[si][0].c1.cout, co = e->stages[si][0].c3.cout;
            void* t1 = off(e->t1[si], px * mid);
            void* t2 = off(e->t2[si], px * mid);
            void* scb = off(e->scb[si], px * co);
            void* resb = off(e->res[si], px * co);
            void* xtmp = off(e->xtmp[si], px * co);
            for (int bi = 0; bi < nb; ++bi) {
                const Block& blk = e->stages[si][bi];
                void* y = ((nb - 1 - bi) % 2 == 0) ? resb : xtmp;
                const void* shortcut = x;
                if (blk.has_sc) {
                    if ((st = run_conv(e, blk.sc, x, nb_img, xh, xw, blk.stride, 0, false, scb, nullptr, 0, s)) < 0) return st;
                    shortcut = scb;
                }
                if ((st = run_conv(e, blk.c1, x, nb_img, xh, xw, blk.stride, 0, true, t1, nullptr, 0, s)) < 0) return st;
                if (e->fuse_tail && (blk.c2.cout == 64 || e->fuse_tail_fp16) && blk.c2.kh == 3 && blk.c2.kw == 3 &&
                    blk.c2.cin == blk.c2.cout && blk.c3.cin == blk.c2.cout && bottleneck_tail_ok(prec, blk.c2.cout, blk.c3.cout)) {
                    if ((st = run_tail(blk, t1, nb_img, oh, ow, y, shortcut, s)) < 0) return st;
                } else {
                    if ((st = run_conv(e, blk.c2, t1, nb_img, oh, ow, 1, 1, true, t2, nullptr, 0, s)) < 0) return st;
                    if ((st = run_conv(e, blk.c3, t2, nb_img, oh, ow, 1, 0, true, y, shortcut, 0, s)) < 0) return st;
                }
                x = y;
                xh = oh;
                xw = ow;
            }
        }
    }
    if (PH(0)) {
    {
    ProfScope fpn_group(e, s, 0, 0.0, 0.0, true);
    const bool group_fpn = prec == TD_PRECISION_FP16 && e->group_levels && groupable(e->fpn_out[0]) && groupable(e->fpn_out[1]) &&
                           groupable(e->fpn_out[2]) && groupable(e->fpn_out[3]);
    for (int l = 3; l >= 0; --l) {
        const void* td_res = l == 3 ? nullptr : e->inner[l + 1];
        if ((st = run_conv(e, e->lateral[l], e->res[l], B, hs[l], wsz[l], 1, 0, false, e->inner[l], td_res, td_res ? 1 : 0, s)) < 0) return st;
        if (!group_fpn && (st = run_conv(e, e->fpn_out[l], e->inner[l], B, hs[l], wsz[l], 1, 1, false, e->pfeat[l], nullptr, 0, s)) < 0) return st;
    }
    if (group_fpn) {
        const ConvLayer* Ls[4] = {&e->fpn_out[0], &e->fpn_out[1], &e->fpn_out[2], &e->fpn_out[3]};
        const void* xs[4] = {e->inner[0], e->inner[1], e->inner[2], e->inner[3]};
        void* ys[4] = {e->pfeat[0], e->pfeat[1], e->pfeat[2], e->pfeat[3]};
        if ((st = run_grouped(Ls, xs, ys, nullptr, 4, hs, wsz, false, nullptr, s)) < 0) return st;
    }
    }
    { ProfScope ps(e, s, 2);
    if ((st = subsample2_launch(e->pfeat[3], e->pfeat[4], B, hs[3], wsz[3], e->fpn_c, prec, s)) < 0) return st; }
    {
        ProfScope rpn_group(e, s, 0, 0.0, 0.0, true);
        const bool group_rpn = prec == TD_PRECISION_FP16 && e->group_levels && e->fuse_head && groupable(e->rpn_conv) && e->rpn_head.cin == 256 &&
                               e->rpn_head.kh == 1 && e->rpn_head.kw == 1 && e->rpn_head.cout <= 32 && e->rpn_head.out_f32 && !e->rpn_head.scale;
        if (group_rpn) {
            const ConvLayer* Ls[5] = {&e->rpn_conv, &e->rpn_conv, &e->rpn_conv, &e->rpn_conv, &e->rpn_conv};
            const void* xs[5] = {e->pfeat[0], e->pfeat[1], e->pfeat[2], e->pfeat[3], e->pfeat[4]};
            float* hy[5] = {e->rpn_headbuf[0], e->rpn_headbuf[1], e->rpn_headbuf[2], e->rpn_headbuf[3], e->rpn_headbuf[4]};
            if ((st = run_grouped(Ls, xs, nullptr, hy, 5, hs, wsz, true, &e->rpn_head, s)) < 0) return st;
        }
        for (int l = 0; l < 5 && !group_rpn; ++l) {
            bool fused = false;
            if ((st = run_conv(e, e->rpn_conv, e->pfeat[l], B, hs[l], wsz[l], 1, 1, true, e->rpn_t, nullptr, 0, s, nullptr, 1, 0,
                               &e->rpn_head, e->rpn_headbuf[l], &fused)) < 0) return st;
            if (!fused && (st = run_conv(e, e->rpn_head, e->rpn_t, B, hs[l], wsz[l], 1, 0, false, e->rpn_headbuf[l], nullptr, 0, s)) < 0) return st;
        }
    }
    trunk_group.reset();
    }
    RpnLevels lv{};
    {
        static const int sizes[5] = {32, 64, 128, 256, 512};
        static const double ratios[3] = {0.5, 1.0, 2.0};
        int off = 0;
        for (int l = 0; l < 5; ++l) {
            lv.head[l] = e->rpn_headbuf[l];
            lv.h[l] = hs[l];
            lv.w[l] = wsz[l];
            lv.stride[l] = 4 << l;
            lv.anchor_off[l] = off;
            off += hs[l] * wsz[l] * RPN_A;
            const double area = (double)sizes[l] * sizes[l];
            for (int a = 0; a < 3; ++a) {
                const double w = std::sqrt(area / ratios[a]);
                const double h = ratios[a] * w;
                lv.base[l][a][0] = (float)(-w / 2.0);
                lv.base[l][a][1] = (float)(-h / 2.0);
                lv.base[l][a][2] = (float)(w / 2.0);
                lv.base[l][a][3] = (float)(h / 2.0);
            }
        }
        lv.total_anchors = off;
    }
    const int P = g.P, D = g.D, mrows = g.mrows;
    FeatLevels fl{};
    for (int l = 0; l < 4; ++l) {
        fl.feat[l] = e->pfeat[l];
        fl.h[l] = hs[l];
        fl.w[l] = wsz[l];
        fl.scale[l] = 1.0f / (float)(4 << l);
    }
    fl.C = e->fpn_c;
    float* o_boxes = out->boxes ? out->boxes : e->o_boxes;
    float* o_scores = out->scores ? out->scores : e->o_scores;
    int* o_classes = out->classes ? out->classes : e->o_classes;
    int* o_count = out->count ? out->count : e->o_count;
    float* o_probs = out->mask_probs ? out->mask_probs : e->o_mask_probs;
    if (PH(1)) {
    { ProfScope ps(e, s, 3);
    if ((st = rpn_topk_decode_launch(lv, valid, B, e->desc.pre_nms_topk, e->key_ws, e->cand_boxes, e->cand_scores,
                                     e->cand_valid, e->cand_idx, s)) < 0) return st; }
    { ProfScope ps(e, s, 3);
    if ((st = nms_launch(e->cand_boxes, nullptr, e->cand_valid, B * RPN_LEVELS, RPN_CAND, e->desc.rpn_nms_thresh,
                         e->nms_mask, e->rpn_keep, e->rpn_keep_count, RPN_CAND, s)) < 0) return st; }
    { ProfScope ps(e, s, 3);
    if ((st = rpn_merge_launch(e->cand_boxes, e->cand_scores, e->rpn_keep, e->rpn_keep_count, B, P, e->props,
                               e->prop_scores, e->prop_count, P, s)) < 0) return st; }
    { ProfScope ps(e, s, 4);
    if ((st = roi_align_launch(fl, e->props, e->prop_count, B, P, 7, 0, e->pooled7, nullptr, prec, s)) < 0) return st; }
    }
    if (PH(2)) {
    {
    ProfScope box_group(e, s, 0, 0.0, 0.0, true);
    if ((st = run_conv(e, e->fc1, e->pooled7, B * P, 1, 1, 1, 0, true, e->fc1_out, nullptr, 0, s)) < 0) return st;
    if ((st = run_conv(e, e->fc2, e->fc1_out, B * P, 1, 1, 1, 0, true, e->fc2_out, nullptr, 0, s)) < 0) return st;
    if ((st = run_conv(e, e->pred, e->fc2_out, B * P, 1, 1, 1, 0, false, e->pred_out, nullptr, 0, s)) < 0) return st;
    }
    }
    if (PH(3)) {
    { ProfScope ps(e, s, 5);
    if ((st = det_decode_launch(e->pred_out, 6, e->props, e->prop_count, valid, B, P, e->desc.score_thresh, e->dboxes,
                                e->dscores, e->dflags, s)) < 0) return st; }
    { ProfScope ps(e, s, 5);
    if ((st = sort_boxes_launch(e->dboxes, e->dscores, e->dflags, e->prop_count, B, P, e->sboxes, e->sscores, e->sidx,
                                e->scount, s)) < 0) return st; }
    { ProfScope ps(e, s, 5);
    if ((st = nms_launch(e->sboxes, e->scount, nullptr, B, P, e->desc.nms_thresh, e->nms_mask, e->det_keep,
                         e->det_keep_count, D, s)) < 0) return st; }
    { ProfScope ps(e, s, 5);
    if ((st = det_finalize_launch(e->sboxes, e->sscores, e->det_keep, e->det_keep_count, valid, outsz, B, P, D,
                                  e->det_boxes_net, o_boxes, o_scores, o_classes, o_count, s)) < 0) return st; }
    { ProfScope ps(e, s, 4);
    if ((st = roi_align_launch(fl, e->det_boxes_net, o_count, B, D, 14, 1, e->pooled14, e->total_rows, prec, s)) < 0) return st; }
    }
    if (PH(4)) {
    const void* mx = e->pooled14;
    void* mbuf[2] = {e->mbuf0, e->mbuf1};
    {
    ProfScope mask_group(e, s, 7, 0.0, 0.0, true);
    for (int i = 0; i < 4; ++i) {
        if ((st = run_conv(e, e->mask_fcn[i], mx, mrows, 14, 14, 1, 1, true, mbuf[i & 1], nullptr, 0, s, e->total_rows, 196)) < 0) return st;
        mx = mbuf[i & 1];
    }
    if ((st = run_conv(e, e->deconv, mx, mrows, 14, 14, 1, 0, true, e->deconv_out, nullptr, 0, s, e->total_rows, 196, 1)) < 0) return st;
    }
    }
    if (PH(5)) {
    { ProfScope ps(e, s, 6);
    if ((st = mask_predict_launch(e->deconv_out, e->mask_pred_w, e->mask_pred_b, e->deconv.cout / 4, mrows * 784,
                                  e->total_rows, 784, e->mask_logits, e->mask_probs_compact, prec, s)) < 0) return st; }
    { ProfScope ps(e, s, 6);
    if ((st = mask_scatter_launch(e->mask_probs_compact, o_count, B, D, o_probs, s)) < 0) return st; }
    if (out->mask_bits) {
        { ProfScope ps(e, s, 6);
        if ((st = paste_masks_launch(o_probs, o_boxes, o_count, outsz, B, D, e->desc.mask_thresh, out->mask_region,
                                     reinterpret_cast<long long*>(out->mask_offset), out->mask_bits,
                                     out->mask_words_per_image, s)) < 0) return st; }
    }
    }
    for (int k = 0; k <= TD_PHASE_STEM; ++k) if (PH(k)) publish(e, g, k);
    return TD_OK;
}

td_status set_forward_ctx(td_engine* e, const void* images, int input_format, const int32_t* hw_valid,
// ... 179 lines not shown
```

Baseline: 730.1.

## Run fused bottleneck tail 3x3 conv via split-bf16 MFMA with prepacked weights

Adds a split-bf16 (three-term bf16 decomposition) path for the fp32 3x3 conv inside the fused bottleneck tail kernel of stage 0. Weights are packed per tap at load time, and the kernel runs 32x32x16 bf16 MFMAs with a double-buffered tap pipeline, with the two K-halves reduced through LDS. This targets the slow fp32 3x3 math in the tail and replaces it with matrix-core work. In exchange it needs extra MFMA passes per product, accepts small numerical differences from the split approximation, and adds a mid-only output mode and a standalone API entry.

```diff
diff --git a/include/treedet.h b/include/treedet.h
--- a/include/treedet.h
+++ b/include/treedet.h
@@ -101,6 +101,10 @@
 td_status td_bottleneck_tail_nhwc(const void* x, const void* w2, const float* scale2, const float* bias2, const void* w3,
                                   const float* scale3, const float* bias3, const void* shortcut, void* y, int B, int H, int W,
                                   int mid, int cout, int precision, void* stream);
+td_status td_bottleneck_tail_split_nhwc(const void* x, const void* w2, const float* scale2, const float* bias2, const void* w3,
+                                        const float* scale3, const float* bias3, const void* shortcut, void* y, void* mid_out,
+                                        int B, int H, int W, int mid, int cout, void* stream);
+int64_t td_conv_split_pack(const float* w, int cout, int cin, int taps, uint8_t* out, int64_t out_bytes);
 td_status td_conv2d_nhwc(const void* x, const void* w, const float* scale, const float* bias,
                          const void* residual, int res_shift, void* y, int B, int H, int W, int Cin,
                          int Cout, int KH, int KW, int stride, int pad, int relu, int precision,
diff --git a/treedetection_amd/_lib.py b/treedetection_amd/_lib.py
--- a/treedetection_amd/_lib.py
+++ b/treedetection_amd/_lib.py
@@ -80,6 +80,8 @@
     "td_resize_batch_u8": (C.c_int, [C.POINTER(C.c_void_p), C.c_int, C.c_int, C.c_int, C.c_int, C.c_void_p, C.c_int, C.c_int,
                                      C.c_int, C.c_int64, C.c_void_p, C.c_void_p]),
     "td_bottleneck_tail_nhwc": (C.c_int, [C.c_void_p] * 9 + [C.c_int] * 6 + [C.c_void_p]),
+    "td_bottleneck_tail_split_nhwc": (C.c_int, [C.c_void_p] * 10 + [C.c_int] * 5 + [C.c_void_p]),
+    "td_conv_split_pack": (C.c_int64, [C.c_void_p, C.c_int, C.c_int, C.c_int, C.c_void_p, C.c_int64]),
     "td_resize_bilinear_f64": (C.c_int, [C.c_void_p, C.c_int, C.c_int, C.c_int, C.c_void_p, C.c_int, C.c_int, C.c_int, C.c_int64, C.c_void_p]),
     "td_windows_u16_to_input": (C.c_int, [C.c_void_p, C.c_int, C.c_int, C.c_int, C.c_void_p, C.c_int, C.c_void_p, C.c_void_p, C.c_int, C.c_int,
                                           C.c_int, C.c_int64, C.c_int64, C.c_void_p]),
diff --git a/treedetection_amd/csrc/api.cpp b/treedetection_amd/csrc/api.cpp
--- a/treedetection_amd/csrc/api.cpp
+++ b/treedetection_amd/csrc/api.cpp
@@ -4,6 +4,7 @@
 #include <cstdio>
 #include <cmath>
 #include <cstdlib>
+#include <cstring>
 #include <vector>
 
 
@@ -214,6 +215,44 @@
     return bottleneck_tail_launch(a, precision, static_cast<hipStream_t>(stream));
 }
 
+td_status td_bottleneck_tail_split_nhwc(const void* x, const void* w2, const float* scale2, const float* bias2, const void* w3,
+                                        const float* scale3, const float* bias3, const void* shortcut, void* y, void* mid_out,
+                                        int B, int H, int W, int mid, int cout, void* stream) {
+    TD_REQUIRE(x && w2 && B > 0 && H > 0 && W > 0, "td_bottleneck_tail_split_nhwc: null argument or empty tensor");
+    TD_REQUIRE(mid_out || (w3 && shortcut && y), "td_bottleneck_tail_split_nhwc: the fused launch needs w3, shortcut and y");
+    TD_REQUIRE(bottleneck_tail_split_ok(TD_PRECISION_FP32, mid, cout, (long long)B * H * W), "td_bottleneck_tail_split_nhwc: mid 64, cout 256, output below 4 GB");
+    hipStream_t s = static_cast<hipStream_t>(stream);
+    const size_t n = (size_t)mid * 9 * mid;
+    std::vector<float> wh(n);
+    std::vector<unsigned char> packed;
+    TD_HIP_CHECK(hipStreamSynchronize(s));
+    TD_HIP_CHECK(hipMemcpy(wh.data(), w2, n * sizeof(float), hipMemcpyDeviceToHost));
+    conv_split_pack(wh.data(), mid, mid, packed, 9);
+    void* ws = nullptr;
+    td_status st = scratch(&ws, packed.size());
+    if (st < 0) return st;
+    hipError_t herr = hipMemcpy(ws, packed.data(), packed.size(), hipMemcpyHostToDevice);
+    TailArgs a{};
+    a.x = x; a.w2 = w2; a.w2_split = ws; a.scale2 = scale2; a.bias2 = bias2; a.B = B; a.H = H; a.W = W; a.MID = mid; a.COUT = cout; a.M = B * H * W;
+    if (mid_out) a.mid_out = static_cast<float*>(mid_out);
+    else { a.w3 = w3; a.scale3 = scale3; a.bias3 = bias3; a.res = shortcut; a.y = y; }
+    if (herr == hipSuccess) st = bottleneck_tail_launch(a, TD_PRECISION_FP32, s);
+    hipError_t herr2 = hipStreamSynchronize(s);
+    (void)hipFree(ws);
+    if (st < 0) return st;
+    TD_HIP_CHECK(herr);
+    TD_HIP_CHECK(herr2);
+    return TD_OK;
+}
+
+int64_t td_conv_split_pack(const float* w, int cout, int cin, int taps, uint8_t* out, int64_t out_bytes) {
+    TD_REQUIRE(w && cout >= 1 && cin >= 32 && cin % 32 == 0 && taps >= 1 && taps <= 64, "td_conv_split_pack: cout >= 1, cin a multiple of 32, 1 <= taps <= 64");
+    std::vector<unsigned char> packed;
+    conv_split_pack(w, cout, cin, packed, taps);
+    if (out && out_bytes >= (int64_t)packed.size()) memcpy(out, packed.data(), packed.size());
+    return (int64_t)packed.size();
+}
+
 td_status td_resize_bilinear_f64(const double* src, int c, int h, int w, float* dst, int out_h, int out_w, int dst_pitch_px,
                                  int64_t dst_plane_stride, void* stream) {
     return resize_bilinear_f64_launch(src, c, h, w, dst, out_h, out_w, dst_pitch_px, (long long)dst_plane_stride, static_cast<hipStream_t>(stream));
diff --git a/treedetection_amd/csrc/bottleneck.hip b/treedetection_amd/csrc/bottleneck.hip
--- a/treedetection_amd/csrc/bottleneck.hip
+++ b/treedetection_amd/csrc/bottleneck.hip
@@ -34,9 +34,10 @@
     static constexpr int BPC = 160 * 1024 / LDS_BYTES >= 4 ? 4 : 160 * 1024 / LDS_BYTES;
 };
 
-template <typename T, int MID, bool OVERLAP, int MT, bool FAST>
+template <typename T, int MID, bool OVERLAP, int MT, bool FAST, bool SPLIT = false>
 __device__ __forceinline__ void bottleneck_tail_body(const TailArgs& a, char* lds) {
     typedef TailGeom<T, MID, OVERLAP, MT, FAST> G;
+    static_assert(!SPLIT || (FAST && sizeof(T) == 4 && MID == 64 && MT == 1), "the split form is the fp32 64-row tail's");
     constexpr int ES = G::ES, KE = G::KE, KC = G::KC, BM = G::BM, LDROWS = G::LDROWS, NT1 = G::NT1;
     constexpr int AROWS = BM / LDROWS, BROWS1 = MID / LDROWS, BROWS3 = 128 / LDROWS;
     char* As = lds;
@@ -152,6 +153,79 @@
 #pragma unroll
             for (int r = 0; r < 16; ++r) acc2[i][j][r] = 0.f;
 
+    [[maybe_unused]] bool mid_only = false;
+    if constexpr (SPLIT) mid_only = a.mid_out != nullptr;
+    if constexpr (SPLIT) {
+        const int wk = wn;
+        const __amdgpu_buffer_rsrc_t wsrsrc = __builtin_amdgcn_make_buffer_rsrc(
+            const_cast<void*>(a.w2_split), 0, (MID / 32) * 9 * KC * SPLIT_CHUNK_BYTES, 0x00020000);
+        unsigned ws_off[2];
+#pragma unroll
+        for (int j = 0; j < 2; ++j) ws_off[j] = (unsigned)((j * KC + wk) * 9) * (unsigned)SPLIT_CHUNK_BYTES + (unsigned)lane * 16u;
+        auto stage_s = [&](int buf, int tap) {
+            const int ky = tap / 3, kx = tap - 3 * ky;
+            const unsigned xs = (unsigned)(ky * a.W + kx) * pix_bytes;
+#pragma unroll
+            for (int cc = 0; cc < KC; ++cc)
+#pragma unroll
+                for (int i = 0; i < AROWS; ++i) {
+                    const unsigned off = ((a_ok[i] >> tap) & 1u) ? a_off[i] + xs + (unsigned)cc * CHUNK_BYTES : OOB;
+                    char* dst = As + (((unsigned)buf * KC + (unsigned)cc) * BM + (unsigned)LDROWS * i + wave_rows) * CHUNK_BYTES;
+                    __builtin_amdgcn_raw_ptr_buffer_load_lds(xrsrc, (lds_void*)dst, 16, off, 0, 0, 0);
+                }
+        };
+        auto load_f = [&](f32x4 (&f)[2][3], int tap, int sl) {
+#pragma unroll
+            for (int j = 0; j < 2; ++j)
+#pragma unroll
+                for (int q = 0; q < 3; ++q)
+                    f[j][q] = __builtin_bit_cast(f32x4, __builtin_amdgcn_raw_buffer_load_b128(
+                        wsrsrc, ws_off[j], tap * SPLIT_CHUNK_BYTES + (3 * sl + q) * 1024, 0));
+        };
+        auto mma6 = [&](const bf16x8 (&pa)[3], const f32x4 (&f)[2][3], f32x16 (&acc)[2]) {
+            constexpr int PA[6] = {0, 2, 1, 0, 1, 0}, QB[6] = {2, 0, 1, 1, 0, 0};
+#pragma unroll
+            for (int t = 0; t < 6; ++t)
+#pragma unroll
+                for (int j = 0; j < 2; ++j)
+                    acc[j] = __builtin_amdgcn_mfma_f32_32x32x16_bf16(pa[PA[t]], __builtin_bit_cast(bf16x8, f[j][QB[t]]), acc[j], 0, 0, 0);
+        };
+        f32x16 accs[2];
+#pragma unroll
+        for (int j = 0; j < 2; ++j)
+#pragma unroll
+            for (int r = 0; r < 16; ++r) accs[j][r] = 0.f;
+        f32x4 fb[2][2][3];
+        stage_s(0, 0);
+        load_f(fb[0], 0, 0);
+        asm volatile("s_waitcnt vmcnt(0)" ::: "memory");
+        __builtin_amdgcn_s_barrier();
+        for (int tap = 0; tap < 9; ++tap) {
+            const int cur = tap & 1;
+            load_f(fb[1], tap, 1);
+            if (tap + 1 < 9) stage_s(cur ^ 1, tap + 1);
+            const char* Ab = As + ((cur * KC + wk) * BM + wm * 32) * CHUNK_BYTES;
+            bf16x8 pa[2][3];
+#pragma unroll
+            for (int sl = 0; sl < 2; ++sl)
+                split8(*reinterpret_cast<const f32x4*>(Ab + frag_off[2 * sl]), *reinterpret_cast<const f32x4*>(Ab + frag_off[2 * sl + 1]), pa[sl]);
+            mma6(pa[0], fb[0], accs);
+            if (tap + 1 < 9) load_f(fb[0], tap + 1, 0);
+            mma6(pa[1], fb[1], accs);
+            asm volatile("s_waitcnt vmcnt(6)" ::: "memory");
+            asm volatile("s_waitcnt lgkmcnt(0)" ::: "memory");
+            __builtin_amdgcn_s_barrier();
+        }
+        float* X = reinterpret_cast<float*>(T2s);
+#pragma unroll
+        for (int r = 0; r < 16; ++r) X[wave * 1024 + r * 64 + lane] = wk ? accs[0][r] : accs[1][r];
+        asm volatile("s_waitcnt lgkmcnt(0)" ::: "memory");
+        __builtin_amdgcn_s_barrier();
+#pragma unroll
+        for (int r = 0; r < 16; ++r) acc2[0][0][r] = __fadd_rn(wk ? accs[1][r] : accs[0][r], X[(wave ^ 1) * 1024 + r * 64 + lane]);
+        asm volatile("s_waitcnt lgkmcnt(0)" ::: "memory");
+        __builtin_amdgcn_s_barrier();
+    } else {
 #if defined(TD_TAIL_DIAG) && (TD_TAIL_DIAG & 1)
     if (false)
 #endif
@@ -184,6 +258,7 @@
         asm volatile("s_waitcnt vmcnt(0)" ::: "memory");
         asm volatile("s_waitcnt lgkmcnt(0)" ::: "memory");
         __builtin_amdgcn_s_barrier();
+    }
     }
 
     auto stage_w3 = [&](int nc) {
@@ -197,7 +272,7 @@
                 __builtin_amdgcn_raw_ptr_buffer_load_lds(w3rsrc, (lds_void*)dst, 16, off, 0, 0, 0);
             }
     };
-    stage_w3(0);
+    if (!mid_only) stage_w3(0);
 
     typedef unsigned u32x4 __attribute__((ext_vector_type(4)));
     constexpr int NDMA3 = KC * BROWS3;
@@ -265,6 +340,9 @@
                     t = t > 0.f ? t : 0.f;
                     const unsigned row = (unsigned)(wm * 32 * MT + i * 32 + (q & 3) + 8 * (q >> 2) + 4 * (lane >> 5));
                     *reinterpret_cast<float*>(T2s + (c * BM + row) * CHUNK_BYTES + ((piece ^ ((row >> 1) & 7)) << 4) + inb) = t;
+                    if constexpr (SPLIT) {
+                        if (mid_only && m0 + (int)row < M) a.mid_out[(size_t)(m0 + (int)row) * MID + n] = t;
+                    }
                 }
             } else {
                 const int odd = lane & 1;
@@ -296,6 +374,9 @@
         asm volatile("s_waitcnt vmcnt(0) lgkmcnt(0)" ::: "memory");
     }
     __builtin_amdgcn_s_barrier();
+    if constexpr (SPLIT) {
+        if (mid_only) return;
+    }
 
 #if defined(TD_TAIL_DIAG) && (TD_TAIL_DIAG & 2)
     if (tid == 0 && m0 == 0x7fffff00) static_cast<T*>(a.y)[0] = *reinterpret_cast<const T*>(T2s);
@@ -527,19 +608,19 @@
     }
 }
 
-template <typename T, int MID, bool OVERLAP, int MT, bool FAST, int BPC>
+template <typename T, int MID, bool OVERLAP, int MT, bool FAST, int BPC, bool SPLIT = false>
 __global__ __launch_bounds__(256, BPC)
 void bottleneck_tail_kernel(const TailArgs a) {
     static_assert(BPC >= 1 && BPC * TailGeom<T, MID, OVERLAP, MT, FAST>::LDS_BYTES <= 160 * 1024, "LDS footprint does not allow that many blocks per CU");
     __shared__ __attribute__((aligned(16))) char lds[TailGeom<T, MID, OVERLAP, MT, FAST>::LDS_BYTES];
-    bottleneck_tail_body<T, MID, OVERLAP, MT, FAST>(a, lds);
-}
-
-template <typename T, int MID, bool OVERLAP, int MT, bool FAST = false>
+    bottleneck_tail_body<T, MID, OVERLAP, MT, FAST, SPLIT>(a, lds);
+}
+
+template <typename T, int MID, bool OVERLAP, int MT, bool FAST = false, bool SPLIT = false>
 td_status launch_tail(const TailArgs& a, hipStream_t stream) {
     typedef TailGeom<T, MID, OVERLAP, MT, FAST> G;
     const int tiles = td_cdiv(a.M, G::BM);
-    hipLaunchKernelGGL((bottleneck_tail_kernel<T, MID, OVERLAP, MT, FAST, G::BPC>), dim3(tiles), dim3(256), 0, stream, a);
+    hipLaunchKernelGGL((bottleneck_tail_kernel<T, MID, OVERLAP, MT, FAST, G::BPC, SPLIT>), dim3(tiles), dim3(256), 0, stream, a);
     TD_KERNEL_CHECK();
     return TD_OK;
 }
@@ -550,6 +631,10 @@
     if (cout != 4 * mid) return false;
     if (precision == TD_PRECISION_FP32) return mid == 64;
     return mid == 64 || mid == 128;
+}
+
+bool bottleneck_tail_split_ok(int precision, int mid, int cout, long long M) {
+    return precision == TD_PRECISION_FP32 && mid == 64 && cout == 4 * mid && M > 0 && (size_t)M * cout * 4 < 0xfffffff0ull - (1u << 20);
 }
 
 td_status bottleneck_tail_launch(const TailArgs& a, int precision, hipStream_t stream) {
@@ -557,6 +642,12 @@
     TD_REQUIRE(a.M == a.B * a.H * a.W && a.M > 0, "bottleneck tail: M must be B*H*W");
     const size_t es = precision == TD_PRECISION_FP16 ? 2 : 4;
     TD_REQUIRE((size_t)a.M * a.MID * es < 0xfffffff0ull - (1u << 20), "bottleneck tail: input tensor must stay below 4 GB (32-bit buffer offsets)");
+    if (a.w2_split) {
+        TD_REQUIRE(bottleneck_tail_split_ok(precision, a.MID, a.COUT, a.M), "bottleneck tail: the split form runs fp32, mid 64, outputs below 4 GB");
+        TD_REQUIRE(a.mid_out || (a.w3 && a.y), "bottleneck tail: the split form needs the 1x1's filters and an output, or mid_out");
+        return launch_tail<float, 64, false, 1, true, true>(a, stream);
+    }
+    TD_REQUIRE(!a.mid_out, "bottleneck tail: mid_out is the split form's (w2_split)");
     static const int forced = getenv("TD_TAIL_BM") ? atoi(getenv("TD_TAIL_BM")) : 0;
     const int bm = forced == 64 || forced == 128 ? forced : 64;
     static const int fast_env32 = getenv("TD_TAIL_FAST") ? atoi(getenv("TD_TAIL_FAST")) : 1;
diff --git a/treedetection_amd/csrc/common.h b/treedetection_amd/csrc/common.h
--- a/treedetection_amd/csrc/common.h
+++ b/treedetection_amd/csrc/common.h
@@ -136,7 +136,7 @@
 td_status conv_bd_launch(const ConvArgs& a, int precision, int variant, hipStream_t stream);
 bool conv_bs_ok(const ConvArgs& a, int precision);
 td_status conv_bs_launch(const ConvArgs& a, int precision, hipStream_t stream);
-void conv_split_pack(const float* w, int cout, int cin, std::vector<unsigned char>& out);
+void conv_split_pack(const float* w, int cout, int cin, std::vector<unsigned char>& out, int taps = 1);
 bool conv_split_ok(const ConvArgs& a, int precision);
 td_status conv_split_launch(const ConvArgs& a, int variant, hipStream_t stream);
 td_status wino_gemm_launch(const ConvArgs& a, hipStream_t stream);
@@ -152,8 +152,11 @@
     const void* res;
     void* y;
     int B, H, W, MID, COUT, M;
+    const void* w2_split;
+    float* mid_out;
 };
 bool bottleneck_tail_ok(int precision, int mid, int cout);
+bool bottleneck_tail_split_ok(int precision, int mid, int cout, long long M);
 td_status bottleneck_tail_launch(const TailArgs& a, int precision, hipStream_t stream);
 
 td_status wino_input_launch(const float* x, int B, int H, int W, int C, float* V, const int* m_dyn, int m_mul, long long t0, int Ts,
diff --git a/treedetection_amd/csrc/conv_split.hip b/treedetection_amd/csrc/conv_split.hip
--- a/treedetection_amd/csrc/conv_split.hip
+++ b/treedetection_amd/csrc/conv_split.hip
@@ -4,35 +4,11 @@
 
 namespace {
 
-typedef __bf16 bf16x8 __attribute__((ext_vector_type(8)));
-typedef __bf16 bf16x2 __attribute__((ext_vector_type(2)));
-typedef float f32x2 __attribute__((ext_vector_type(2)));
 typedef unsigned u32x4 __attribute__((ext_vector_type(4)));
-
-constexpr int SPLIT_CHUNK_BYTES = 6144;
 
 template <int... R, class F>
 __device__ __forceinline__ void static_for(std::integer_sequence<int, R...>, F&& f) {
     (f(std::integral_constant<int, R>{}), ...);
-}
-
-__device__ __forceinline__ void split8(const f32x4& lo, const f32x4& hi, bf16x8 (&p)[3]) {
-    u32x4 w[3];
-#pragma unroll
-    for (int e = 0; e < 4; ++e) {
-        f32x2 v = e < 2 ? f32x2{lo[2 * e], lo[2 * e + 1]} : f32x2{hi[2 * e - 4], hi[2 * e - 3]};
-#pragma unroll
-        for (int k = 0; k < 3; ++k) {
-            const unsigned u = __builtin_bit_cast(unsigned, __builtin_convertvector(v, bf16x2));
-            w[k][e] = u;
-            if (k < 2) {
-                const f32x2 back = {__builtin_bit_cast(float, u << 16), __builtin_bit_cast(float, u & 0xffff0000u)};
-                v = v - back;
-            }
-        }
-    }
-#pragma unroll
-    for (int k = 0; k < 3; ++k) p[k] = __builtin_bit_cast(bf16x8, w[k]);
 }
 
 template <int MT, int NT, int WM, int WN>
@@ -277,8 +253,8 @@
 
 }
 
-void conv_split_pack(const float* w, int cout, int cin, std::vector<unsigned char>& out) {
-    const int nit = cin / 32, nt32 = (cout + 31) / 32;
+void conv_split_pack(const float* w, int cout, int cin, std::vector<unsigned char>& out, int taps) {
+    const int nit = taps * (cin / 32), nt32 = (cout + 31) / 32;
     out.assign((size_t)nt32 * nit * SPLIT_CHUNK_BYTES, (unsigned char)0);
     unsigned short* o = reinterpret_cast<unsigned short*>(out.data());
     for (int t = 0; t < nt32; ++t)
@@ -287,8 +263,9 @@
                 for (int l = 0; l < 64; ++l) {
                     const int n = t * 32 + (l & 31), h = l >> 5;
                     if (n >= cout) continue;
+                    const int cc = c / taps, tap = c - cc * taps;
                     for (int e = 0; e < 8; ++e) {
-                        float v = w[(size_t)n * cin + (size_t)c * 32 + 16 * s + 8 * (e >> 2) + 4 * h + (e & 3)];
+                        float v = w[((size_t)n * taps + tap) * cin + (size_t)cc * 32 + 16 * s + 8 * (e >> 2) + 4 * h + (e & 3)];
                         for (int p = 0; p < 3; ++p) {
                             const unsigned short b = bf16_rne(v);
                             o[(((((size_t)t * nit + c) * 2 + s) * 3 + p) * 64 + l) * 8 + e] = b;
diff --git a/treedetection_amd/csrc/conv_tiles.h b/treedetection_amd/csrc/conv_tiles.h
--- a/treedetection_amd/csrc/conv_tiles.h
+++ b/treedetection_amd/csrc/conv_tiles.h
@@ -57,6 +57,32 @@
     }
     static __device__ __forceinline__ float to_f32(_Float16 v) { return (float)v; }
 };
+
+typedef __bf16 bf16x8 __attribute__((ext_vector_type(8)));
+typedef __bf16 bf16x2 __attribute__((ext_vector_type(2)));
+typedef float f32x2 __attribute__((ext_vector_type(2)));
+
+constexpr int SPLIT_CHUNK_BYTES = 6144;
+
+__device__ __forceinline__ void split8(const f32x4& lo, const f32x4& hi, bf16x8 (&p)[3]) {
+    typedef unsigned u32x4 __attribute__((ext_vector_type(4)));
+    u32x4 w[3];
+#pragma unroll
+    for (int e = 0; e < 4; ++e) {
+        f32x2 v = e < 2 ? f32x2{lo[2 * e], lo[2 * e + 1]} : f32x2{hi[2 * e - 4], hi[2 * e - 3]};
+#pragma unroll
+        for (int k = 0; k < 3; ++k) {
+            const unsigned u = __builtin_bit_cast(unsigned, __builtin_convertvector(v, bf16x2));
+            w[k][e] = u;
+            if (k < 2) {
+                const f32x2 back = {__builtin_bit_cast(float, u << 16), __builtin_bit_cast(float, u & 0xffff0000u)};
+                v = v - back;
+            }
+        }
+    }
+#pragma unroll
+    for (int k = 0; k < 3; ++k) p[k] = __builtin_bit_cast(bf16x8, w[k]);
+}
 
 template <typename TO, int MT, int NT, int WM, int WN, int RWM, bool WIDE_OK = true>
 constexpr int conv_epilogue_lds_bytes() {
diff --git a/treedetection_amd/csrc/engine.cpp b/treedetection_amd/csrc/engine.cpp
--- a/treedetection_amd/csrc/engine.cpp
+++ b/treedetection_amd/csrc/engine.cpp
@@ -37,6 +37,7 @@
     bool out_f32 = false;
     void* w_frag = nullptr;
     void* w_split = nullptr;
+    void* w_tail_split = nullptr;
     float* wino_u = nullptr;
     float* wino_u43 = nullptr;
 };
@@ -90,6 +91,7 @@
     int wino43_min = 12;
     int wino_fold = 39;
     int f32_split = SPLIT_DEFAULT;
+    bool f32_split_tail = true;
     std::string tune_cache;
     void* tune_evict = nullptr;
     size_t tune_evict_bytes = 0;
@@ -190,6 +192,19 @@
     unsigned char* d = nullptr;
     td_status st = upload(e, packed, &d);
     L.w_split = d;
+    return st;
+}
+
+td_status upload_tail_split(td_engine* e, const std::vector<float>& w_ohwi, ConvLayer& L, int cout3) {
+    L.w_tail_split = nullptr;
+    if (!e->f32_split_tail || L.kh != 3 || L.kw != 3 || L.cin != L.cout || !bottleneck_tail_split_ok(e->desc.precision, L.cout, cout3, 1) ||
+        (size_t)L.cout * 9 * L.cin != w_ohwi.size())
+        return TD_OK;
+    std::vector<unsigned char> packed;
+    conv_split_pack(w_ohwi.data(), L.cout, L.cin, packed, 9);
+    unsigned char* d = nullptr;
+    td_status st = upload(e, packed, &d);
+    L.w_tail_split = d;
     return st;
 }
 
@@ -429,6 +444,7 @@
     if (const char* gl = getenv("TD_GROUP_LEVELS")) e->group_levels = atoi(gl) != 0;
     if (const char* ft = getenv("TD_FUSE_TAIL")) { e->fuse_tail = atoi(ft) != 0; e->fuse_tail_fp16 = atoi(ft) == 2; }
     if (const char* sp = getenv("TD_F32_SPLIT")) e->f32_split = atoi(sp);
+    if (const char* spt = getenv("TD_F32_SPLIT_TAIL")) e->f32_split_tail = atoi(spt) != 0;
     e->desc = d;
     read_rule_switches(e);
     load_tune_cache(e);
@@ -529,6 +545,7 @@
             if ((st = load_conv_bn(e, tm, p + ".conv1", blk.c1, si > 0 ? SPLIT_CONV1 : 0)) < 0) return st;
             if ((st = load_conv_bn(e, tm, p + ".conv2", blk.c2)) < 0) return st;
             if ((st = load_conv_bn(e, tm, p + ".conv3", blk.c3, si > 0 ? SPLIT_CONV3 : 0)) < 0) return st;
+            if (si == 0 && (st = upload_tail_split(e, pack_ohwi(tm.at(p + ".conv2.weight")), blk.c2, blk.c3.cout)) < 0) return st;
             blk.has_sc = tm.find(p + ".shortcut.weight") != tm.end();
             if (blk.has_sc && (st = load_conv_bn(e, tm, p + ".shortcut", blk.sc, si > 0 ? SPLIT_SHORTCUT : 0)) < 0) return st;
             e->stages[si].push_back(blk);
@@ -913,21 +930,33 @@
         ClassScope cs(e, s_, TD_CLS_CONV3X3, flops, bytes);
         return conv_pp8_grouped_launch(a, s_);
     };
-    auto run_tail = [&](const Block& blk, const void* t1_, int B_, int H_, int W_, void* y_, const void* shortcut_, hipStream_t s_) -> td_status {
+    auto run_tail = [&](const Block& blk, const void* t1_, int B_, int H_, int W_, void* y_, const void* shortcut_, hipStream_t s_,
+                        bool split_ = false, void* mid_out_ = nullptr) -> td_status {
         TailArgs a{};
         a.x = t1_; a.w2 = blk.c2.w; a.scale2 = blk.c2.scale; a.bias2 = blk.c2.bias;
         a.w3 = blk.c3.w; a.scale3 = blk.c3.scale; a.bias3 = blk.c3.bias; a.res = shortcut_; a.y = y_;
         a.B = B_; a.H = H_; a.W = W_; a.MID = blk.c2.cout; a.COUT = blk.c3.cout; a.M = B_ * H_ * W_;
+        if (split_) a.w2_split = blk.c2.w_tail_split;
         const double M = (double)a.M, mid = a.MID, co = a.COUT, es = prec == TD_PRECISION_FP16 ? 2.0 : 4.0;
-        const double flops = 2.0 * M * mid * (9.0 * mid) + 2.0 * M * co * mid;
-        const double bytes = es * (M * mid + 2.0 * M * co + 9.0 * mid * mid + co * mid);
+        const double f2 = 2.0 * M * mid * (9.0 * mid), f2pipe = split_ ? f2 * 6.0 / 16.0 : f2, w2b = (split_ ? 6.0 : es) * 9.0 * mid * mid;
+        if (mid_out_) {
+            a.mid_out = static_cast<float*>(mid_out_);
+            a.w3 = nullptr; a.scale3 = nullptr; a.bias3 = nullptr; a.res = nullptr; a.y = nullptr;
+            const double bytes = es * 2.0 * M * mid + w2b;
+            ProfScope ps(e, s_, 0, f2, bytes);
+            if (e->prof) e->prof_flops[8] += f2pipe;
+            ClassScope cs(e, s_, TD_CLS_CONV3X3, f2pipe, bytes);
+            return bottleneck_tail_launch(a, prec, s_);
+        }
+        const double f3 = 2.0 * M * co * mid, flops = f2 + f3;
+        const double bytes = es * (M * mid + 2.0 * M * co + co * mid) + w2b;
         ProfScope ps(e, s_, 0, flops, bytes);
         if (e->prof) {
-            e->prof_flops[8] += flops;
+            e->prof_flops[8] += f2pipe + f3;
             e->prof_launches[0] += 1;
             e->prof_bytes[0] += es * 2.0 * M * mid;
         }
-        ClassScope cs(e, s_, TD_CLS_TAIL, flops, bytes);
+        ClassScope cs(e, s_, TD_CLS_TAIL, f2pipe + f3, bytes);
         return bottleneck_tail_launch(a, prec, s_);
     };
     const WsGeom g = engine_geom(e, B, Hp, Wp);
@@ -979,9 +1008,15 @@
                     shortcut = scb;
                 }
                 if ((st = run_conv(e, blk.c1, x, nb_img, xh, xw, blk.stride, 0, true, t1, nullptr, 0, s)) < 0) return st;
-                if (e->fuse_tail && (blk.c2.cout == 64 || e->fuse_tail_fp16) && blk.c2.kh == 3 && blk.c2.kw == 3 &&
-                    blk.c2.cin == blk.c2.cout && blk.c3.cin == blk.c2.cout && bottleneck_tail_ok(prec, blk.c2.cout, blk.c3.cout)) {
-                    if ((st = run_tail(blk, t1, nb_img, oh, ow, y, shortcut, s)) < 0) return st;
+                const bool tail_shape = blk.c2.kh == 3 && blk.c2.kw == 3 && blk.c2.cin == blk.c2.cout && blk.c3.cin == blk.c2.cout &&
+                                        bottleneck_tail_ok(prec, blk.c2.cout, blk.c3.cout);
+                const bool split_tail = tail_shape && blk.c2.w_tail_split &&
+                                        bottleneck_tail_split_ok(prec, blk.c2.cout, blk.c3.cout, (long long)nb_img * oh * ow);
+                if (e->fuse_tail && (blk.c2.cout == 64 || e->fuse_tail_fp16) && tail_shape) {
+                    if ((st = run_tail(blk, t1, nb_img, oh, ow, y, shortcut, s, split_tail)) < 0) return st;
+                } else if (split_tail) {
+                    if ((st = run_tail(blk, t1, nb_img, oh, ow, nullptr, nullptr, s, true, t2)) < 0) return st;
+                    if ((st = run_conv(e, blk.c3, t2, nb_img, oh, ow, 1, 0, true, y, shortcut, 0, s)) < 0) return st;
                 } else {
                     if ((st = run_conv(e, blk.c2, t1, nb_img, oh, ow, 1, 1, true, t2, nullptr, 0, s)) < 0) return st;
                     if ((st = run_conv(e, blk.c3, t2, nb_img, oh, ow, 1, 0, true, y, shortcut, 0, s)) < 0) return st;
```

After: 739.4 (median of 6 runs). 1.01x the previous value.
